# casys-kaist/CoVA

Measured on AMD Instinct MI355X. Metric: compressed-domain frames/sec (BlobNet+bboxcc) at 1080p b=256, higher is better.
Workload: dtype f16

## Files before the change

cova_amd/_lib.py:

```python
from __future__ import annotations

import ctypes as C
import os

import numpy as np

_HERE = os.path.dirname(os.path.abspath(__file__))
LIB_PATH = os.path.join(_HERE, "libcovahip.so")

OK = 0
MEM_HOST, MEM_DEVICE = 0, 1
AU_DELTA_UNIT, AU_DISCONT, AU_DROPPABLE = 1, 2, 4


class CovahipError(RuntimeError):
    def __init__(self, status: int, where: str, detail: str = ""):
        self.status = status
        try:
            text = lib().covahip_strerror(status).decode()
        except AttributeError:
            text = "error"
        msg = f"{where}: {text} (status {status})"
        if detail:
            msg += f" [{detail}]"
# ... 114 lines not shown
    "covahip_memcpy_h2d": (C.c_int, [_P, _P, _P, _SZ]),
    "covahip_memcpy_d2h": (C.c_int, [_P, _P, _P, _SZ]),
    "covahip_memset": (C.c_int, [_P, _P, C.c_int, _SZ]),
    "covahip_timer_start": (C.c_int, [_P, C.c_int]),
    "covahip_timer_stop": (C.c_int, [_P, C.c_int]),
    "covahip_timer_elapsed_ms": (C.c_int, [_P, C.c_int, C.POINTER(C.c_float)]),
    "covahip_profile_enable": (C.c_int, [_P, C.c_int]),
    "covahip_profile_filter": (C.c_int, [_P, C.c_char_p]),
    "covahip_profile_reset": (C.c_int, [_P]),
    "covahip_profile_read": (C.c_int, [_P, _P, C.c_int, C.POINTER(C.c_int)]),
    "covahip_blobnet_load": (C.c_int, [_P, _P, _SZ, C.c_int, C.c_int, C.c_int, C.c_int]),
    "covahip_blobnet_forward": (C.c_int, [_P, _P, C.c_int, _P, _P, C.c_int]),
    "covahip_blobnet_macs_per_frame": (C.c_int, [_P, C.POINTER(C.c_int64)]),
    "covahip_bboxcc": (C.c_int, [_P, _P, C.c_int, C.c_int, C.c_int, C.c_int, _P, _P, C.c_int, C.c_int]),
    "covahip_filter_forward": (C.c_int, [_P, _P, C.c_int, C.c_int, _P, _P, C.c_int, _P, _P, C.c_int]),
    "covahip_filter_forward_frames": (C.c_int, [_P, _P, C.c_int, _P, C.c_int, C.c_int, _P, _P, C.c_int, _P, _P, C.c_int]),
    "covahip_pipe_create": (C.c_int, [_P, C.c_int, C.c_int, C.c_int, C.c_int, C.c_int, C.POINTER(_P)]),
    "covahip_pipe_destroy": (None, [_P]),
    "covahip_pipe_set_packed": (C.c_int, [_P, C.c_int]),
    "covahip_pipe_set_blocking_wait": (C.c_int, [_P, C.c_int]),
    "covahip_pipe_acquire": (C.c_int, [_P, C.POINTER(C.c_int), C.POINTER(_P), C.POINTER(_P)]),
    "covahip_pipe_submit": (C.c_int, [_P, C.c_int, C.c_int, C.c_int, C.c_int]),
    "covahip_pipe_wait": (C.c_int, [_P, C.c_int]),
    "covahip_pipe_abort": (C.c_int, [_P, C.c_int]),
    "covahip_pipe_collect": (C.c_int, [_P, C.c_int, C.POINTER(_P), C.POINTER(_P), C.POINTER(_P), C.POINTER(_P)]),
    "covahip_pipe_release": (C.c_int, [_P, C.c_int]),
    "covahip_boxes_to_bbox": (None, [_P, C.c_int, _P]),
    "covahip_bbox_serialize_vec": (_SZ, [_P, _SZ, _P, _SZ, C.POINTER(C.c_int)]),
    "covahip_bbox_deserialize_vec": (C.c_int, [_P, _SZ, _P, _SZ, C.POINTER(_SZ)]),
    "covahip_frame_serialize": (_SZ, [C.c_uint64, C.c_uint64, _P, _SZ, _P, _SZ, C.POINTER(C.c_int)]),
    "covahip_bbox_iou": (C.c_float, [_P, _P]),
    "covahip_tfrecord_example": (_SZ, [_P, _P, C.c_int, C.c_int, C.c_int, C.c_int, _P, _SZ, C.POINTER(C.c_int)]),
    "covahip_bbox_csv": (_SZ, [_P, _SZ, C.c_int, _P, _SZ, C.POINTER(C.c_int)]),
    "covahip_tracks_export": (_SZ, [C.c_uint64, C.c_uint64, _P, _P, _SZ, _P, _SZ, C.POINTER(C.c_int)]),
    "covahip_assoc_default_cfg": (None, [C.POINTER(AssocCfg)]),
    "covahip_assoc_new": (C.c_int, [C.POINTER(AssocCfg), _P, _SZ, C.POINTER(_P)]),
    "covahip_assoc_free": (None, [_P]),
    "covahip_assoc_push_track": (C.c_int, [_P, C.c_uint64, C.c_uint64, _P, _SZ]),
    "covahip_assoc_push_track_frame": (C.c_int, [_P, _P, _SZ]),
    "covahip_assoc_push_dnn": (C.c_int, [_P, _P, _SZ]),
    "covahip_assoc_push_dnn_text": (C.c_int, [_P, C.c_char_p, _SZ]),
    "covahip_assoc_terminate": (C.c_int, [_P]),
    "covahip_assoc_csv": (_SZ, [_P, C.c_int, _P, _SZ, C.POINTER(C.c_int)]),
    "covahip_h264_open_mp4": (C.c_int, [_P, _SZ, C.POINTER(_P)]),
    "covahip_h264_close": (None, [_P]),
    "covahip_h264_get_info": (C.c_int, [_P, _P]),
    "covahip_h264_sample": (C.c_int, [_P, C.c_int, C.POINTER(C.c_uint64), C.POINTER(C.c_uint32), C.POINTER(C.c_int)]),
    "covahip_h264_sample_slices": (C.c_int, [_P, C.c_int, _P, C.c_int, C.POINTER(C.c_int)]),
    "covahip_h264_decode_records": (C.c_int, [_P, C.c_int, _P, _SZ]),
    "covahip_h264_display_order": (C.c_int, [_P, C.c_void_p, C.c_int, C.POINTER(C.c_int)]),
    "covahip_h264_colocated": (C.c_int, [_P, C.c_int, C.POINTER(C.c_int), C.POINTER(C.c_int)]),
    "covahip_h264_open_avcc": (C.c_int, [_P, _SZ, C.POINTER(_P)]),
    "covahip_h264_decode_au": (C.c_int, [_P, _P, _SZ, _P, _SZ, _P, C.POINTER(C.c_int64)]),
    "covahip_carrier_write_records": (C.c_int, [_P, _P, _P, C.c_int, C.c_int, _P, _SZ]),
    "covahip_carrier_pack": (None, [_P, _SZ, _P]),
    "covahip_filter_forward_frames_packed": (C.c_int, [_P, _P, C.c_int, _P, C.c_int, C.c_int, _P, _P, C.c_int, _P, _P]),
    "covahip_blobnet_load_set": (C.c_int, [_P, C.c_int, _P, _P, C.c_int, C.c_int, C.c_int, C.c_int]),
    "covahip_blobnet_num_models": (C.c_int, [_P, _P]),
    "covahip_blobnet_set_post": (C.c_int, [_P, C.c_int, C.POINTER(BlobNetPost)]),
    "covahip_blobnet_get_post": (C.c_int, [_P, C.c_int, C.POINTER(C.c_float), _P, C.POINTER(C.c_int)]),
    "covahip_blobnet_set_area": (C.c_int, [_P, C.c_int, C.c_int]),
    "covahip_blobnet_get_area": (C.c_int, [_P, C.c_int, C.POINTER(C.c_int)]),
    "covahip_bboxcc_v": (C.c_int, [_P, _P, C.c_int, C.c_int, C.c_int, _P, _P, _P, C.c_int, C.c_int]),
    "covahip_pipe_model_ids": (C.c_int, [_P, C.c_int, _P]),
    "covahip_blobnet_forward_m": (C.c_int, [_P, _P, _P, C.c_int, _P, _P, C.c_int]),
    "covahip_filter_forward_m": (C.c_int, [_P, _P, _P, C.c_int, C.c_int, _P, _P, C.c_int, _P, _P, C.c_int]),
    "covahip_filter_forward_frames_m": (C.c_int, [_P, _P, C.c_int, _P, _P, C.c_int, C.c_int, _P, _P, C.c_int, _P, _P, C.c_int]),
    "covahip_filter_forward_frames_packed_m": (C.c_int, [_P, _P, C.c_int, _P, _P, C.c_int, C.c_int, _P, _P, C.c_int, _P, _P]),
    "covahip_stack_new": (C.c_int, [_SZ, C.c_uint, C.c_uint, C.POINTER(_P)]),
    "covahip_stack_free": (None, [_P]),
    "covahip_stack_push": (C.c_int, [_P, _P, _SZ, _P, _SZ, C.POINTER(C.c_int)]),
    "covahip_stack_out_dims": (None, [C.c_int, C.c_int, C.c_uint, C.POINTER(C.c_int), C.POINTER(C.c_int)]),
    "covahip_sort_new": (C.c_int, [C.c_uint64, C.c_uint64, C.c_float, C.POINTER(_P)]),
    "covahip_sort_free": (None, [_P]),
    "covahip_sort_update": (C.c_int, [_P, _P, _SZ, C.c_uint64, _P, _SZ, C.POINTER(_SZ), _P, _SZ, C.POINTER(_SZ)]),
    "covahip_sort_finalize": (C.c_int, [_P, _P, _SZ, C.POINTER(_SZ), _P, _SZ, C.POINTER(_SZ)]),
    "covahip_sort_mark_seen": (C.c_int, [_P, C.c_uint64]),
    "covahip_sort_num_trackers": (C.c_int, [_P, C.POINTER(_SZ)]),
    "covahip_sort_tracker_info": (C.c_int, [_P, _SZ, C.POINTER(C.c_uint64), C.POINTER(C.c_int),
                                            C.POINTER(C.c_uint64), C.POINTER(C.c_uint64), _P]),
    "covahip_sort_tracker_predict": (C.c_int, [_P, _SZ, C.c_uint64, _P]),
    "covahip_sort_tracker_update": (C.c_int, [_P, _SZ, _P]),
    "covahip_linear_assignment": (_SZ, [_P, _SZ, _SZ, _P, _SZ]),
    "covahip_gopfilter_default_cfg": (None, [C.POINTER(GopFilterCfg)]),
    "covahip_gopfilter_new": (C.c_int, [C.POINTER(GopFilterCfg), C.POINTER(_P)]),
    "covahip_gopfilter_free": (None, [_P]),
    "covahip_gopfilter_push_enc": (C.c_int, [_P, C.c_uint64, C.c_uint64, C.c_uint32]),
    "covahip_gopfilter_push_boxes": (C.c_int, [_P, _P, _SZ, C.c_uint64, _P, _SZ, C.POINTER(_SZ)]),
    "covahip_gopfilter_eos": (C.c_int, [_P, _P, _SZ, C.POINTER(_SZ)]),
    "covahip_gopfilter_take_dropped": (C.c_int, [_P, _P, _SZ, C.POINTER(_SZ)]),
    "covahip_gopfilter_take_track_export": (_SZ, [_P, _P, _SZ, C.POINTER(C.c_int)]),
    "covahip_gopfilter_counters": (C.c_int, [_P, C.POINTER(C.c_uint64), C.POINTER(C.c_uint64),
                                             C.POINTER(C.c_uint64)]),
    "covahip_train_default_cfg": (None, [C.POINTER(TrainCfg)]),
    "covahip_train_create": (C.c_int, [_P, C.POINTER(TrainCfg), _P, _SZ, C.POINTER(_P)]),
    "covahip_train_step": (C.c_int, [_P, _P, _P, C.c_int, C.c_float, C.POINTER(C.c_float), C.c_int]),
    "covahip_train_metrics": (C.c_int, [_P, C.POINTER(C.c_int64)]),
    "covahip_train_weights": (C.c_int, [_P, _P, _SZ, C.POINTER(_SZ)]),
    "covahip_train_grads": (C.c_int, [_P, _P, _SZ]),
    "covahip_train_create_set": (C.c_int, [_P, C.POINTER(TrainCfg), C.c_int, _P, _P, _P, C.POINTER(_P)]),
    "covahip_train_num_models": (C.c_int, [_P, C.POINTER(C.c_int)]),
    "covahip_train_step_set": (C.c_int, [_P, _P, _P, _P, _P, _P, C.c_int]),
    "covahip_train_metrics_m": (C.c_int, [_P, C.c_int, C.POINTER(C.c_int64)]),
    "covahip_train_weights_m": (C.c_int, [_P, C.c_int, _P, _SZ, C.POINTER(_SZ)]),
    "covahip_train_grads_m": (C.c_int, [_P, C.c_int, _P, _SZ]),
    "covahip_train_eval": (C.c_int, [_P, _P, _P, C.c_int, _P, _P, C.POINTER(TrainEvalResult), C.c_int]),
    "covahip_train_eval_set": (C.c_int, [_P, _P, _P, _P, _P, _P, C.POINTER(TrainEvalResult), C.c_int]),
    "covahip_train_state_size": (C.c_int, [_P, C.POINTER(_SZ)]),
    "covahip_train_save_state": (C.c_int, [_P, C.c_uint64, _P, _SZ, C.POINTER(_SZ)]),
    "covahip_train_load_state": (C.c_int, [_P, _P, _SZ, C.POINTER(C.c_uint64)]),
    "covahip_train_set_plan": (C.c_int, [_P, C.POINTER(TrainPlan)]),
    "covahip_train_get_plan": (C.c_int, [_P, C.POINTER(TrainPlan)]),
    "covahip_train_set_post": (C.c_int, [_P, C.c_int, C.POINTER(BlobNetPost)]),
    "covahip_train_get_post": (C.c_int, [_P, C.c_int, C.POINTER(C.c_float), _P, C.POINTER(C.c_int)]),
    "covahip_train_destroy": (None, [_P]),
    "covahip_train_data_create": (C.c_int, [_P, C.c_int, C.c_int, C.c_int64, C.POINTER(_P)]),
    "covahip_train_data_append": (C.c_int, [_P, _P, _P, C.c_int, C.c_int, C.POINTER(C.c_int64)]),
    "covahip_train_data_frames": (C.c_int, [_P, C.POINTER(C.c_int64)]),
    "covahip_train_data_gather": (C.c_int, [_P, _P, C.c_int, _P, _P, C.c_int]),
    "covahip_train_data_label_mass": (C.c_int, [_P, C.c_int64, C.c_int64, _P, _P, C.c_int]),
    "covahip_train_data_destroy": (None, [_P]),
    "covahip_train_step_data": (C.c_int, [_P, _P, _P, C.c_int, C.c_float, C.POINTER(C.c_float)]),
    "covahip_train_step_set_data": (C.c_int, [_P, _P, _P, _P, _P, _P]),
    "covahip_train_eval_data": (C.c_int, [_P, _P, _P, C.c_int, _P, _P, C.POINTER(TrainEvalResult), C.c_int]),
    "covahip_train_eval_set_data": (C.c_int, [_P, _P, _P, _P, _P, _P, C.POINTER(TrainEvalResult), C.c_int]),
    "covahip_post_sweep": (C.c_int, [_P, C.POINTER(SweepCfg), _P, _P, C.c_int, C.c_int, _P, _P, _P, C.POINTER(SweepResult)]),
    "covahip_post_heat_begin": (C.c_int, [_P, C.POINTER(HeatCfg)]),
    "covahip_post_heat_add": (C.c_int, [_P, _P, _P, C.c_int, C.c_int]),
    "covahip_post_heat_end": (C.c_int, [_P, _P, _P, _P, C.POINTER(C.c_int64)]),
    "covahip_monitor_begin": (C.c_int, [_P, C.POINTER(MonitorCfg)]),
    "covahip_monitor_add": (C.c_int, [_P, _P, _P, _P, _P, C.c_int, C.c_int]),
    "covahip_monitor_read": (C.c_int, [_P, C.c_int, _P, _P, _P, _P, _P, _P, C.POINTER(C.c_int64), C.POINTER(C.c_int64)]),
    "covahip_monitor_end": (C.c_int, [_P]),
    "covahip_mog_default_cfg": (None, [C.POINTER(MogCfg)]),
    "covahip_mog_create": (C.c_int, [_P, C.POINTER(MogCfg), C.POINTER(_P)]),
    "covahip_mog_create_grid": (C.c_int, [_P, C.POINTER(MogCfg), C.c_int, C.POINTER(_P)]),
    "covahip_mog_dims": (C.c_int, [_P, C.POINTER(C.c_int32), C.POINTER(C.c_int32), C.POINTER(C.c_int32), C.POINTER(C.c_int32)]),
    "covahip_mog_apply": (C.c_int, [_P, _P, C.c_int, _P, _P, C.c_int]),
    "covahip_mog_yuv_tight": (C.c_int, [_P, C.c_int, C.c_int, C.POINTER(MogYuv)]),
    "covahip_mog_apply_yuv": (C.c_int, [_P, C.POINTER(MogYuv), _P, C.c_int, _P, _P, C.c_int]),
    "covahip_mog_reset": (C.c_int, [_P, C.c_int]),
    "covahip_mog_destroy": (None, [_P]),
}

DEV_PROTOTYPES = {
    "covahip_blobnet_set_impl": (C.c_int, [_P, C.c_int]),
    "covahip_bboxcc_set_wave_cap": (C.c_int, [_P, C.c_int]),
    "covahip_blobnet_set_enc_plan": (C.c_int, [_P, C.c_int, C.c_int, C.c_int]),
    "covahip_dev_clock_mhz": (C.c_int, [_P, C.c_int, C.POINTER(C.c_float)]),
    "covahip_dev_graph_probe": (C.c_int, [_P, _P, C.c_int, _P, C.c_int, C.c_int, _P, _P, C.c_int, _P, C.c_int, C.POINTER(C.c_float),
                                          C.POINTER(C.c_float)]),
    "covahip_dev_bboxcc_overflow": (C.c_int, [_P, C.POINTER(C.c_int32)]),
    "covahip_dev_blobnet_tail_form": (C.c_int, [_P, C.POINTER(C.c_int)]),
    "covahip_dev_pipe_queue_plan": (C.c_int, [_P, C.POINTER(C.c_int), C.POINTER(C.c_int)]),
    "covahip_dev_blobnet_buffer": (C.c_int, [_P, C.c_int, C.c_int, C.POINTER(C.c_void_p), C.POINTER(C.c_size_t), C.POINTER(C.c_int32)]),
    "covahip_dev_mog_masks": (C.c_int, [_P, _P, _P, _SZ, C.POINTER(C.c_int)]),
    "covahip_dev_mog_state": (C.c_int, [_P, C.c_int, _P, _P, _P, _P, C.POINTER(C.c_int64)]),
    "covahip_dev_mog_set_stage_budget": (C.c_int, [_P, _SZ]),
    "covahip_dev_mog_post_masks": (C.c_int, [_P, _P, C.c_int, _P]),
    "covahip_dev_mog_set_post_form": (C.c_int, [_P, C.c_int, C.c_int]),
    "covahip_dev_mog_band_plan": (C.c_int, [C.c_int, C.c_int, C.POINTER(C.c_int), C.POINTER(C.c_int), C.POINTER(C.c_size_t)]),
    "covahip_dev_monitor_slice": (C.c_int, [_P, C.c_int]),
    "covahip_dev_heat_set_stage": (C.c_int, [_P, _SZ]),
    "covahip_dev_train_data_set_stage": (C.c_int, [_P, _SZ]),
}

_lib = None


def lib() -> C.CDLL:
    global _lib
    if _lib is None:
        san = os.environ.get("COVAHIP_HOST_SAN_LIB")
        if san:
            L = C.CDLL(san)
            for name, (res, args) in list(PROTOTYPES.items()) + list(DEV_PROTOTYPES.items()):
                fn = getattr(L, name, None)
                if fn is not None:
                    fn.restype = res
                    fn.argtypes = args
            _lib = L
            return _lib
        if not os.path.exists(LIB_PATH):
            raise ImportError(
                f"{LIB_PATH} not found: build it with `python -c 'import __graft_entry__ as g; g.build()'` "
                "or `make -C cova_amd/csrc` -- cova_amd has no CPU fallback")
        L = C.CDLL(LIB_PATH)
        for name, (res, args) in list(PROTOTYPES.items()) + list(DEV_PROTOTYPES.items()):
            fn = getattr(L, name)
            fn.restype = res
            fn.argtypes = args
        _lib = L
    return _lib


def check(status: int, where: str, ctx=None) -> None:
    if status != OK:
        detail = ""
        if ctx is not None and status == 3:
            detail = lib().covahip_last_hip_error(ctx).decode()
        raise CovahipError(status, where, detail)
```

cova_amd/csrc/blobnet.h:

```cpp
#pragma once
#include <hip/hip_fp16.h>

#include <vector>

#include "blobnet_params.h"
#include "internal.h"

constexpr int BN_KTAB_STACKS = 256;

struct BnLevelGeom {
    int H, W;
};

struct BnWorkspace {
    bool ready = false;
    __half *act[BN_LEVELS + 1] = {};
    __half *dact[BN_LEVELS] = {};
    __half *pbuf = nullptr;
    size_t pbuf_frames = 0;
    float *part = nullptr;
    ResidentTable<int32_t> index;
    int index_frames = 0;
    std::vector<int32_t> kept_table;
    ResidentTable<uint8_t> models;
    ResidentTable<int32_t> areas;
};

struct covahip_blobnet {
    int H = 0, W = 0, max_batch = 0;
    int n_models = 1;
    BnLevelGeom lv[BN_LEVELS + 1];
    int enc_c[BN_LEVELS + 1], dec_ci[BN_LEVELS], dec_co[BN_LEVELS];
    int dec_cy[BN_LEVELS], dec_cx[BN_LEVELS];
    BnWorkspace ws[COVAHIP_MAX_LANES];
    void *d_prepared = nullptr;
    size_t prepared_bytes = 0;
    struct Prepared *prep = nullptr;
    int fuse_tail = 1;
    int fuse_dec = 1;
    int enc1_tile16 = 1;
    int tail_rows = 1;
    int tail_part = 1;
    int fuse_enc23 = 1;
    int enc_rowtiles = 1;
    int64_t macs_per_frame = 0;
    std::vector<float> post_thr;
    std::vector<int32_t> post_area;
    bool area_on = false;
    std::vector<std::vector<uint8_t>> post_keep;
    bool post_on = false;
    void *d_post = nullptr;
    size_t post_area_off = 0, post_keep_off = 0, post_planes_off = 0, post_keep_stride = 0, post_planes_stride = 0, post_bytes = 0;
    covahip_blobnet() {
        std::copy(BN_ENC_C, BN_ENC_C + BN_LEVELS + 1, enc_c);
        std::copy(BN_DEC_CI, BN_DEC_CI + BN_LEVELS, dec_ci);
        std::copy(BN_DEC_CO, BN_DEC_CO + BN_LEVELS, dec_co);
    }
};

constexpr int BN_E1_MAXW = 62;
inline bool bn_level1_on_enc1(const covahip_ctx *ctx, const covahip_blobnet *m) {
    return m->enc1_tile16 && m->enc_c[1] == 16 && m->enc_c[2] == 32 && m->lv[1].W <= BN_E1_MAXW && m->lv[1].H >= 2 &&
           !ctx->enc_plan[1].nbands;
}

int blobnet_prepare_mfma(covahip_ctx *ctx, covahip_blobnet *m, const float *const *h_weights, int n_models);
void blobnet_release_mfma(covahip_ctx *ctx, covahip_blobnet *m);
struct BnCcTail {
    int area_thresh, max_boxes;
    covahip_box *boxes;
    int32_t *counts;
};
struct BnInput {
    const uint8_t *stack = nullptr;
    const uint8_t *frames = nullptr;
    int n_frames = 0;
    const int32_t *index = nullptr;
    const int32_t *h_index = nullptr;
    bool packed = false;
    bool dry = false;
    int model = 0;
    const uint8_t *model_ids = nullptr;
    const uint8_t *frame_models = nullptr;
    const uint8_t *h_model_ids = nullptr;
    bool mixed = false;
};
int blobnet_forward_mfma(covahip_ctx *ctx, covahip_blobnet *m, BnWorkspace &ws, const BnInput &in, int batch, float *d_logits,
                         uint8_t *d_mask, const BnCcTail *cc = nullptr, bool *cc_done = nullptr);
```

cova_amd/csrc/blobnet.hip:

```cpp
#include <algorithm>
#include <cmath>
#include <cstdlib>
#include <cstring>
#include <vector>

#include "blobnet.h"
#include "covahip_dev.h"

static void free_model(covahip_ctx *ctx, covahip_blobnet *m) {
    if (!m) return;
    blobnet_release_mfma(ctx, m);
    if (m->d_post) hipFree(m->d_post);
    for (BnWorkspace &ws : m->ws) {
        for (int i = 0; i <= BN_LEVELS; i++)
            if (ws.act[i]) hipFree(ws.act[i]);
        for (int j = 0; j < BN_LEVELS; j++)
            if (ws.dact[j]) hipFree(ws.dact[j]);
        if (ws.pbuf) hipFree(ws.pbuf);
        if (ws.part) hipFree(ws.part);
        ws.index.release();
        ws.models.release();
        ws.areas.release();
    }
    delete m;
}

void covahip_blobnet_destroy(covahip_ctx *ctx) {
    if (!ctx->blobnet) return;
    hipSetDevice(ctx->device);
    covahip_sync_all(ctx);
    covahip_monitor_close(ctx, true);
    free_model(ctx, ctx->blobnet);
    ctx->blobnet = nullptr;
}

int covahip_blobnet_geometry(covahip_ctx *ctx, int *h, int *w) {
    if (!ctx->blobnet) return COVAHIP_ERR_NOT_LOADED;
    *h = ctx->blobnet->H;
    *w = ctx->blobnet->W;
    return COVAHIP_OK;
}

static int check_model_ids(const covahip_blobnet *m, const uint8_t *model_ids, int batch) {
    if (model_ids)
        for (int b = 0; b < batch; b++)
            if (model_ids[b] >= m->n_models) return COVAHIP_ERR_INVALID_ARG;
    return COVAHIP_OK;
}

static int resolve_models(covahip_ctx *ctx, covahip_blobnet *m, BnWorkspace &ws, const uint8_t *model_ids, int batch,
                          const int32_t *table, int n_frames, BnInput &in) {
    in.model = 0;
    in.model_ids = nullptr;
    in.frame_models = nullptr;
    in.h_model_ids = nullptr;
    if (!model_ids) return COVAHIP_OK;
    if (int rc = check_model_ids(m, model_ids, batch)) return rc;
    bool uniform = true;
    for (int b = 1; b < batch && uniform; b++) uniform = model_ids[b] == model_ids[0];
    if (uniform) {
        in.model = model_ids[0];
        return COVAHIP_OK;
    }
    std::vector<uint8_t> ids((size_t)batch + n_frames, 0);
    std::vector<uint8_t> seen((size_t)n_frames, 0);
    std::copy(model_ids, model_ids + batch, ids.begin());
    for (int b = 0; b < batch; b++)
        for (int t = 0; t < BN_T; t++) {
            const int f = table ? table[(size_t)b * BN_T + t] : b * BN_T + t;
            uint8_t &fm = ids[(size_t)batch + f];
            if (seen[f] && fm != model_ids[b]) return COVAHIP_ERR_INVALID_ARG;
            seen[f] = 1;
            fm = model_ids[b];
        }
    if (int rc = ws.models.reserve(ctx, (size_t)m->max_batch * (1 + BN_T))) return rc;
    if (int rc = ws.models.upload(ctx, ids.data(), ids.size(), &in.model_ids)) return rc;
    in.frame_models = in.model_ids + batch;
    in.h_model_ids = model_ids;
    return COVAHIP_OK;
}

static int resolve_areas(covahip_ctx *ctx, covahip_blobnet *m, BnWorkspace &ws, const BnInput &in, int batch, int area_thresh,
                         const int32_t **d_out) {
    *d_out = nullptr;
    if (!m->area_on) return COVAHIP_OK;
    std::vector<int32_t> eff((size_t)batch);
    for (int b = 0; b < batch; b++) {
        const int32_t a = m->post_area[in.h_model_ids ? in.h_model_ids[b] : in.model];
        eff[b] = a >= 1 ? a : area_thresh;
    }
    if (int rc = ws.areas.reserve(ctx, (size_t)m->max_batch)) return rc;
    return ws.areas.upload(ctx, eff.data(), eff.size(), d_out);
}

static int ensure_pbuf(covahip_ctx *ctx, covahip_blobnet *m, BnWorkspace &ws, int n_frames);
static int filter_dev(covahip_ctx *ctx, BnInput &in, int batch, float *d_logits, uint8_t *d_mask,
                      bool with_cc, int area_thresh, covahip_box *d_boxes, int32_t *d_counts, int max_boxes,
                      const uint8_t *model_ids = nullptr) {
    covahip_blobnet *m = ctx->blobnet;
    if (!m) return COVAHIP_ERR_NOT_LOADED;
    if (batch > m->max_batch) return COVAHIP_ERR_INVALID_ARG;
    if (batch == 0) return COVAHIP_OK;
    if (in.stack) {
        int rc = resolve_models(ctx, m, m->ws[ctx->cur_lane], model_ids, batch, nullptr, batch * BN_T, in);
        if (rc) return rc;
        rc = ensure_pbuf(ctx, m, m->ws[ctx->cur_lane], batch * BN_T);
        if (rc) return rc;
    }
    BnCcTail tail{area_thresh, max_boxes, d_boxes, d_counts};
    bool cc_done = false;
    int rc = blobnet_forward_mfma(ctx, m, m->ws[ctx->cur_lane], in, batch, d_logits, d_mask, with_cc ? &tail : nullptr, &cc_done);
    if (rc) return rc;
    if (with_cc && !cc_done) {
        const int32_t *d_areas = nullptr;
        rc = resolve_areas(ctx, m, m->ws[ctx->cur_lane], in, batch, area_thresh, &d_areas);
        if (rc) return rc;
        rc = covahip_bboxcc_launch(ctx, d_mask, batch, m->H, m->W, area_thresh, d_boxes, d_counts, max_boxes, d_areas);
    }
    return rc;
}

static int prepare_frames(covahip_ctx *ctx, covahip_blobnet *m, BnWorkspace &ws, const uint8_t *d_frames, int n_frames,
                          const int32_t *stack_index, int batch, BnInput &in, const uint8_t *model_ids = nullptr) {
    if (n_frames < BN_T || n_frames > BN_T * m->max_batch) return COVAHIP_ERR_INVALID_ARG;
    if (!stack_index && batch != n_frames - (BN_T - 1)) return COVAHIP_ERR_INVALID_ARG;
    std::vector<int32_t> table((size_t)batch * BN_T);
    for (int b = 0; b < batch; b++)
        for (int t = 0; t < BN_T; t++) {
            const int32_t f = stack_index ? stack_index[b * BN_T + t] : b + (BN_T - 1) - t;
            if (f < 0 || f >= n_frames) return COVAHIP_ERR_INVALID_ARG;
            table[(size_t)b * BN_T + t] = f;
        }
    if (int rc = resolve_models(ctx, m, ws, model_ids, batch, table.data(), n_frames, in)) return rc;
    const bool by_value = batch <= BN_KTAB_STACKS && n_frames <= 65535 && bn_level1_on_enc1(ctx, m);
    in.frames = d_frames;
    in.n_frames = n_frames;
    if (by_value) {
        ws.kept_table = std::move(table);
        in.h_index = ws.kept_table.data();
    } else {
        if (n_frames != ws.index_frames) ws.index.invalidate();
        if (int rc = ws.index.reserve(ctx, (size_t)m->max_batch * BN_T)) return rc;
        if (int rc = ws.index.upload(ctx, table.data(), table.size(), &in.index)) return rc;
        ws.index_frames = n_frames;
    }
    return ensure_pbuf(ctx, m, ws, n_frames);
}

static int ensure_pbuf(covahip_ctx *ctx, covahip_blobnet *m, BnWorkspace &ws, int n_frames) {
    if (ws.pbuf_frames < (size_t)n_frames) {
        const size_t want = std::min((size_t)BN_T * m->max_batch, std::max((size_t)n_frames, 2 * ws.pbuf_frames));
        const size_t bytes = want * m->lv[1].H * m->lv[1].W * m->enc_c[1] * sizeof(__half);
        if (ws.pbuf) {
            COVAHIP_CHECK_HIP(ctx, hipStreamSynchronize(ctx->stream));
            COVAHIP_CHECK_HIP(ctx, hipFree(ws.pbuf));
            ws.pbuf = nullptr;
            ws.pbuf_frames = 0;
        }
        COVAHIP_CHECK_HIP(ctx, hipMalloc((void **)&ws.pbuf, bytes));
        COVAHIP_CHECK_HIP(ctx, hipMemsetAsync(ws.pbuf, 0, bytes, ctx->stream));
        ws.pbuf_frames = want;
    }
    return COVAHIP_OK;
}

int covahip_blobnet_forward_dev(covahip_ctx *ctx, const uint8_t *d_stack, int batch, float *d_logits,
                                uint8_t *d_mask, const uint8_t *model_ids) {
    BnInput in;
    in.stack = d_stack;
    return filter_dev(ctx, in, batch, d_logits, d_mask, false, 0, nullptr, nullptr, 0, model_ids);
}

static int alloc_workspace(covahip_ctx *ctx, covahip_blobnet *m, BnWorkspace &ws) {
    if (ws.ready) return COVAHIP_OK;
    for (int i = 1; i <= BN_LEVELS; i++) {
        const size_t tt = (i == BN_LEVELS) ? 1 : BN_T;
        const size_t n = (size_t)m->max_batch * tt * m->lv[i].H * m->lv[i].W * m->enc_c[i];
        COVAHIP_CHECK_HIP(ctx, hipMalloc((void **)&ws.act[i], n * sizeof(__half)));
        COVAHIP_CHECK_HIP(ctx, hipMemsetAsync(ws.act[i], 0, n * sizeof(__half), ctx->stream));
    }
    for (int j = 0; j < BN_LEVELS - 1; j++) {
        const BnLevelGeom out = m->lv[BN_LEVELS - 1 - j];
        const size_t n = (size_t)m->max_batch * out.H * out.W * m->dec_co[j];
        COVAHIP_CHECK_HIP(ctx, hipMalloc((void **)&ws.dact[j], n * sizeof(__half)));
    }
    COVAHIP_CHECK_HIP(ctx, hipMalloc((void **)&ws.part, (size_t)m->max_batch * (m->lv[1].H + 1) * (m->lv[1].W + 1) * 4 * sizeof(float)));
    ws.ready = true;
    return COVAHIP_OK;
}

int covahip_blobnet_grow_lanes(covahip_ctx *ctx, int n_lanes) {
    covahip_blobnet *m = ctx->blobnet;
    if (!m) return COVAHIP_OK;
    for (int k = 0; k < n_lanes && k < COVAHIP_MAX_LANES; k++) {
        const int rc = alloc_workspace(ctx, m, m->ws[k]);
        if (rc) return rc;
    }
    COVAHIP_CHECK_HIP(ctx, hipStreamSynchronize(ctx->stream));
    return COVAHIP_OK;
}

static int build_model(covahip_ctx *ctx, covahip_blobnet *m, const float *const *h_w, int n_models, int h_mb, int w_mb, int max_batch) {
    m->H = h_mb;
    m->W = w_mb;
    m->max_batch = max_batch;
    m->lv[0] = {h_mb, w_mb};
    for (int i = 0; i < BN_LEVELS; i++) m->lv[i + 1] = {(m->lv[i].H + 1) / 2, (m->lv[i].W + 1) / 2};
    for (int j = 0; j < BN_LEVELS; j++) {
        const BnLevelGeom in = m->lv[BN_LEVELS - j], out = m->lv[BN_LEVELS - 1 - j];
        const int ph = 2 * in.H + 2 - out.H, pw = 2 * in.W + 2 - out.W;
        if (ph < 0 || pw < 0) return COVAHIP_ERR_UNSUPPORTED;
        m->dec_cy[j] = ph / 2 + ph % 2;
        m->dec_cx[j] = pw / 2 + pw % 2;
    }
    int64_t macs = 0;
    for (int i = 0; i < BN_LEVELS; i++) {
        macs += (int64_t)BN_T * m->lv[i].H * m->lv[i].W * 9 * m->enc_c[i] * m->enc_c[i + 1];
        macs += (int64_t)m->lv[i + 1].H * m->lv[i + 1].W * m->enc_c[i + 1] * 32;
    }
    for (int j = 0; j < BN_LEVELS; j++) {
        const BnLevelGeom in = m->lv[BN_LEVELS - j];
        macs += (int64_t)in.H * in.W * 16 * m->dec_ci[j] * m->dec_co[j];
    }
    macs += (int64_t)h_mb * w_mb * 16;
    m->macs_per_frame = macs;

    for (int k = 0; k < ctx->n_lanes; k++) {
        const int rc = alloc_workspace(ctx, m, m->ws[k]);
        if (rc) return rc;
    }
    int rc = blobnet_prepare_mfma(ctx, m, h_w, n_models);
    if (rc) return rc;
    m->post_thr.assign(n_models, 0.f);
    m->post_keep.assign(n_models, {});
    m->post_area.assign(n_models, 0);
    BnInput plan;
    plan.dry = true;
    for (int pass = 0; pass < (n_models > 1 ? 8 : 4) && !rc; pass++) {
        const int b = (pass & 1) ? max_batch : 1;
        plan.n_frames = (pass & 2) ? b + BN_T - 1 : 0;
        plan.mixed = (pass & 4) != 0;
        rc = blobnet_forward_mfma(ctx, m, m->ws[0], plan, b, nullptr, nullptr, nullptr, nullptr);
    }
    return rc;
}

extern "C" {

int covahip_blobnet_load(covahip_ctx *ctx, const void *weights, size_t weights_bytes, int h_mb, int w_mb, int t,
                         int max_batch) {
    if (!ctx || !weights) return COVAHIP_ERR_INVALID_ARG;
    if (t == BN_T && h_mb >= 16 && w_mb >= 16 && h_mb <= 1024 && w_mb <= 1024 && max_batch > 0 && !bn_check_blob(weights, weights_bytes))
        return COVAHIP_ERR_BAD_WEIGHTS;
    return covahip_blobnet_load_set(ctx, 1, &weights, &weights_bytes, h_mb, w_mb, t, max_batch);
}

int covahip_blobnet_load_set(covahip_ctx *ctx, int n_models, const void *const *weights, const size_t *weights_bytes, int h_mb,
                             int w_mb, int t, int max_batch) {
    if (!ctx || !weights || !weights_bytes || h_mb <= 0 || w_mb <= 0 || max_batch <= 0) return COVAHIP_ERR_INVALID_ARG;
    if (n_models < 1 || n_models > COVAHIP_MAX_MODELS) return COVAHIP_ERR_INVALID_ARG;
    for (int k = 0; k < n_models; k++)
        if (!weights[k]) return COVAHIP_ERR_INVALID_ARG;
    if (t != BN_T) return COVAHIP_ERR_UNSUPPORTED;
    if (h_mb < 16 || w_mb < 16 || h_mb > 1024 || w_mb > 1024) return COVAHIP_ERR_UNSUPPORTED;
    std::vector<const float *> h_w(n_models);
    bool bad = false;
    for (int k = 0; k < n_models; k++) bad = bad || !(h_w[k] = bn_check_blob(weights[k], weights_bytes[k]));

    COVAHIP_CHECK_HIP(ctx, hipSetDevice(ctx->device));
    covahip_blobnet_destroy(ctx);
    if (bad) return COVAHIP_ERR_BAD_WEIGHTS;
    covahip_blobnet *m = new covahip_blobnet();
    int rc = build_model(ctx, m, h_w.data(), n_models, h_mb, w_mb, max_batch);
    if (rc == COVAHIP_OK && hipStreamSynchronize(ctx->stream) != hipSuccess) rc = COVAHIP_ERR_HIP;
    if (rc) {
        hipStreamSynchronize(ctx->stream);
        (void)hipGetLastError();
        free_model(ctx, m);
        return rc;
    }
    ctx->blobnet = m;
    return COVAHIP_OK;
}

int covahip_blobnet_num_models(covahip_ctx *ctx, int *n_models) {
    if (!ctx || !n_models) return COVAHIP_ERR_INVALID_ARG;
    if (!ctx->blobnet) return COVAHIP_ERR_NOT_LOADED;
    *n_models = ctx->blobnet->n_models;
    return COVAHIP_OK;
}

static int upload_post(covahip_ctx *ctx, covahip_blobnet *m) {
    const size_t hw = (size_t)m->H * m->W, n = (size_t)m->n_models;
    if (!m->d_post) {
        m->post_keep_stride = (hw + 15) & ~(size_t)15;
        m->post_planes_stride = (size_t)m->H * 16;
        m->post_area_off = n * sizeof(float);
        m->post_keep_off = align256(m->post_area_off + n * sizeof(int32_t));
        m->post_planes_off = align256(m->post_keep_off + n * m->post_keep_stride);
        m->post_bytes = m->post_planes_off + n * m->post_planes_stride;
        COVAHIP_CHECK_HIP(ctx, hipMalloc(&m->d_post, m->post_bytes));
    }
    std::vector<uint8_t> host(m->post_bytes, 0);
    std::memcpy(host.data(), m->post_thr.data(), n * sizeof(float));
    std::memcpy(host.data() + m->post_area_off, m->post_area.data(), n * sizeof(int32_t));
    for (size_t k = 0; k < n; k++) {
        uint8_t *kb = host.data() + m->post_keep_off + k * m->post_keep_stride;
        uint32_t *kp = reinterpret_cast<uint32_t *>(host.data() + m->post_planes_off + k * m->post_planes_stride);
        const std::vector<uint8_t> &keep = m->post_keep[k];
        for (int y = 0; y < m->H; y++)
            for (int x = 0; x < m->W; x++) {
                const bool on = keep.empty() || keep[(size_t)y * m->W + x];
                kb[(size_t)y * m->W + x] = on ? 1 : 0;
                if (on && x < 128) kp[y * 4 + 2 * (x & 1) + (x >> 6)] |= 1u << ((x >> 1) & 31);
            }
    }
    COVAHIP_CHECK_HIP(ctx, hipMemcpy(m->d_post, host.data(), host.size(), hipMemcpyHostToDevice));
    return COVAHIP_OK;
}

static int commit_post(covahip_ctx *ctx, covahip_blobnet *m) {
    bool on = false, area = false;
    for (int k = 0; k < m->n_models; k++) {
        area = area || m->post_area[k] >= 1;
        on = on || m->post_thr[k] != 0.f || !m->post_keep[k].empty() || m->post_area[k] >= 1;
    }
    if (on || m->d_post) {
        if (int rc = upload_post(ctx, m)) {
            m->post_thr.assign(m->n_models, 0.f);
            m->post_keep.assign(m->n_models, {});
            m->post_area.assign(m->n_models, 0);
            m->post_on = m->area_on = false;
            return rc;
        }
    }
    m->post_on = on;
    m->area_on = area;
    return COVAHIP_OK;
}

int covahip_blobnet_set_post(covahip_ctx *ctx, int model, const covahip_blobnet_post *post) {
    if (!ctx) return COVAHIP_ERR_INVALID_ARG;
    covahip_blobnet *m = ctx->blobnet;
    if (!m) return COVAHIP_ERR_NOT_LOADED;
    if (model < 0 || model >= m->n_models) return COVAHIP_ERR_INVALID_ARG;
    if (post && !std::isfinite(post->logit_thresh)) return COVAHIP_ERR_INVALID_ARG;
    COVAHIP_CHECK_HIP(ctx, hipSetDevice(ctx->device));
    if (int rc = covahip_sync_all(ctx)) return rc;
    const size_t hw = (size_t)m->H * m->W;
    m->post_thr[model] = post ? post->logit_thresh : 0.f;
    m->post_keep[model].clear();
    if (post && post->keep) {
        m->post_keep[model].resize(hw);
        for (size_t i = 0; i < hw; i++) m->post_keep[model][i] = post->keep[i] ? 1 : 0;
    }
    return commit_post(ctx, m);
}

int covahip_blobnet_set_area(covahip_ctx *ctx, int model, int area_thresh) {
    if (!ctx) return COVAHIP_ERR_INVALID_ARG;
    covahip_blobnet *m = ctx->blobnet;
    if (!m) return COVAHIP_ERR_NOT_LOADED;
    if (model < 0 || model >= m->n_models || area_thresh < 0) return COVAHIP_ERR_INVALID_ARG;
    COVAHIP_CHECK_HIP(ctx, hipSetDevice(ctx->device));
    if (int rc = covahip_sync_all(ctx)) return rc;
    m->post_area[model] = area_thresh;
    return commit_post(ctx, m);
}

int covahip_blobnet_get_area(covahip_ctx *ctx, int model, int *area_thresh) {
    if (!ctx || !area_thresh) return COVAHIP_ERR_INVALID_ARG;
    covahip_blobnet *m = ctx->blobnet;
    if (!m) return COVAHIP_ERR_NOT_LOADED;
    if (model < 0 || model >= m->n_models) return COVAHIP_ERR_INVALID_ARG;
    *area_thresh = m->post_area[model];
    return COVAHIP_OK;
}

int covahip_blobnet_get_post(covahip_ctx *ctx, int model, float *logit_thresh, uint8_t *keep_or_null, int *has_keep) {
    if (!ctx) return COVAHIP_ERR_INVALID_ARG;
    covahip_blobnet *m = ctx->blobnet;
    if (!m) return COVAHIP_ERR_NOT_LOADED;
    if (model < 0 || model >= m->n_models) return COVAHIP_ERR_INVALID_ARG;
    const std::vector<uint8_t> &keep = m->post_keep[model];
    if (logit_thresh) *logit_thresh = m->post_thr[model];
    if (has_keep) *has_keep = keep.empty() ? 0 : 1;
    if (keep_or_null) {
        const size_t hw = (size_t)m->H * m->W;
        if (keep.empty()) std::memset(keep_or_null, 1, hw);
        else std::memcpy(keep_or_null, keep.data(), hw);
    }
    return COVAHIP_OK;
}

int covahip_blobnet_macs_per_frame(covahip_ctx *ctx, int64_t *macs) {
    if (!ctx || !macs) return COVAHIP_ERR_INVALID_ARG;
    if (!ctx->blobnet) return COVAHIP_ERR_NOT_LOADED;
    *macs = ctx->blobnet->macs_per_frame;
    return COVAHIP_OK;
}

int covahip_blobnet_set_enc_plan(covahip_ctx *ctx, int level, int nbands, int nbuf) {
    if (!ctx || level < 1 || level > 3 || nbands < 0 || nbands > 64 || (nbands && nbuf != 1 && nbuf != 2)) return COVAHIP_ERR_INVALID_ARG;
    ctx->enc_plan[level].nbands = nbands;
    ctx->enc_plan[level].nbuf = nbands ? nbuf : 0;
    return COVAHIP_OK;
}

int covahip_blobnet_set_impl(covahip_ctx *ctx, int impl) {
    if (!ctx || !ctx->blobnet) return COVAHIP_ERR_NOT_LOADED;
    if (impl != 1 && (impl < 4 || impl > 10)) return COVAHIP_ERR_INVALID_ARG;
    ctx->blobnet->fuse_dec = impl != 4;
    ctx->blobnet->enc1_tile16 = impl != 5;
    ctx->blobnet->enc_rowtiles = impl != 6;
    ctx->blobnet->fuse_enc23 = impl == 7 ? 0 : impl == 8 ? 2 : 1;
    ctx->blobnet->tail_part = impl != 9;
    ctx->blobnet->tail_rows = impl != 10;
    return COVAHIP_OK;
}

static int filter_placed(covahip_ctx *ctx, covahip_blobnet *m, const uint8_t *d_src, int n_frames, const int32_t *stack_index,
                         int batch, int area_thresh, covahip_box *d_boxes, int32_t *d_counts, int max_boxes, float *d_logits,
                         uint8_t *d_mask, bool packed = false, const uint8_t *model_ids = nullptr) {
    if (!d_mask) {
        CtxLane &l = ctx->lane();
        int rc = covahip_ensure_buffer(ctx, &l.cc_scratch, &l.cc_scratch_bytes, (size_t)batch * m->H * m->W);
        if (rc) return rc;
        d_mask = (uint8_t *)l.cc_scratch;
    }
    BnInput in;
    if (n_frames > 0) {
        int rc = prepare_frames(ctx, m, m->ws[ctx->cur_lane], d_src, n_frames, stack_index, batch, in, model_ids);
        if (rc) return rc;
        in.packed = packed;
    } else {
        in.stack = d_src;
    }
    int rc = filter_dev(ctx, in, batch, d_logits, d_mask, true, area_thresh, d_boxes, d_counts, max_boxes, n_frames > 0 ? nullptr : model_ids);
    if (rc == COVAHIP_OK && batch > 0 && ctx->mon && ctx->mon->attached && !ctx->mon_suspended)
        rc = covahip_monitor_hook(ctx, d_mask, d_counts, d_boxes, max_boxes, model_ids, batch);
    return rc;
}

static int filter_any(covahip_ctx *ctx, const uint8_t *src, int n_frames, const int32_t *stack_index, int batch,
                      int area_thresh, covahip_box *boxes, int32_t *counts, int max_boxes, float *logits, uint8_t *mask,
                      int mem_kind, const uint8_t *model_ids = nullptr) {
    if (!ctx || batch < 0 || max_boxes < 0 || n_frames < 0) return COVAHIP_ERR_INVALID_ARG;
    covahip_blobnet *m = ctx->blobnet;
    if (!m) return COVAHIP_ERR_NOT_LOADED;
    if (batch == 0) return COVAHIP_OK;
    if (!src || !counts || (!boxes && max_boxes > 0) || batch > m->max_batch) return COVAHIP_ERR_INVALID_ARG;
    if (int rc = check_model_ids(m, model_ids, batch)) return rc;
    COVAHIP_CHECK_HIP(ctx, hipSetDevice(ctx->device));
    const bool by_frames = n_frames > 0;
    const size_t hw = (size_t)m->H * m->W;
    const size_t in_bytes = by_frames ? (size_t)n_frames * hw * 4 : (size_t)batch * BN_T * hw * 4;
    const size_t mask_bytes = (size_t)batch * hw;
    const size_t logit_bytes = mask_bytes * sizeof(float);
    const size_t box_bytes = (size_t)batch * max_boxes * sizeof(covahip_box);
    const size_t cnt_bytes = (size_t)batch * sizeof(int32_t);
    if (mem_kind != COVAHIP_MEM_DEVICE && mem_kind != COVAHIP_MEM_HOST) return COVAHIP_ERR_INVALID_ARG;

    if (mem_kind == COVAHIP_MEM_DEVICE) {
        LaneScope lane(ctx);
        if (!lane.ok()) return COVAHIP_ERR_HIP;
        return filter_placed(ctx, m, src, n_frames, stack_index, batch, area_thresh, boxes, counts, max_boxes, logits, mask, false, model_ids);
    }
    if (int rc = covahip_primary_op(ctx)) return rc;
    const uint8_t *d_src = src;
    int rc = covahip_ensure_buffer(ctx, &ctx->stage_in, &ctx->stage_in_bytes, in_bytes);
    if (rc) return rc;
    rc = covahip_ensure_buffer(ctx, &ctx->stage_out, &ctx->stage_out_bytes,
                               align256(mask_bytes) + align256(logit_bytes) + align256(box_bytes) + align256(cnt_bytes));
    if (rc) return rc;
    uint8_t *base = (uint8_t *)ctx->stage_out;
    uint8_t *d_mask = base;
    float *d_logits = logits ? (float *)(base + align256(mask_bytes)) : nullptr;
    covahip_box *d_boxes = (covahip_box *)(base + align256(mask_bytes) + align256(logit_bytes));
    int32_t *d_counts = (int32_t *)(base + align256(mask_bytes) + align256(logit_bytes) + align256(box_bytes));
    COVAHIP_CHECK_HIP(ctx, hipMemcpyAsync(ctx->stage_in, src, in_bytes, hipMemcpyHostToDevice, ctx->stream));
    d_src = (const uint8_t *)ctx->stage_in;
    rc = filter_placed(ctx, m, d_src, n_frames, stack_index, batch, area_thresh, d_boxes, d_counts, max_boxes, d_logits, d_mask, false,
                       model_ids);
    if (rc) return rc;
    if (logits) COVAHIP_CHECK_HIP(ctx, hipMemcpyAsync(logits, d_logits, logit_bytes, hipMemcpyDeviceToHost, ctx->stream));
    if (mask) COVAHIP_CHECK_HIP(ctx, hipMemcpyAsync(mask, d_mask, mask_bytes, hipMemcpyDeviceToHost, ctx->stream));
    if (box_bytes) COVAHIP_CHECK_HIP(ctx, hipMemcpyAsync(boxes, d_boxes, box_bytes, hipMemcpyDeviceToHost, ctx->stream));
    COVAHIP_CHECK_HIP(ctx, hipMemcpyAsync(counts, d_counts, cnt_bytes, hipMemcpyDeviceToHost, ctx->stream));
    COVAHIP_CHECK_HIP(ctx, hipStreamSynchronize(ctx->stream));
    return COVAHIP_OK;
}

int covahip_filter_forward(covahip_ctx *ctx, const uint8_t *rgba_stack, int batch, int area_thresh,
                           covahip_box *boxes, int32_t *counts, int max_boxes, float *logits, uint8_t *mask,
                           int mem_kind) {
    return filter_any(ctx, rgba_stack, 0, nullptr, batch, area_thresh, boxes, counts, max_boxes, logits, mask, mem_kind);
}

int covahip_filter_forward_m(covahip_ctx *ctx, const uint8_t *rgba_stack, const uint8_t *model_ids, int batch, int area_thresh,
                             covahip_box *boxes, int32_t *counts, int max_boxes, float *logits, uint8_t *mask, int mem_kind) {
    return filter_any(ctx, rgba_stack, 0, nullptr, batch, area_thresh, boxes, counts, max_boxes, logits, mask, mem_kind, model_ids);
}

int covahip_filter_forward_frames(covahip_ctx *ctx, const uint8_t *frames, int n_frames, const int32_t *stack_index,
                                  int batch, int area_thresh, covahip_box *boxes, int32_t *counts, int max_boxes,
                                  float *logits, uint8_t *mask, int mem_kind) {
    if (n_frames <= 0) return COVAHIP_ERR_INVALID_ARG;
    return filter_any(ctx, frames, n_frames, stack_index, batch, area_thresh, boxes, counts, max_boxes, logits, mask, mem_kind);
}

int covahip_filter_forward_frames_m(covahip_ctx *ctx, const uint8_t *frames, int n_frames, const int32_t *stack_index,
                                    const uint8_t *model_ids, int batch, int area_thresh, covahip_box *boxes, int32_t *counts,
                                    int max_boxes, float *logits, uint8_t *mask, int mem_kind) {
    if (n_frames <= 0) return COVAHIP_ERR_INVALID_ARG;
    return filter_any(ctx, frames, n_frames, stack_index, batch, area_thresh, boxes, counts, max_boxes, logits, mask, mem_kind,
                      model_ids);
}

int covahip_filter_forward_frames_packed(covahip_ctx *ctx, const uint16_t *d_records, int n_frames, const int32_t *stack_index,
                                         int batch, int area_thresh, covahip_box *d_boxes, int32_t *d_counts, int max_boxes,
                                         float *d_logits, uint8_t *d_mask) {
    return covahip_filter_forward_frames_packed_m(ctx, d_records, n_frames, stack_index, nullptr, batch, area_thresh, d_boxes,
                                                  d_counts, max_boxes, d_logits, d_mask);
}

int covahip_filter_forward_frames_packed_m(covahip_ctx *ctx, const uint16_t *d_records, int n_frames, const int32_t *stack_index,
                                           const uint8_t *model_ids, int batch, int area_thresh, covahip_box *d_boxes,
                                           int32_t *d_counts, int max_boxes, float *d_logits, uint8_t *d_mask) {
    if (!ctx || batch < 0 || max_boxes < 0 || n_frames <= 0) return COVAHIP_ERR_INVALID_ARG;
    covahip_blobnet *m = ctx->blobnet;
    if (!m) return COVAHIP_ERR_NOT_LOADED;
    if (batch == 0) return COVAHIP_OK;
    if (!d_records || !d_counts || (!d_boxes && max_boxes > 0) || batch > m->max_batch) return COVAHIP_ERR_INVALID_ARG;
    if (int rc = check_model_ids(m, model_ids, batch)) return rc;
    COVAHIP_CHECK_HIP(ctx, hipSetDevice(ctx->device));
    LaneScope lane(ctx);
    if (!lane.ok()) return COVAHIP_ERR_HIP;
    return filter_placed(ctx, m, reinterpret_cast<const uint8_t *>(d_records), n_frames, stack_index, batch, area_thresh, d_boxes, d_counts,
                         max_boxes, d_logits, d_mask, true, model_ids);
}

int covahip_dev_blobnet_tail_form(covahip_ctx *ctx, int *form) {
    if (!ctx || !form) return COVAHIP_ERR_INVALID_ARG;
    *form = ctx->tail_form;
    return COVAHIP_OK;
}

int covahip_dev_blobnet_buffer(covahip_ctx *ctx, int which, int index, void **dptr, size_t *bytes, int32_t dims[5]) {
    if (!ctx || !dptr || !bytes || !dims) return COVAHIP_ERR_INVALID_ARG;
    covahip_blobnet *m = ctx->blobnet;
    if (!m) return COVAHIP_ERR_NOT_LOADED;
    const BnWorkspace &ws = m->ws[0];
    int64_t d[5] = {0, 0, 0, 0, 0};
    size_t elem = sizeof(__half);
    void *p = nullptr;
    if (which == 0 && index == 0) {
        p = ws.pbuf;
        d[0] = (int64_t)ws.pbuf_frames; d[1] = m->lv[1].H; d[2] = m->lv[1].W; d[3] = m->enc_c[1];
    } else if (which == 1 && index >= 1 && index <= BN_LEVELS) {
        p = ws.act[index];
        const BnLevelGeom g = m->lv[index];
        if (index < BN_LEVELS) { d[0] = m->max_batch; d[1] = BN_T; d[2] = g.H; d[3] = g.W; d[4] = m->enc_c[index]; }
        else { d[0] = m->max_batch; d[1] = g.H; d[2] = g.W; d[3] = m->enc_c[index]; }
    } else if (which == 2 && index >= 0 && index < BN_LEVELS - 1) {
        p = ws.dact[index];
        const BnLevelGeom g = m->lv[BN_LEVELS - 1 - index];
        d[0] = m->max_batch; d[1] = g.H; d[2] = g.W; d[3] = m->dec_co[index];
    } else if (which == 3 && index == 0) {
        p = ws.part;
        elem = sizeof(float);
        d[0] = m->max_batch; d[1] = m->lv[1].H + 1; d[2] = m->lv[1].W + 1; d[3] = 4;
    } else {
        return COVAHIP_ERR_INVALID_ARG;
    }
    size_t n = p ? elem : 0;
    for (int k = 0; k < 5; k++) {
        dims[k] = p ? (int32_t)d[k] : 0;
        if (d[k]) n *= (size_t)d[k];
    }
    *dptr = p;
    *bytes = n;
    return COVAHIP_OK;
}

int covahip_dev_graph_probe(covahip_ctx *ctx, const uint8_t *d_frames, int n_frames, const int32_t *stack_index, int batch,
                            int area_thresh, covahip_box *d_boxes, int32_t *d_counts, int max_boxes, uint8_t *d_mask, int iters,
                            float *ms_direct, float *ms_graph) {
    if (!ctx || !ctx->blobnet || !ms_direct || !ms_graph || iters < 1) return COVAHIP_ERR_INVALID_ARG;
    covahip_blobnet *m = ctx->blobnet;
    COVAHIP_CHECK_HIP(ctx, hipSetDevice(ctx->device));
    if (int rc = covahip_primary_op(ctx)) return rc;
    if (!m->fuse_tail) return COVAHIP_ERR_UNSUPPORTED;
    hipEvent_t e0 = nullptr, e1 = nullptr;
    hipGraph_t graph = nullptr;
    hipGraphExec_t exec = nullptr;
    int rc = COVAHIP_OK;
    auto hip_ok = [&](hipError_t e, const char *what) {
        if (e == hipSuccess || rc) return e == hipSuccess;
        ctx->last_hip_error = std::string(what) + ": " + hipGetErrorString(e);
        rc = COVAHIP_ERR_HIP;
        return false;
    };
    auto run = [&](int n) {
        for (int i = 0; i < n && !rc; i++)
            rc = filter_placed(ctx, m, d_frames, n_frames, stack_index, batch, area_thresh, d_boxes, d_counts, max_boxes, nullptr, d_mask);
    };
    bool capturing = false;
    const bool was_suspended = ctx->mon_suspended;
    ctx->mon_suspended = true;
    do {
        if (!hip_ok(hipEventCreate(&e0), "hipEventCreate") || !hip_ok(hipEventCreate(&e1), "hipEventCreate")) break;
        run(3);
        if (rc || !hip_ok(hipStreamSynchronize(ctx->stream), "hipStreamSynchronize")) break;
        if (!hip_ok(hipEventRecord(e0, ctx->stream), "hipEventRecord")) break;
        run(iters);
        if (rc || !hip_ok(hipEventRecord(e1, ctx->stream), "hipEventRecord") || !hip_ok(hipEventSynchronize(e1), "hipEventSynchronize") ||
            !hip_ok(hipEventElapsedTime(ms_direct, e0, e1), "hipEventElapsedTime"))
            break;
        if (!hip_ok(hipStreamBeginCapture(ctx->stream, hipStreamCaptureModeRelaxed), "hipStreamBeginCapture")) break;
        capturing = true;
        run(1);
        capturing = false;
        const hipError_t ee = hipStreamEndCapture(ctx->stream, &graph);
        if (rc || !hip_ok(ee, "hipStreamEndCapture")) break;
        if (!hip_ok(hipGraphInstantiate(&exec, graph, nullptr, nullptr, 0), "hipGraphInstantiate")) break;
        for (int i = 0; i < 3 && !rc; i++) hip_ok(hipGraphLaunch(exec, ctx->stream), "hipGraphLaunch");
        if (rc || !hip_ok(hipStreamSynchronize(ctx->stream), "hipStreamSynchronize") || !hip_ok(hipEventRecord(e0, ctx->stream), "hipEventRecord")) break;
        for (int i = 0; i < iters && !rc; i++) hip_ok(hipGraphLaunch(exec, ctx->stream), "hipGraphLaunch");
        if (rc || !hip_ok(hipEventRecord(e1, ctx->stream), "hipEventRecord") || !hip_ok(hipEventSynchronize(e1), "hipEventSynchronize")) break;
        hip_ok(hipEventElapsedTime(ms_graph, e0, e1), "hipEventElapsedTime");
    } while (false);
    ctx->mon_suspended = was_suspended;
    if (capturing) (void)hipStreamEndCapture(ctx->stream, &graph);
    if (exec) (void)hipGraphExecDestroy(exec);
    if (graph) (void)hipGraphDestroy(graph);
    if (e0) (void)hipEventDestroy(e0);
    if (e1) (void)hipEventDestroy(e1);
    return rc;
}

int covahip_blobnet_forward(covahip_ctx *ctx, const uint8_t *rgba_stack, int batch, float *logits, uint8_t *mask,
                            int mem_kind) {
    return covahip_blobnet_forward_m(ctx, rgba_stack, nullptr, batch, logits, mask, mem_kind);
}

int covahip_blobnet_forward_m(covahip_ctx *ctx, const uint8_t *rgba_stack, const uint8_t *model_ids, int batch, float *logits,
                              uint8_t *mask, int mem_kind) {
    if (!ctx || batch < 0) return COVAHIP_ERR_INVALID_ARG;
    covahip_blobnet *m = ctx->blobnet;
    if (!m) return COVAHIP_ERR_NOT_LOADED;
    if (batch == 0) return COVAHIP_OK;
    if (!rgba_stack || batch > m->max_batch) return COVAHIP_ERR_INVALID_ARG;
    if (int rc = check_model_ids(m, model_ids, batch)) return rc;
    COVAHIP_CHECK_HIP(ctx, hipSetDevice(ctx->device));
    if (int prc = covahip_primary_op(ctx)) return prc;
    if (mem_kind == COVAHIP_MEM_DEVICE) return covahip_blobnet_forward_dev(ctx, rgba_stack, batch, logits, mask, model_ids);
    if (mem_kind != COVAHIP_MEM_HOST) return COVAHIP_ERR_INVALID_ARG;
    const size_t hw = (size_t)m->H * m->W;
    const size_t in_bytes = (size_t)batch * BN_T * hw * 4;
    const size_t mask_bytes = (size_t)batch * hw;
    const size_t logit_bytes = mask_bytes * sizeof(float);
    int rc = covahip_ensure_buffer(ctx, &ctx->stage_in, &ctx->stage_in_bytes, in_bytes);
    if (rc) return rc;
    rc = covahip_ensure_buffer(ctx, &ctx->stage_out, &ctx->stage_out_bytes, align256(mask_bytes) + align256(logit_bytes));
    if (rc) return rc;
    uint8_t *d_mask = (uint8_t *)ctx->stage_out;
    float *d_logits = (float *)((uint8_t *)ctx->stage_out + align256(mask_bytes));
    COVAHIP_CHECK_HIP(ctx, hipMemcpyAsync(ctx->stage_in, rgba_stack, in_bytes, hipMemcpyHostToDevice, ctx->stream));
    rc = covahip_blobnet_forward_dev(ctx, (const uint8_t *)ctx->stage_in, batch, logits ? d_logits : nullptr,
                                     mask ? d_mask : nullptr, model_ids);
    if (rc) return rc;
    if (logits) COVAHIP_CHECK_HIP(ctx, hipMemcpyAsync(logits, d_logits, logit_bytes, hipMemcpyDeviceToHost, ctx->stream));
    if (mask) COVAHIP_CHECK_HIP(ctx, hipMemcpyAsync(mask, d_mask, mask_bytes, hipMemcpyDeviceToHost, ctx->stream));
    COVAHIP_CHECK_HIP(ctx, hipStreamSynchronize(ctx->stream));
    return COVAHIP_OK;
}

}
```

cova_amd/csrc/blobnet_mfma.hip:

```cpp
#include <algorithm>
#include <cmath>
#include <cstdlib>
#include <cstring>
#include <mutex>
#include <type_traits>
#include <utility>
#include <vector>

#include "bboxcc_body.h"
#include "bboxcc_wave.h"
#include "blobnet.h"
#include "covahip_dev.h"

typedef _Float16 half8 __attribute__((ext_vector_type(8)));
typedef _Float16 half4 __attribute__((ext_vector_type(4)));
typedef float f32x16 __attribute__((ext_vector_type(16)));
typedef float f32x4 __attribute__((ext_vector_type(4)));
typedef _Float16 half2v __attribute__((ext_vector_type(2)));

namespace {

constexpr float BN_EPS = 1e-3f;
constexpr int WG = 256;

struct EncPrep {
    size_t wfrag;
    size_t epi;
};
struct DecPrep {
    size_t wfrag;
    size_t epi;
};

}

struct Prepared {
    EncPrep enc[BN_LEVELS];
    DecPrep dec[BN_LEVELS - 1];
    size_t enc1w;
    size_t final_w;
    size_t final_epi;
    size_t final_w_up;
    size_t tail_w;
    size_t zero;
    bool allpos[BN_LEVELS];
    size_t total;
};

namespace {

inline _Float16 f2h(float v) { return (_Float16)v; }

__device__ __forceinline__ uint32_t fdiv(uint32_t n, uint32_t mul) { return mul ? __umulhi(n, mul) : n; }
inline uint32_t magic(uint32_t d) { return d <= 1 ? 0u : (uint32_t)(((1ull << 32) / d) + 1); }

template <bool MS>
__device__ __forceinline__ uint32_t model_off(const uint8_t *mid, uint32_t stride, int idx) {
    if constexpr (!MS) return 0u;
    else return __builtin_amdgcn_readfirstlane((uint32_t)mid[idx] * stride);
}
template <typename T>
__device__ __forceinline__ const T *at_model(const T *ptr, uint32_t off) {
    return reinterpret_cast<const T *>(reinterpret_cast<const uint8_t *>(ptr) + off);
}
template <typename T>
using gptr = const __attribute__((address_space(1))) T *;
template <typename T>
__device__ __forceinline__ gptr<T> as_global(const T *ptr) {
    return (gptr<T>)ptr;
}

template <bool ALLPOS>
__device__ __forceinline__ float pool4(float a0, float a1, float a2, float a3, float e0, float e1, float e2) {
    if constexpr (ALLPOS) {
        const float t = fmaxf(fmaxf(a0, a1), a2);
        return fmaxf(fmaxf(t, a3), e0) + e1;
    } else {
        const float mx = fmaxf(fmaxf(fmaxf(a0, a1), a2), a3);
        return __builtin_amdgcn_fmed3f(mx, e0, e2) + e1;
    }
}

struct TmixW {
    half4 a1, a2, id;
};
__device__ __forceinline__ TmixW load_tmix(const float *tm, int lane) {
    const int i = lane & 3;
    TmixW w;
#pragma unroll
    for (int t = 0; t < BN_T; t++) {
        w.a1[t] = (_Float16)tm[t * BN_T + i];
        w.a2[t] = (_Float16)tm[16 + t * BN_T + i];
        w.id[t] = (_Float16)(t == i ? 1.f : 0.f);
    }
    return w;
}
template <int N>
__device__ __forceinline__ void tmix_core(const TmixW &w, const half4 (&pb)[N], f32x4 (&sum)[N], f32x4 (&pvf)[N]) {
    const f32x4 z = {0.f, 0.f, 0.f, 0.f};
    const half4 hz = {(_Float16)0, (_Float16)0, (_Float16)0, (_Float16)0};
    f32x4 u[N];
#pragma unroll
    for (int e = 0; e < N; e++) u[e] = __builtin_amdgcn_mfma_f32_4x4x4f16(w.a1, pb[e], z, 0, 0, 0);
#pragma unroll
    for (int e = 0; e < N; e++) pvf[e] = __builtin_amdgcn_mfma_f32_4x4x4f16(w.id, pb[e], z, 0, 0, 0);
#pragma unroll
    for (int e = 0; e < N; e++) {
        const half4 ub = __builtin_elementwise_max(__builtin_convertvector(u[e], half4), hz);
        sum[e] = __builtin_amdgcn_mfma_f32_4x4x4f16(w.a2, ub, pvf[e], 0, 0, 0);
    }
}
template <int N>
__device__ __forceinline__ void tmix4f(const TmixW &w, const half4 (&pb)[N], f32x4 (&r)[N]) {
    f32x4 sum[N], pvf[N];
    tmix_core<N>(w, pb, sum, pvf);
#pragma unroll
    for (int e = 0; e < N; e++)
#pragma unroll
        for (int t = 0; t < BN_T; t++) r[e][t] = fmaxf(fmaxf(sum[e][t], pvf[e][t]), 0.f);
}
template <int N>
__device__ __forceinline__ void tmix4h(const TmixW &w, const half4 (&pb)[N], half4 (&o)[N]) {
    f32x4 r[N];
    tmix4f<N>(w, pb, r);
#pragma unroll
    for (int e = 0; e < N; e++) o[e] = __builtin_convertvector(r[e], half4);
}
__device__ __forceinline__ void tmix4h(const TmixW &w, const half4 pb, half4 &o) {
    const half4 pbs[1] = {pb};
    half4 os[1];
    tmix4h<1>(w, pbs, os);
    o = os[0];
}
typedef __attribute__((address_space(3))) void lds_void;
__device__ __forceinline__ void glds16(const void *gsrc, uint8_t *lds_base_uniform) {
    const uint32_t a = __builtin_amdgcn_readfirstlane((uint32_t)(uintptr_t)(lds_void *)lds_base_uniform);
    __builtin_amdgcn_global_load_lds((const __attribute__((address_space(1))) void *)gsrc,
                                     (lds_void *)(uintptr_t)a, 16, 0, 0);
}

__device__ __forceinline__ void lds_barrier() {
    __builtin_amdgcn_fence(__ATOMIC_RELEASE, "workgroup", "local");
    __builtin_amdgcn_s_barrier();
    __builtin_amdgcn_fence(__ATOMIC_ACQUIRE, "workgroup", "local");
}
__device__ __forceinline__ void wait_vmem() { __builtin_amdgcn_s_waitcnt(0x0F70); }
template <int N>
__device__ __forceinline__ void lds_barrier_vmem_but() {
    static_assert(N >= 0 && N < 64, "vmcnt is a six-bit counter");
    asm volatile("" ::: "memory");
    __builtin_amdgcn_s_waitcnt(0x0070 | (N & 15) | ((N >> 4) << 14));
    __builtin_amdgcn_s_barrier();
    asm volatile("" ::: "memory");
}

struct Swz {
    int p, a, b, c, L;
};
template <int CPP>
__device__ __forceinline__ int swz_eval(const Swz &w, int xx, int yy) {
    return ((((yy * w.L + xx) >> w.p) * w.a) + yy * w.b + (yy & 1) * w.c) & (CPP - 1);
}

struct ItemPlan {
    int paired;
    int cnt[2];
    unsigned long long band[2];
};
struct ItemIter {
    int b, band;
    int k, j, role, half;
    int my_cnt;
    unsigned long long my_bands;
    __device__ __forceinline__ bool start(const ItemPlan &pl, int B, int nbands) {
        k = 0; j = 0;
        half = (int)gridDim.x >> 1;
        role = pl.paired && (int)blockIdx.x >= half;
        my_cnt = role ? pl.cnt[1] : pl.cnt[0];
        my_bands = role ? pl.band[1] : pl.band[0];
        return next(pl, B, nbands);
    }
    __device__ __forceinline__ bool next(const ItemPlan &pl, int B, int nbands) {
        if (!pl.paired) {
            const int item = (int)blockIdx.x + k * (int)gridDim.x;
            k++;
            if (item >= B * nbands) return false;
            b = item / nbands;
            band = item - b * nbands;
            return true;
        }
        if (j >= my_cnt) { j = 0; k++; }
        b = ((int)blockIdx.x - role * half) + k * half;
        if (b >= B) return false;
        band = (int)((my_bands >> (8 * j)) & 0xFF);
        j++;
        return true;
    }
};

struct EncArgs {
    const __half *in;
    __half *out;
    const half8 *wfrag;
    const float *epi;
    int B, H, W, Hp, Wp, Ho, Wo, oy, ox, To;
    int RB, nbands, TR, TC;
    uint32_t mWp, mNb, mRC;
    const void *zero;
    Swz swz;
    int scr_off;
    int nbuf, buf_stride;
    ItemPlan plan;
// ... 1273 lines not shown
            if constexpr (!FINAL) {
#pragma unroll
                for (int r = 0; r < 16; r++) {
                    const int n = mtile * 32 + (r & 3) + 8 * (r >> 2) + 4 * kh;
                    es[r] = ep[n % COUT];
                    eb[r] = ep[COUT + n % COUT];
                }
            } else {
                fbias = ep[0];
            }
        }
        const int u0 = band * GH / p.nbands, u1 = (band + 1) * GH / p.nbands;
        const int nu = u1 - u0;
        lds_barrier();
        {
            const int RC = TC * CPP;
            const int nchunk = (nu + 1) * RC;
            const __half *su = p.up + ((size_t)b) * p.Hi * p.Wi * C1;
            const __half *ss = p.skip + ((size_t)b * p.Ts) * p.Hi * p.Wi * C2;
            for (int s0 = wave * 64; s0 < nchunk; s0 += NW * 64) {
                const int sidx = s0 + lane;
                if (sidx < nchunk) {
                    const int r = fdiv(sidx, p.mRC), within = sidx - r * RC;
                    const int c = within / CPP, chp = within % CPP;
                    const int cb = (chp ^ swz_eval<CPP>(p.swz, c, r)) * 8;
                    const int y = u0 - 1 + r, x = c - 1;
                    const void *src = p.zero;
                    if (y >= 0 && y < p.Hi && x >= 0 && x < p.Wi) {
                        const size_t pix = (size_t)y * p.Wi + x;
                        if constexpr (C1 == 0) {
                            src = ss + pix * C2 + cb;
                        } else {
                            if (cb < C1) src = su + pix * C1 + cb;
                            else src = ss + pix * C2 + (cb - C1);
                        }
                    }
                    glds16(src, smem + s0 * 16);
                }
            }
        }
        wait_vmem();
        lds_barrier();
        uint8_t *const mrows = smem + p.mask_off;
        const int Yb = max(0, 2 * u0 - p.cy), Ye = min(p.Hd, 2 * u1 - p.cy);
        const int npos = nu * GW;
        const int ntiles = (npos + 31) / 32;
        for (int tile = pgroup; tile < ntiles; tile += PG) {
            const int q = tile * 32 + (lane & 31);
            const int qc = min(q, npos - 1);
            const int ul = fdiv(qc, p.mGW), v = qc - ul * GW;
            f32x16 acc;
#pragma unroll
            for (int r = 0; r < 16; r++) acc[r] = 0.f;
#pragma unroll
            for (int a = 0; a < 2; a++)
#pragma unroll
                for (int bb = 0; bb < 2; bb++) {
                    const int yy = ul + 1 - a, xx = v + 1 - bb;
                    const int pbase = (yy * TC + xx) * PS;
                    const int s = swz_eval<CPP>(p.swz, xx, yy);
#pragma unroll
                    for (int kc = 0; kc < KC; kc++) {
                        const half8 av = *reinterpret_cast<const half8 *>(smem + pbase + (((kc * 2 + kh) ^ s) * 16));
                        acc = __builtin_amdgcn_mfma_f32_32x32x16_f16(wf[(a * 2 + bb) * KC + kc], av, acc, 0, 0, 0);
                    }
                }
            if constexpr (FINAL) {
                if (q >= npos) continue;
                const int u = u0 + ul;
                if (kh == 0) {
                    f32x4 pl = {0.f, 0.f, 0.f, 0.f};
                    if constexpr (C2 == 0) pl = reinterpret_cast<const f32x4 *>(p.part)[((size_t)b * GH + u) * GW + v];
#pragma unroll
                    for (int r = 0; r < 4; r++) {
                        const int Y = 2 * u + (r >> 1) - p.cy, X = 2 * v + (r & 1) - p.cx;
                        if (Y >= 0 && Y < p.Hd && X >= 0 && X < p.Wd) {
                            float l = acc[r] + fbias;
                            if constexpr (C2 == 0) l += pl[r];
                            if (p.logits) p.logits[((size_t)b * p.Hd + Y) * p.Wd + X] = l;
                            bool fg = l > sp.thr;
                            if constexpr (POST) fg = fg && sp.keep[Y * p.Wd + X];
                            mrows[(Y - Yb) * p.Wd + X] = fg ? 1 : 0;
                        }
                    }
                }
            } else {
                uint8_t *const scr = smem + p.scr_off + wave * 2048;
                const int pos = lane & 31;
#pragma unroll
                for (int g = 0; g < 4; g++) {
                    half4 o;
#pragma unroll
                    for (int j = 0; j < 4; j++)
                        o[j] = (_Float16)fmaxf(acc[4 * g + j] * es[4 * g + j] + eb[4 * g + j], 0.f);
                    *reinterpret_cast<half4 *>(scr + pos * 64 + ((g ^ ((pos >> 2) & 3)) * 16) + kh * 8) = o;
                }
                __builtin_amdgcn_fence(__ATOMIC_RELEASE, "wavefront");
                __builtin_amdgcn_wave_barrier();
                __builtin_amdgcn_fence(__ATOMIC_ACQUIRE, "wavefront");
#pragma unroll
                for (int j = 0; j < 2; j++) {
                    const int c = j * 64 + lane;
                    const int rp = c >> 2;
                    const int g = (c & 3) ^ ((rp >> 2) & 3);
                    const int rq = tile * 32 + rp;
                    if (rq < npos) {
                        const int rul = fdiv(rq, p.mGW), rv = rq - rul * GW;
                        const int n0 = mtile * 32 + 8 * g;
                        const int phase = n0 / COUT, co0 = n0 % COUT;
                        const int Y = 2 * (u0 + rul) + (phase >> 1) - p.cy, X = 2 * rv + (phase & 1) - p.cx;
                        if (Y >= 0 && Y < p.Hd && X >= 0 && X < p.Wd)
                            *reinterpret_cast<uint4 *>(p.out + (((size_t)b * p.Hd + Y) * p.Wd + X) * COUT + co0) =
                                *reinterpret_cast<const uint4 *>(scr + c * 16);
                    }
                }
                __builtin_amdgcn_fence(__ATOMIC_RELEASE, "wavefront");
                __builtin_amdgcn_wave_barrier();
            }
        }
        if constexpr (FINAL) {
            if (p.mask) {
                lds_barrier();
                uint8_t *dst = p.mask + ((size_t)b * p.Hd + Yb) * p.Wd;
                const int nbytes = (Ye - Yb) * p.Wd;
                if ((p.Wd & 3) == 0 && (reinterpret_cast<uintptr_t>(p.mask) & 3) == 0) {
                    for (int i = tid; i < nbytes / 4; i += NW * 64)
                        reinterpret_cast<uint32_t *>(dst)[i] = reinterpret_cast<const uint32_t *>(mrows)[i];
                } else {
                    for (int i = tid; i < nbytes; i += NW * 64) dst[i] = mrows[i];
                }
            }
        }
    }
}

struct DecLvl {
    int Hi, Wi, Hd, Wd, cy, cx;
    uint32_t mGW, mRC;
    Swz swz;
    int tile_off;
};
struct Dec012Args {
    const __half *skip[3];
    int Ts[3];
    __half *out;
    const half8 *wf[3];
    const float *epi[3];
    DecLvl lv[3];
    int B, scr_off;
    const void *zero;
    const uint8_t *model_ids;
    uint32_t mstride;
};

template <int C>
__device__ __forceinline__ void dec012_zero_border(uint8_t *tile, const DecLvl &g, int tid) {
    constexpr int CPP = C / 8;
    const int RC = (g.Wi + 2) * CPP;
    const int n_rows = 2 * RC, n_cols = 2 * CPP * g.Hi;
    for (int i = tid; i < n_rows + n_cols; i += 512) {
        int piece;
        if (i < n_rows) {
            piece = i < RC ? i : (g.Hi + 1) * RC + (i - RC);
        } else {
            const int j = i - n_rows, y = j / (2 * CPP), k = j % (2 * CPP);
            piece = (y + 1) * RC + (k < CPP ? k : (g.Wi + 1) * CPP + (k - CPP));
        }
        *reinterpret_cast<uint4 *>(tile + piece * 16) = uint4{0, 0, 0, 0};
    }
}
template <int C1, int C2>
__device__ __forceinline__ void dec012_stage(uint8_t *tile, const __half *ss, const DecLvl &g, int wave, int lane, int first) {
    constexpr int C = C1 + C2, CPP = C / 8;
    const int RC = (g.Wi + 2) * CPP, NI = g.Wi * CPP;
    for (int y = (wave + 8 - first) & 7; y < g.Hi; y += 8) {
        const int r = y + 1;
        const __half *rowp = ss + (size_t)y * g.Wi * C2;
        uint8_t *rowl = tile + (r * RC + CPP) * 16;
        for (int q0 = 0; q0 < NI; q0 += 64) {
            const int q = q0 + lane;
            const int px = q / CPP, chp = q % CPP;
            const int cb = (chp ^ swz_eval<CPP>(g.swz, px + 1, r)) * 8;
            if (q < NI && cb >= C1) glds16(rowp + px * C2 + (cb - C1), rowl + q0 * 16);
        }
    }
}

template <int C, int COUT>
struct Dec012W {
    half8 wf[4 * (C / 16)];
    float es[16], eb[16];
};
constexpr int DEC012_W0_KEPT = 4 * (128 / 16);
template <int C, int COUT>
__device__ __forceinline__ void dec012_load(Dec012W<C, COUT> &w, const half8 *wfrag, const float *epi, int wave, int lane) {
    constexpr int MT = 4 * COUT / 32, KSTEPS = 4 * (C / 16);
    const int mtile = wave % MT, kh = lane >> 5;
    asm volatile("" : "+s"(wfrag), "+s"(epi));
    const gptr<half8> wg = as_global(wfrag);
    const gptr<float> eg = as_global(epi);
#pragma unroll
    for (int ks = 0; ks < KSTEPS; ks++) w.wf[ks] = wg[(mtile * KSTEPS + ks) * 64 + lane];
#pragma unroll
    for (int gq = 0; gq < 4; gq++) {
        const int c0 = (mtile * 32 + 8 * gq + 4 * kh) % COUT;
        const f32x4 sc = *(gptr<f32x4>)(eg + c0), sh = *(gptr<f32x4>)(eg + COUT + c0);
#pragma unroll
        for (int j = 0; j < 4; j++) { w.es[4 * gq + j] = sc[j]; w.eb[4 * gq + j] = sh[j]; }
    }
}
template <int C1, int C2, int COUT, int CN>
__device__ __forceinline__ void dec012_block(const uint8_t *lds0, const uint8_t *tile, uint8_t *next_tile, __half *gout, uint8_t *scr_base,
                                             const Dec012W<C1 + C2, COUT> &w, const DecLvl &g, const DecLvl &gn,
                                             int wave, int lane) {
    constexpr int C = C1 + C2, MT = 4 * COUT / 32, PG = 8 / MT;
    constexpr int KC = C / 16, KSTEPS = 4 * KC, CPP = C / 8, PS = C * 2;
    constexpr int AD = C == 128 ? 4 : 8;
    const int mtile = wave % MT, pgroup = wave / MT;
    const int TC = g.Wi + 2, GW = g.Wi + 1, GH = g.Hi + 1;
    const int kh = lane >> 5;
    const half8 (&wf)[KSTEPS] = w.wf;
    const float (&es)[16] = w.es, (&eb)[16] = w.eb;
    const int npos = GH * GW;
    const int ntiles = (npos + 31) / 32;
    for (int tile_i = pgroup; tile_i < ntiles; tile_i += PG) {
        const int q = tile_i * 32 + (lane & 31);
        const int qc = min(q, npos - 1);
        const int u = fdiv(qc, g.mGW), v = qc - u * GW;
        const uint32_t toff = (uint32_t)(uintptr_t)(lds_void *)tile;
        uint32_t pk[4];
#pragma unroll
        for (int tp = 0; tp < 4; tp++) {
            const int yy = u + 1 - (tp >> 1), xx = v + 1 - (tp & 1);
            pk[tp] = (toff + (uint32_t)((yy * TC + xx) * PS)) | (uint32_t)((kh ^ swz_eval<CPP>(g.swz, xx, yy)) << 4);
        }
        auto frag = [&](int ks) -> half8 {
            const int tp = ks / KC, kc = ks % KC;
            typedef const __attribute__((address_space(3))) half8 *lds_half8_ptr;
            return *(lds_half8_ptr)(uintptr_t)(pk[tp] ^ (uint32_t)(kc << 5));
        };
        half8 ring[AD];
#pragma unroll
        for (int ks = 0; ks < AD; ks++) ring[ks] = frag(ks);
        f32x16 acc;
#pragma unroll
        for (int r = 0; r < 16; r++) acc[r] = 0.f;
#pragma unroll
        for (int ks = 0; ks < KSTEPS; ks++) {
            acc = __builtin_amdgcn_mfma_f32_32x32x16_f16(wf[ks], ring[ks % AD], acc, 0, 0, 0);
            if (ks + AD < KSTEPS) ring[ks % AD] = frag(ks + AD);
        }
        __builtin_amdgcn_sched_group_barrier(0x100, AD, 0);
#pragma unroll
        for (int ks = 0; ks < KSTEPS; ks++) {
            __builtin_amdgcn_sched_group_barrier(0x008, 1, 0);
            if (ks + AD < KSTEPS) __builtin_amdgcn_sched_group_barrier(0x100, 1, 0);
        }
        if constexpr (CN > 0) {
            constexpr int CPPN = CN / 8, PSN = CN * 2;
            const int TCN = gn.Wi + 2;
            static_assert(COUT >= 32 && COUT % 32 == 0, "one output pixel per lane and tile");
            const int nb = mtile * 32 + 4 * kh;
            const int phase = nb / COUT, cob = nb % COUT;
            const int Y = 2 * u + (phase >> 1) - g.cy, X = 2 * v + (phase & 1) - g.cx;
            if (q < npos && Y >= 0 && Y < g.Hd && X >= 0 && X < g.Wd) {
                const int yy = Y + 1, xx = X + 1;
                uint8_t *const pix = next_tile + (yy * TCN + xx) * PSN + (cob & 7) * 2;
                const int sw = swz_eval<CPPN>(gn.swz, xx, yy);
#pragma unroll
                for (int gq = 0; gq < 4; gq++) {
                    half4 o;
#pragma unroll
                    for (int j = 0; j < 4; j++)
                        o[j] = (_Float16)fmaxf(acc[4 * gq + j] * es[4 * gq + j] + eb[4 * gq + j], 0.f);
                    *reinterpret_cast<half4 *>(pix + ((((cob >> 3) + gq) ^ sw) * 16)) = o;
                }
            }
        } else {
            uint8_t *const scr = scr_base + wave * 2048;
            const int pos = lane & 31;
#pragma unroll
            for (int gq = 0; gq < 4; gq++) {
                half4 o;
#pragma unroll
                for (int j = 0; j < 4; j++) o[j] = (_Float16)fmaxf(acc[4 * gq + j] * es[4 * gq + j] + eb[4 * gq + j], 0.f);
                *reinterpret_cast<half4 *>(scr + pos * 64 + ((gq ^ ((pos >> 2) & 3)) * 16) + kh * 8) = o;
            }
            __builtin_amdgcn_fence(__ATOMIC_RELEASE, "wavefront");
            __builtin_amdgcn_wave_barrier();
            __builtin_amdgcn_fence(__ATOMIC_ACQUIRE, "wavefront");
#pragma unroll
            for (int j = 0; j < 2; j++) {
                const int c = j * 64 + lane;
                const int rp = c >> 2;
                const int gq = (c & 3) ^ ((rp >> 2) & 3);
                const int rq = tile_i * 32 + rp;
                if (rq < npos) {
                    const int ru = fdiv(rq, g.mGW), rv = rq - ru * GW;
                    const int n0 = mtile * 32 + 8 * gq;
                    const int phase = n0 / COUT, co0 = n0 % COUT;
                    const int Y = 2 * ru + (phase >> 1) - g.cy, X = 2 * rv + (phase & 1) - g.cx;
                    if (Y >= 0 && Y < g.Hd && X >= 0 && X < g.Wd)
                        *reinterpret_cast<uint4 *>(gout + ((size_t)Y * g.Wd + X) * COUT + co0) =
                            *reinterpret_cast<const uint4 *>(scr + c * 16);
                }
            }
            __builtin_amdgcn_fence(__ATOMIC_RELEASE, "wavefront");
            __builtin_amdgcn_wave_barrier();
        }
    }
}

template <bool MS = false>
__global__ __launch_bounds__(512, 2) void dec012_mfma(Dec012Args p) {
    extern __shared__ __attribute__((aligned(256))) uint8_t smem[];
    const int tid = threadIdx.x, lane = tid & 63, wave = tid >> 6;
    uint8_t *const t0 = smem + p.lv[0].tile_off, *const t1 = smem + p.lv[1].tile_off, *const t2 = smem + p.lv[2].tile_off;
    WGSPAN_BEGIN();
#ifdef PHASE_TIMING
    unsigned long long ph_[9] = {0, 0, 0, 0, 0, 0, 0, 0, 0}, last_ = __builtin_amdgcn_s_memrealtime();
#endif
    dec012_zero_border<128>(t0, p.lv[0], tid);
    dec012_zero_border<128>(t1, p.lv[1], tid);
    dec012_zero_border<64>(t2, p.lv[2], tid);
    for (int b = blockIdx.x; b < p.B; b += gridDim.x) {
        [[maybe_unused]] const uint32_t moff = model_off<MS>(p.model_ids, p.mstride, b);
        if (b != (int)blockIdx.x) lds_barrier();
        PHASE_MARK(0);
        {
            dec012_stage<0, 128>(t0, p.skip[0] + (size_t)b * p.Ts[0] * p.lv[0].Hi * p.lv[0].Wi * 128, p.lv[0], wave, lane, 0);
            dec012_stage<64, 64>(t1, p.skip[1] + (size_t)b * p.Ts[1] * p.lv[1].Hi * p.lv[1].Wi * 64, p.lv[1], wave, lane, p.lv[0].Hi & 7);
            dec012_stage<32, 32>(t2, p.skip[2] + (size_t)b * p.Ts[2] * p.lv[2].Hi * p.lv[2].Wi * 32, p.lv[2], wave, lane,
                                 (p.lv[0].Hi + p.lv[1].Hi) & 7);
            __builtin_amdgcn_sched_barrier(0);
            Dec012W<128, 64> w0;
            dec012_load(w0, at_model(p.wf[0], moff), at_model(p.epi[0], moff), wave, lane);
            __builtin_amdgcn_sched_barrier(0);
            PHASE_MARK(1);
            lds_barrier_vmem_but<DEC012_W0_KEPT>();
            PHASE_MARK(2);
            dec012_block<0, 128, 64, 128>(smem, t0, t1, nullptr, nullptr, w0, p.lv[0], p.lv[1], wave, lane);
        }
        PHASE_MARK(3);
        {
            Dec012W<128, 32> w1;
            dec012_load(w1, at_model(p.wf[1], moff), at_model(p.epi[1], moff), wave, lane);
            lds_barrier();
#ifdef PHASE_TIMING
            asm volatile("s_waitcnt vmcnt(0)" ::: "memory");
#endif
            PHASE_MARK(4);
            dec012_block<64, 64, 32, 64>(smem, t1, t2, nullptr, nullptr, w1, p.lv[1], p.lv[2], wave, lane);
        }
        PHASE_MARK(5);
        {
            Dec012W<64, 16> w2;
            dec012_load(w2, at_model(p.wf[2], moff), at_model(p.epi[2], moff), wave, lane);
            lds_barrier();
#ifdef PHASE_TIMING
            asm volatile("s_waitcnt vmcnt(0)" ::: "memory");
#endif
            PHASE_MARK(6);
            dec012_block<32, 32, 16, 0>(smem, t2, nullptr, p.out + (size_t)b * p.lv[2].Hd * p.lv[2].Wd * 16, smem + p.scr_off, w2,
                                        p.lv[2], p.lv[2], wave, lane);
        }
        PHASE_MARK(7);
    }
#ifdef PHASE_TIMING
    if (tid == 0)
        for (int i = 0; i < 9; i++) atomicAdd(&g_phase[48 + i], ph_[i]);
#endif
    WGSPAN_END(3);
}

struct Dec3ccArgs {
    DecArgs d;
    ccbody::CcGeom g;
    ccwave::WvGeom wg;
    int use_wv;
    covahip_box *boxes;
    int32_t *counts;
    int area_thresh, max_boxes;
    int tile_bytes;
    int mfull_off, cc_off;
    int part_off;
    DecMs ms;
};

template <bool WV, bool PART, bool MS = false, bool POST = false>
__global__ __launch_bounds__(ccbody::CC_THREADS) void dec3cc_mfma(Dec3ccArgs q, PostArg<POST> qp) {
    constexpr int C1 = 16, C2 = PART ? 0 : 16, C = C1 + C2, NW = ccbody::CC_THREADS / 64;
    constexpr int KC = C / 16, KSTEPS = 4 * KC, CPP = C / 8, PS = C * 2;
    extern __shared__ __attribute__((aligned(16))) uint8_t smem[];
    const DecArgs &p = q.d;
    const int tid = threadIdx.x, lane = tid & 63, wave = tid >> 6;
    const int TC = p.Wi + 2;
    const int GW = p.Wi + 1, GH = p.Hi + 1;
    const int kh = lane >> 5;
    float fbias = p.epi[0];
    uint8_t *const mfull = smem + q.mfull_off;
    WGSPAN_BEGIN();
#ifdef PHASE_TIMING
    unsigned long long ph_[9] = {0, 0, 0, 0, 0, 0, 0, 0, 0}, last_ = __builtin_amdgcn_s_memrealtime();
#endif

    for (int b = blockIdx.x; b < p.B; b += gridDim.x) {
        const StackPost sp = stack_post<POST, MS>(qp, q.ms.model_ids, b);
        half8 wf[KSTEPS];
        if constexpr (MS) {
            const uint32_t moff = model_off<MS>(q.ms.model_ids, q.ms.mstride, b);
            fbias = at_model(p.epi, moff)[0];
#pragma unroll
            for (int ks = 0; ks < KSTEPS; ks++) wf[ks] = at_model(p.wfrag, moff)[ks * 64 + lane];
        } else {
#pragma unroll
            for (int ks = 0; ks < KSTEPS; ks++) wf[ks] = p.wfrag[ks * 64 + lane];
        }
        auto stage = [&](int band, uint8_t *buf) {
            const int u0 = band * GH / p.nbands, u1 = (band + 1) * GH / p.nbands;
            const int RC = TC * CPP;
            const int nchunk = (u1 - u0 + 1) * RC;
            const __half *su = p.up + ((size_t)b) * p.Hi * p.Wi * C1;
            const __half *ss = p.skip + ((size_t)b * p.Ts) * p.Hi * p.Wi * C2;
            for (int s0 = wave * 64; s0 < nchunk; s0 += NW * 64) {
                const int sidx = s0 + lane;
                if (sidx < nchunk) {
                    const int r = fdiv(sidx, p.mRC), within = sidx - r * RC;
                    const int c = within / CPP, chp = within % CPP;
                    const int cb = (chp ^ swz_eval<CPP>(p.swz, c, r)) * 8;
                    const int y = u0 - 1 + r, x = c - 1;
                    const void *src = p.zero;
                    if (y >= 0 && y < p.Hi && x >= 0 && x < p.Wi) {
                        const size_t pix = (size_t)y * p.Wi + x;
                        src = (PART || cb < C1) ? (const void *)(su + pix * C1 + cb) : (const void *)(ss + pix * C2 + (cb - C1));
                    }
                    glds16(src, buf + s0 * 16);
                }
            }
        };
        if (b != (int)blockIdx.x) lds_barrier();
        PHASE_MARK(0);
        if constexpr (PART) {
            const uint8_t *ps = reinterpret_cast<const uint8_t *>(p.part) + (size_t)b * GH * GW * 16;
            const int nch = GH * GW;
            for (int s0 = wave * 64; s0 < nch; s0 += NW * 64)
                if (s0 + lane < nch) glds16(ps + (size_t)(s0 + lane) * 16, smem + q.part_off + s0 * 16);
        }
        stage(0, smem);
        PHASE_MARK(1);
        for (int band = 0; band < p.nbands; band++) {
            uint8_t *const cur = smem + (band & 1) * q.tile_bytes;
            wait_vmem();
            lds_barrier();
            PHASE_MARK(2);
            if (band + 1 < p.nbands) stage(band + 1, smem + ((band + 1) & 1) * q.tile_bytes);
            PHASE_MARK(3);
            const int u0 = band * GH / p.nbands, u1 = (band + 1) * GH / p.nbands;
            const int npos = (u1 - u0) * GW;
            const int ntiles = (npos + 31) / 32;
            for (int tile = wave; tile < ntiles; tile += NW) {
                const int qi = tile * 32 + (lane & 31);
                const int qc = min(qi, npos - 1);
                const int ul = fdiv(qc, p.mGW), v = qc - ul * GW;
                f32x16 acc;
#pragma unroll
                for (int r = 0; r < 16; r++) acc[r] = 0.f;
#pragma unroll
                for (int a = 0; a < 2; a++)
#pragma unroll
                    for (int bb = 0; bb < 2; bb++) {
                        const int yy = ul + 1 - a, xx = v + 1 - bb;
                        const int pbase = (yy * TC + xx) * PS;
                        const int s = swz_eval<CPP>(p.swz, xx, yy);
#pragma unroll
                        for (int kc = 0; kc < KC; kc++) {
                            const half8 av = *reinterpret_cast<const half8 *>(cur + pbase + (((kc * 2 + kh) ^ s) * 16));
                            acc = __builtin_amdgcn_mfma_f32_32x32x16_f16(wf[(a * 2 + bb) * KC + kc], av, acc, 0, 0, 0);
                        }
                    }
                if (qi < npos && kh == 0) {
                    const int u = u0 + ul;
                    f32x4 pl = {0.f, 0.f, 0.f, 0.f};
                    if constexpr (PART) pl = reinterpret_cast<const f32x4 *>(smem + q.part_off)[u * GW + v];
#pragma unroll
                    for (int r = 0; r < 4; r++) {
                        const int Y = 2 * u + (r >> 1) - p.cy, X = 2 * v + (r & 1) - p.cx;
                        if (Y >= 0 && Y < p.Hd && X >= 0 && X < p.Wd) {
                            float l = acc[r] + fbias;
                            if constexpr (PART) l += pl[r];
                            if (p.logits) p.logits[((size_t)b * p.Hd + Y) * p.Wd + X] = l;
                            bool fg = l > sp.thr;
                            if constexpr (POST) fg = fg && sp.keep[Y * p.Wd + X];
                            mfull[Y * p.Wd + X] = fg ? 1 : 0;
                        }
                    }
                }
            }
        }
        PHASE_MARK(4);
        lds_barrier();
        PHASE_MARK(5);
        if (p.mask) {
            uint8_t *dst = p.mask + (size_t)b * p.Hd * p.Wd;
            const int nbytes = p.Hd * p.Wd;
            if ((nbytes & 3) == 0 && (reinterpret_cast<uintptr_t>(p.mask) & 3) == 0) {
                for (int i = tid; i < nbytes / 4; i += NW * 64)
                    reinterpret_cast<uint32_t *>(dst)[i] = reinterpret_cast<const uint32_t *>(mfull)[i];
            } else {
                for (int i = tid; i < nbytes; i += NW * 64) dst[i] = mfull[i];
            }
        }
        PHASE_MARK(6);
        const int area = stack_area<POST, MS>(qp, q.ms.model_ids, b, q.area_thresh);
        if constexpr (WV)
            ccwave::frame_wg<ccbody::CC_THREADS>(mfull, smem + q.cc_off, q.wg, area, q.boxes + (size_t)b * q.max_boxes,
                                                 q.counts + b, q.max_boxes, tid);
        else
            ccbody::bboxcc_frame(mfull, smem + q.cc_off, q.g, area, q.boxes + (size_t)b * q.max_boxes, q.counts + b,
                                 q.max_boxes, tid);
        PHASE_MARK(7);
    }
#ifdef PHASE_TIMING
    if (tid == 0)
        for (int i = 0; i < 9; i++) atomicAdd(&g_phase[64 + i], ph_[i]);
#endif
    WGSPAN_END(4);
}

template <bool MS = false, bool POST = false>
__global__ __launch_bounds__(ccbody::CC_THREADS) void dec3cc_rows_mfma(Dec3ccArgs q, PostArg<POST> qp) {
    constexpr int NW = ccbody::CC_THREADS / 64, PS = 32;
    extern __shared__ __attribute__((aligned(16))) uint8_t smem[];
    const DecArgs &p = q.d;
    const int tid = threadIdx.x, lane = tid & 63, wave = tid >> 6;
    const int TC = p.Wi + 2, GW = p.Wi + 1, GH = p.Hi + 1;
    const int kh = lane >> 5, pos = lane & 31;
    const float fbias0 = p.epi[0];
    uint32_t *const planes = reinterpret_cast<uint32_t *>(smem + q.mfull_off);
    const f32x4 *const part = reinterpret_cast<const f32x4 *>(smem + q.part_off);
    WGSPAN_BEGIN();
#ifdef PHASE_TIMING
    unsigned long long ph_[9] = {0, 0, 0, 0, 0, 0, 0, 0, 0}, last_ = __builtin_amdgcn_s_memrealtime();
#endif
    uint32_t lc[2][2];
#pragma unroll
    for (int h = 0; h < 2; h++)
#pragma unroll
        for (int bb = 0; bb < 2; bb++) {
            const int xx = min(32 * h + pos, GW - 1) + 1 - bb;
            lc[h][bb] = (uint32_t)(xx * PS + ((kh ^ ((xx >> 3) & 1)) << 4));
        }
    const int row_b = TC * PS;
    for (int b = blockIdx.x; b < p.B; b += gridDim.x) {
        const uint32_t moff = model_off<MS>(q.ms.model_ids, q.ms.mstride, b);
        const float fbias = MS ? at_model(p.epi, moff)[0] : fbias0;
        const StackPost sp = stack_post<POST, MS>(qp, q.ms.model_ids, b);
        half8 wf[4];
#pragma unroll
        for (int ks = 0; ks < 4; ks++) wf[ks] = (MS ? at_model(p.wfrag, moff) : p.wfrag)[ks * 64 + lane];
        if (b != (int)blockIdx.x) lds_barrier();
        PHASE_MARK(0);
        {
            const uint8_t *ps = reinterpret_cast<const uint8_t *>(p.part) + (size_t)b * GH * GW * 16;
            const int nch = GH * GW;
            for (int s0 = wave * 64; s0 < nch; s0 += NW * 64)
                if (s0 + lane < nch) glds16(ps + (size_t)(s0 + lane) * 16, smem + q.part_off + s0 * 16);
        }
        {
            const __half *su = p.up + (size_t)b * p.Hi * p.Wi * 16;
            const int NI = 2 * p.Wi;
            for (int y = wave; y < p.Hi; y += NW) {
                const __half *rowp = su + (size_t)y * p.Wi * 16;
                uint8_t *rowl = smem + ((y + 1) * TC + 1) * PS;
                for (int q0 = 0; q0 < NI; q0 += 64) {
                    const int qq = q0 + lane, px = qq >> 1;
                    const int cb = ((qq & 1) ^ (((px + 1) >> 3) & 1)) * 8;
                    if (qq < NI) glds16(rowp + px * 16 + cb, rowl + q0 * 16);
                }
            }
            const int n_rows = 4 * TC, n_cols = 4 * p.Hi;
            for (int i = tid; i < n_rows + n_cols; i += NW * 64) {
                int piece;
                if (i < n_rows) {
                    piece = i < 2 * TC ? i : (p.Hi + 1) * 2 * TC + (i - 2 * TC);
                } else {
                    const int j = i - n_rows, y = j >> 2, k = j & 3;
                    piece = (y + 1) * 2 * TC + (k < 2 ? k : (p.Wi + 1) * 2 + (k - 2));
                }
                *reinterpret_cast<uint4 *>(smem + piece * 16) = uint4{0, 0, 0, 0};
            }
            for (int i = tid; i < q.wg.rows_bytes / 4; i += NW * 64) planes[i] = 0;
        }
        PHASE_MARK(1);
        wait_vmem();
        lds_barrier();
        PHASE_MARK(2);
        for (int t = wave; t < 2 * GH; t += NW) {
            const int u = t >> 1, h = t & 1;
            if (32 * h >= GW) continue;
            const uint32_t rb = (uint32_t)(u * row_b);
            const uint32_t a00 = rb + row_b + (h ? lc[1][0] : lc[0][0]), a01 = rb + row_b + (h ? lc[1][1] : lc[0][1]);
            const uint32_t a10 = rb + (h ? lc[1][0] : lc[0][0]), a11 = rb + (h ? lc[1][1] : lc[0][1]);
            f32x16 acc;
#pragma unroll
            for (int r = 0; r < 16; r++) acc[r] = 0.f;
            acc = __builtin_amdgcn_mfma_f32_32x32x16_f16(wf[0], *reinterpret_cast<const half8 *>(smem + a00), acc, 0, 0, 0);
            acc = __builtin_amdgcn_mfma_f32_32x32x16_f16(wf[1], *reinterpret_cast<const half8 *>(smem + a01), acc, 0, 0, 0);
            acc = __builtin_amdgcn_mfma_f32_32x32x16_f16(wf[2], *reinterpret_cast<const half8 *>(smem + a10), acc, 0, 0, 0);
            acc = __builtin_amdgcn_mfma_f32_32x32x16_f16(wf[3], *reinterpret_cast<const half8 *>(smem + a11), acc, 0, 0, 0);
            const int v = 32 * h + pos;
            const bool live = kh == 0 && v < GW;
            const f32x4 pl = part[u * GW + min(v, GW - 1)];
            float l[4];
#pragma unroll
            for (int r = 0; r < 4; r++) l[r] = (acc[r] + fbias) + pl[r];
            if (p.logits && live) {
#pragma unroll
                for (int r = 0; r < 4; r++) {
                    const int Y = 2 * u + (r >> 1) - p.cy, X = 2 * v + (r & 1) - p.cx;
                    if (Y >= 0 && Y < p.Hd && X >= 0 && X < p.Wd) p.logits[((size_t)b * p.Hd + Y) * p.Wd + X] = l[r];
                }
            }
#pragma unroll
            for (int r = 0; r < 4; r++) {
                const uint64_t bits = (uint64_t)(uint32_t)__ballot(live && l[r] > sp.thr) << (32 * h);
                const int Y = 2 * u + (r >> 1) - p.cy, X0 = (r & 1) - p.cx;
                const int pln = X0 & 1, sh = X0 >> 1;
                const int nb = (p.Wd - pln + 1) >> 1;
                uint64_t w = sh >= 0 ? bits << sh : bits >> (-sh);
                w &= nb >= 64 ? ~0ull : ((1ull << nb) - 1);
                if (Y >= 0 && Y < p.Hd && lane == 0) {
                    uint32_t *rw = planes + (Y + 1) * 4 + 2 * pln;
                    if ((uint32_t)w) atomicOr(rw, (uint32_t)w);
                    if ((uint32_t)(w >> 32)) atomicOr(rw + 1, (uint32_t)(w >> 32));
                }
            }
        }
        PHASE_MARK(4);
        lds_barrier();
        if constexpr (POST) {
            for (int i = tid; i < 4 * p.Hd; i += NW * 64) planes[4 + i] &= sp.planes[i];
            lds_barrier();
        }
        PHASE_MARK(5);
        if (p.mask) {
            uint32_t *dst = reinterpret_cast<uint32_t *>(p.mask + (size_t)b * p.Hd * p.Wd);
            const int wq = p.Wd >> 2, nq = p.Hd * wq;
            for (int i = tid; i < nq; i += NW * 64) {
                const int y = fdiv(i, p.mRC), xq = i - y * wq;
                const int bx = 2 * xq;
                const uint32_t *rw = planes + (y + 1) * 4 + (bx >> 5);
                const uint32_t e2 = (rw[0] >> (bx & 31)) & 3u, o2 = (rw[2] >> (bx & 31)) & 3u;
                dst[i] = (e2 & 1u) | ((o2 & 1u) << 8) | ((e2 >> 1) << 16) | ((o2 >> 1) << 24);
            }
        }
        PHASE_MARK(6);
        ccwave::frame_wg<ccbody::CC_THREADS, true>(nullptr, smem + q.cc_off, q.wg, stack_area<POST, MS>(qp, q.ms.model_ids, b, q.area_thresh), q.boxes + (size_t)b * q.max_boxes,
                                                   q.counts + b, q.max_boxes, tid, planes);
        PHASE_MARK(7);
    }
#ifdef PHASE_TIMING
    if (tid == 0)
        for (int i = 0; i < 9; i++) atomicAdd(&g_phase[64 + i], ph_[i]);
#endif
    WGSPAN_END(4);
}

void enc_epilogue(int cout, bool allpos, const float *bias, const float *gamma, const float *beta, const float *mean,
                  const float *var, std::vector<float> &wscale, float *epi) {
    wscale.assign(cout, 1.f);
    for (int c = 0; c < cout; c++) {
        const float sc = gamma[c] / std::sqrt(var[c] + BN_EPS), sh = beta[c] - mean[c] * sc;
        wscale[c] = sc;
        const float bp = bias[c] * sc;
        epi[cout + c] = bp + sh;
        if (allpos) {
            epi[c] = -bp;
            epi[2 * cout + c] = 0.f;
        } else {
            epi[c] = sc >= 0.f ? -bp : -3.0e38f;
            epi[2 * cout + c] = sc >= 0.f ? 3.0e38f : -bp;
        }
    }
}

void prep_enc0(bool allpos, const float *k, const float *bias, const float *gamma, const float *beta, const float *mean,
               const float *var, const float *w1, const float *w2, _Float16 *wfrag, float *epi) {
    std::vector<float> ws;
    enc_epilogue(16, allpos, bias, gamma, beta, mean, var, ws, epi);
    for (int set = 0; set < 2; set++)
        for (int ks = 0; ks < 2; ks++)
            for (int l = 0; l < 64; l++)
                for (int j = 0; j < 8; j++) {
                    const int n = l & 15, g = l >> 4;
                    const int px = 2 * (g & 1) + (j >> 2), ch = j & 3;
                    const int kx = set == 0 ? px - 1 : px;
                    int ky = -1;
                    if (ks == 0) ky = g >> 1;
                    else if ((g >> 1) == 0) ky = 2;
                    float w = 0.f;
                    if (ky >= 0 && kx >= 0 && kx < 3 && ch < 3) w = k[((ky * 3 + kx) * 3 + ch) * 16 + n] * ws[n] / 6.0f;
                    wfrag[((set * 2 + ks) * 64 + l) * 8 + j] = f2h(w);
                }
    std::memcpy(epi + 48, w1, 16 * sizeof(float));
    std::memcpy(epi + 64, w2, 16 * sizeof(float));
}

void prep_enc(bool allpos, int cin, int cout, const float *k, const float *bias, const float *gamma, const float *beta,
              const float *mean, const float *var, const float *w1, const float *w2, _Float16 *wfrag, float *epi) {
    const int NT = cout / 32, KC = cin / 16, KSTEPS = 9 * KC;
    std::vector<float> ws;
    enc_epilogue(cout, allpos, bias, gamma, beta, mean, var, ws, epi);
    for (int nt = 0; nt < NT; nt++)
        for (int ks = 0; ks < KSTEPS; ks++)
            for (int l = 0; l < 64; l++)
                for (int j = 0; j < 8; j++) {
                    const int tap = ks / KC, kc = ks % KC;
                    const int c = kc * 16 + 8 * (l >> 5) + j, n = nt * 32 + (l & 31);
                    wfrag[(((size_t)nt * KSTEPS + ks) * 64 + l) * 8 + j] = f2h(k[((size_t)tap * cin + c) * cout + n] * ws[n]);
                }
    std::memcpy(epi + 3 * cout, w1, 16 * sizeof(float));
    std::memcpy(epi + 3 * cout + 16, w2, 16 * sizeof(float));
}

void prep_enc1w(bool allpos, const float *k, const float *bias, const float *gamma, const float *beta, const float *mean,
                const float *var, _Float16 *wfrag) {
    static const int pairs[5][2] = {{0, 1}, {3, 4}, {6, 7}, {2, 5}, {8, -1}};
    std::vector<float> ws, epi(3 * 32);
    enc_epilogue(32, allpos, bias, gamma, beta, mean, var, ws, epi.data());
    for (int nt = 0; nt < 2; nt++)
        for (int s = 0; s < 5; s++)
            for (int l = 0; l < 64; l++)
                for (int j = 0; j < 8; j++) {
                    const int kg = l >> 4, tap = pairs[s][kg >> 1], c = 8 * (kg & 1) + j, n = nt * 16 + (l & 15);
                    wfrag[(((size_t)nt * 5 + s) * 64 + l) * 8 + j] = f2h(tap < 0 ? 0.f : k[((size_t)tap * 16 + c) * 32 + n] * ws[n]);
                }
}

void prep_dec(int cin, int cout, const float *k, const float *bias, const float *gamma, const float *beta,
              const float *mean, const float *var, _Float16 *wfrag, float *epi) {
    const int NTT = 4 * cout / 32, KC = cin / 16, KSTEPS = 4 * KC;
    for (int nt = 0; nt < NTT; nt++)
        for (int ks = 0; ks < KSTEPS; ks++)
            for (int l = 0; l < 64; l++)
                for (int j = 0; j < 8; j++) {
                    const int tap = ks / KC, kc = ks % KC, a = tap >> 1, bb = tap & 1;
                    const int c = kc * 16 + 8 * (l >> 5) + j, n = nt * 32 + (l & 31);
                    const int phase = n / cout, co = n % cout, py = phase >> 1, px = phase & 1;
                    const int ky = py + 2 * a, kx = px + 2 * bb;
                    wfrag[(((size_t)nt * KSTEPS + ks) * 64 + l) * 8 + j] =
                        f2h(k[(((size_t)ky * 4 + kx) * cout + co) * cin + c]);
                }
    for (int c = 0; c < cout; c++) {
        const float sc = gamma[c] / std::sqrt(var[c] + BN_EPS);
        epi[c] = sc;
        epi[cout + c] = bias[c] * sc + (beta[c] - mean[c] * sc);
    }
}

float final_fold(int cin, int cout, const float *k, const float *fk, int n, int a, int bb, int c) {
    const int ky = (n >> 1) + 2 * a, kx = (n & 1) + 2 * bb;
    double sacc = 0.0;
    for (int o = 0; o < cout; o++) sacc += (double)fk[o] * k[(((size_t)ky * 4 + kx) * cout + o) * cin + c];
    return (float)sacc;
}
void prep_final(int cin, int cout, const float *k, const float *bias, const float *fk, const float *fb,
                _Float16 *wfrag, float *epi, int c0 = 0, int cwin = 0) {
    if (!cwin) cwin = cin;
    const int KC = cwin / 16, KSTEPS = 4 * KC;
    for (int ks = 0; ks < KSTEPS; ks++)
        for (int l = 0; l < 64; l++)
            for (int j = 0; j < 8; j++) {
                const int tap = ks / KC, kc = ks % KC, a = tap >> 1, bb = tap & 1;
                const int c = c0 + kc * 16 + 8 * (l >> 5) + j, n = l & 31;
                wfrag[((size_t)ks * 64 + l) * 8 + j] = f2h(n < 4 ? final_fold(cin, cout, k, fk, n, a, bb, c) : 0.f);
            }
    if (epi) {
        double bsum = fb[0];
        for (int o = 0; o < cout; o++) bsum += (double)fk[o] * bias[o];
        epi[0] = (float)bsum;
    }
}
void prep_tail(int cin, int cout, const float *k, const float *fk, int c0, _Float16 *wfrag) {
    for (int s = 0; s < 2; s++)
        for (int l = 0; l < 64; l++)
            for (int j = 0; j < 8; j++) {
                const int i = l & 15, kg = l >> 4, c = c0 + 8 * (kg & 1) + j;
                wfrag[((size_t)s * 64 + l) * 8 + j] = f2h(i < 4 ? final_fold(cin, cout, k, fk, i, 1 - s, 1 - (kg >> 1), c) : 0.f);
            }
}

inline int swz_host(const Swz &w, int cpp, int xx, int yy) {
    return ((((yy * w.L + xx) >> w.p) * w.a) + yy * w.b + (yy & 1) * w.c) & (cpp - 1);
}
inline long long lds_cycles(const int (&addr)[64]) {
    static const int grp[4][16] = {{0, 1, 2, 3, 12, 13, 14, 15, 20, 21, 22, 23, 24, 25, 26, 27},
                                   {4, 5, 6, 7, 8, 9, 10, 11, 16, 17, 18, 19, 28, 29, 30, 31},
                                   {32, 33, 34, 35, 44, 45, 46, 47, 52, 53, 54, 55, 56, 57, 58, 59},
                                   {36, 37, 38, 39, 40, 41, 42, 43, 48, 49, 50, 51, 60, 61, 62, 63}};
    long long tot = 0;
    for (int g = 0; g < 4; g++) {
        int cnt[16] = {0}, worst = 0;
        for (int k = 0; k < 16; k++) {
            const int a = addr[grp[g][k]];
            bool dup = false;
            for (int j = 0; j < k; j++) dup = dup || addr[grp[g][j]] == a;
            if (!dup) worst = std::max(worst, ++cnt[(a >> 4) & 15]);
        }
        tot += worst;
    }
    return tot;
}
long long model_enc(int cin, int W, int Wp, int rb, const Swz &w) {
    const int TC = W + 2, PS = cin * 2, KC = cin / 16, CPP = cin / 8, nwin = rb * Wp;
    long long tot = 0;
    for (int tile = 0; tile < (nwin + 7) / 8; tile++)
        for (int ky = 0; ky < 3; ky++)
            for (int kx = 0; kx < 3; kx++)
                for (int kc = 0; kc < KC; kc++) {
                    int addr[64];
                    for (int lane = 0; lane < 64; lane++) {
                        const int m = lane & 31, kh = lane >> 5;
                        const int win = std::min(tile * 8 + (m >> 2), nwin - 1);
                        const int wy = win / Wp, wx = win % Wp;
                        const int yy = 2 * wy + ((m >> 1) & 1) + ky, xx = 2 * wx + (m & 1) + kx;
                        addr[lane] = (yy * TC + xx) * PS + (((kc * 2 + kh) ^ swz_host(w, CPP, xx, yy)) * 16);
                    }
                    tot += lds_cycles(addr);
                }
    return tot;
}
long long model_enc_rows(int cin, int W, int Wp, const Swz &w) {
    const int TC = W + 2, PS = cin * 2, KC = cin / 16, CPP = cin / 8;
    long long tot = 0;
    for (int tc = 0; tc < (Wp + 7) / 8; tc++)
        for (int wy = 0; wy < 2; wy++)
            for (int ky = 0; ky < 3; ky++)
                for (int kx = 0; kx < 3; kx++)
                    for (int kc = 0; kc < KC; kc++) {
                        int addr[64];
                        for (int lane = 0; lane < 64; lane++) {
                            const int m = lane & 31, kh = lane >> 5;
                            const int yy = 2 * wy + ((m >> 1) & 1) + ky, xx = 2 * (8 * tc + (m >> 2)) + (m & 1) + kx;
                            addr[lane] = (yy * TC + xx) * PS + (((kc * 2 + kh) ^ swz_host(w, CPP, xx, yy)) * 16);
                        }
                        tot += lds_cycles(addr);
                    }
    return tot;
}
long long model_dec(int C, int Wi, int nu, const Swz &w) {
    const int TC = Wi + 2, PS = C * 2, KC = C / 16, CPP = C / 8, GW = Wi + 1, npos = nu * GW;
    long long tot = 0;
    for (int tile = 0; tile < (npos + 31) / 32; tile++)
        for (int a = 0; a < 2; a++)
            for (int b = 0; b < 2; b++)
                for (int kc = 0; kc < KC; kc++) {
                    int addr[64];
                    for (int lane = 0; lane < 64; lane++) {
                        const int q = std::min(tile * 32 + (lane & 31), npos - 1);
                        const int yy = q / GW + 1 - a, xx = q % GW + 1 - b;
                        addr[lane] = (yy * TC + xx) * PS + (((kc * 2 + (lane >> 5)) ^ swz_host(w, CPP, xx, yy)) * 16);
                    }
                    tot += lds_cycles(addr);
                }
    return tot;
}
std::mutex g_swz_mutex;
Swz choose_swz(bool enc, int C, int W, int Wp, int rows) {
    struct Key { bool enc; int C, W, Wp, rows; Swz s; };
    static std::vector<Key> cache;
    std::lock_guard<std::mutex> lock(g_swz_mutex);
    for (auto &k : cache)
        if (k.enc == enc && k.C == C && k.W == W && k.Wp == Wp && k.rows == rows) return k.s;
    const int cpp = C / 8, TC = W + 2;
    Swz best{0, 0, 0, 0, 0};
    long long best_cost = -1;
    const long long ideal = enc ? 4LL * ((rows * Wp + 7) / 8) * 9 * (C / 16) : 4LL * ((rows * (W + 1) + 31) / 32) * 4 * (C / 16);
    static const int mult[3] = {0, 1, 3};
    bool done = false;
    for (int L = 0; L <= TC && !done; L += TC)
        for (int p = 0; p < 3 && !done; p++)
            for (int ai = 0; ai < 3 && !done; ai++)
                for (int b = 0; b < cpp && !done; b++)
                    for (int c = 0; c < cpp && !done; c++) {
                        const Swz w{p, mult[ai] % cpp, b, c, L};
                        const long long cost = enc ? model_enc(C, W, Wp, rows, w) : model_dec(C, W, rows, w);
                        if (best_cost < 0 || cost < best_cost) { best_cost = cost; best = w; }
                        if (ideal && cost == ideal) done = true;
                    }
    cache.push_back(Key{enc, C, W, Wp, rows, best});
    return best;
}

Swz choose_swz_periodic(int C, int W, int Wp) {
    struct Key { int C, W, Wp; Swz s; };
    static std::vector<Key> cache;
    std::lock_guard<std::mutex> lock(g_swz_mutex);
    for (auto &k : cache)
        if (k.C == C && k.W == W && k.Wp == Wp) return k.s;
    const int cpp = C / 8;
    Swz best{0, 0, 0, 0, 0};
    long long best_cost = -1;
    for (int p = 0; p < 4; p++)
        for (int a = 0; a < cpp; a++) {
            if (((16 >> p) * a) % cpp) continue;
            for (int c = 0; c < cpp; c++) {
                const Swz w{p, a, 0, c, 0};
                const long long cost = model_enc_rows(C, W, Wp, w);
                if (best_cost < 0 || cost < best_cost) { best_cost = cost; best = w; }
            }
        }
    cache.push_back(Key{C, W, Wp, best});
    return best;
}

ItemPlan make_plan(int grid, int num_cu, int wgs_per_cu, int batch, int nbands, int Hp) {
    ItemPlan pl{};
    if (wgs_per_cu != 2 || grid != 2 * num_cu || (nbands & 1) || nbands > 16 || batch * nbands < grid) return pl;
    std::vector<int> order(nbands);
    for (int k = 0; k < nbands; k++) order[k] = k;
    auto rows = [&](int k) { return ((k + 1) * Hp) / nbands - (k * Hp) / nbands; };
    std::stable_sort(order.begin(), order.end(), [&](int x, int y) { return rows(x) > rows(y); });
    pl.paired = 1;
    pl.cnt[0] = pl.cnt[1] = nbands / 2;
    for (int k = 0; k < nbands / 2; k++) {
        pl.band[0] |= (unsigned long long)order[k] << (8 * k);
        pl.band[1] |= (unsigned long long)order[nbands / 2 + k] << (8 * k);
    }
    return pl;
}


constexpr size_t LDS_LIMIT = 160 * 1024 - 256;

template <typename F>
int with_bools(F &&f) {
    return f();
}
template <typename F, typename... Bs>
int with_bools(F &&f, bool b, Bs... bs) {
    return b ? with_bools([&](auto... rest) { return f(std::true_type{}, rest...); }, bs...)
             : with_bools([&](auto... rest) { return f(std::false_type{}, rest...); }, bs...);
}

template <typename Fit>
int plan_bands(int Hp, int batch, long long slots, Fit fits) {
    long long best = -1;
    int nbands = 0;
    for (int nb = 1; nb <= Hp; nb++) {
        const int rb = (Hp + nb - 1) / nb;
        if (!fits(rb)) continue;
        const long long rounds = ((long long)batch * nb + slots - 1) / slots;
        const long long cost = rounds * (rb + 1);
        if (best < 0 || cost < best) { best = cost; nbands = nb; }
    }
    return nbands;
}

}

int blobnet_prepare_mfma(covahip_ctx *ctx, covahip_blobnet *m, const float *const *ws, int n_models) {
    const BnEncOff *const he = BN_LAYOUT.enc;
    const BnDecOff *const hd = BN_LAYOUT.dec;

    Prepared *pr = new Prepared();
    size_t off = 0;
    for (int i = 0; i < BN_LEVELS; i++) {
        const int ci = m->enc_c[i], co = m->enc_c[i + 1];
        const size_t nfrag = (i == 0) ? 4 * 64 : (size_t)(co / 32) * (9 * ci / 16) * 64;
        pr->enc[i].wfrag = off; off = align256(off + nfrag * 16);
        pr->enc[i].epi = off; off = align256(off + (3 * co + 32) * sizeof(float));
    }
    for (int j = 0; j < BN_LEVELS - 1; j++) {
        const int ci = m->dec_ci[j], co = m->dec_co[j];
        const size_t nfrag = (size_t)(4 * co / 32) * (4 * ci / 16) * 64;
        pr->dec[j].wfrag = off; off = align256(off + nfrag * 16);
        pr->dec[j].epi = off; off = align256(off + 3 * co * sizeof(float));
    }
    pr->enc1w = off; off = align256(off + (size_t)2 * 5 * 64 * 16);
    pr->final_w = off; off = align256(off + (size_t)(4 * m->dec_ci[3] / 16) * 64 * 16);
    pr->final_epi = off; off = align256(off + 16 * sizeof(float));
    pr->final_w_up = off; off = align256(off + (size_t)4 * 64 * 16);
    pr->tail_w = off; off = align256(off + (size_t)2 * 64 * 16);
    pr->zero = off; off = align256(off + 256);
    pr->total = off;

    std::vector<uint8_t> host_all(off * (size_t)n_models, 0);
    for (int i = 0; i < BN_LEVELS; i++) pr->allpos[i] = true;
    for (int k = 0; k < n_models; k++)
        for (int i = 0; i < BN_LEVELS; i++)
            for (int c = 0; c < m->enc_c[i + 1]; c++) pr->allpos[i] = pr->allpos[i] && ws[k][he[i].gamma + c] >= 0.f;
    for (int k = 0; k < n_models; k++) {
        const float *const w = ws[k], *const fk = w + BN_LAYOUT.fk, *const fb = w + BN_LAYOUT.fb;
        uint8_t *const host = host_all.data() + (size_t)k * off;
        prep_enc0(pr->allpos[0], w + he[0].k, w + he[0].b, w + he[0].gamma, w + he[0].beta, w + he[0].mean, w + he[0].var, w + he[0].w1,
                  w + he[0].w2, (_Float16 *)(host + pr->enc[0].wfrag), (float *)(host + pr->enc[0].epi));
        for (int i = 1; i < BN_LEVELS; i++)
            prep_enc(pr->allpos[i], m->enc_c[i], m->enc_c[i + 1], w + he[i].k, w + he[i].b, w + he[i].gamma, w + he[i].beta, w + he[i].mean,
                     w + he[i].var, w + he[i].w1, w + he[i].w2, (_Float16 *)(host + pr->enc[i].wfrag),
                     (float *)(host + pr->enc[i].epi));
        if (m->enc_c[1] == 16 && m->enc_c[2] == 32)
            prep_enc1w(pr->allpos[1], w + he[1].k, w + he[1].b, w + he[1].gamma, w + he[1].beta, w + he[1].mean, w + he[1].var,
                       (_Float16 *)(host + pr->enc1w));
        for (int j = 0; j < BN_LEVELS - 1; j++)
            prep_dec(m->dec_ci[j], m->dec_co[j], w + hd[j].k, w + hd[j].b, w + hd[j].gamma, w + hd[j].beta, w + hd[j].mean, w + hd[j].var,
                     (_Float16 *)(host + pr->dec[j].wfrag), (float *)(host + pr->dec[j].epi));
        prep_final(m->dec_ci[3], m->dec_co[3], w + hd[3].k, w + hd[3].b, fk, fb, (_Float16 *)(host + pr->final_w),
                   (float *)(host + pr->final_epi));
        if (m->dec_ci[3] == 32) {
            prep_final(32, m->dec_co[3], w + hd[3].k, w + hd[3].b, fk, fb, (_Float16 *)(host + pr->final_w_up), nullptr, 0, 16);
            prep_tail(32, m->dec_co[3], w + hd[3].k, fk, 16, (_Float16 *)(host + pr->tail_w));
        }
    }
    m->prep = pr;
    COVAHIP_CHECK_HIP(ctx, hipMalloc(&m->d_prepared, host_all.size()));
    COVAHIP_CHECK_HIP(ctx, hipMemcpy(m->d_prepared, host_all.data(), host_all.size(), hipMemcpyHostToDevice));
    m->prepared_bytes = host_all.size();
    m->n_models = n_models;
    return COVAHIP_OK;
}

void blobnet_release_mfma(covahip_ctx *, covahip_blobnet *m) {
    if (m->d_prepared) hipFree(m->d_prepared);
    m->d_prepared = nullptr;
    delete m->prep;
    m->prep = nullptr;
}

namespace {

struct Fwd {
    covahip_ctx *ctx;
    const covahip_blobnet *m;
    const Prepared *pr;
    BnWorkspace &ws;
    const BnInput &inp;
    int batch;
    const uint8_t *prep;
    uint32_t mstride;
    bool ms;
    bool dry;
    bool by_frames;
    int num_cu;
    const uint8_t *d_frames;
    int n_frames;
    const int32_t *d_index;
    float *d_logits;
    uint8_t *d_mask;
    const BnCcTail *cc;
    bool part_written = false;
    bool post = false;
    DecPost pp{};
};

template <bool POST>
PostArg<POST> post_arg(const Fwd &f) {
    if constexpr (POST) return f.pp;
    else return DecNoPost{};
}

template <typename K, typename... A>
int launch(const Fwd &f, const char *name, K kernel, int grid, int block, size_t lds, const A &...args) {
    if (int rc = covahip_open_lds(f.ctx, kernel, lds, LDS_LIMIT)) return rc;
    ProfScope ps(f.ctx, name);
    if (!f.dry) hipLaunchKernelGGL(kernel, dim3(grid), dim3(block), lds, f.ctx->stream, args...);
    return COVAHIP_OK;
}
int launched(const Fwd &f, int rc) {
    if (rc) return rc;
    COVAHIP_CHECK_HIP(f.ctx, hipGetLastError());
    return COVAHIP_OK;
}

int run_enc0p(const Fwd &f) {
    const covahip_blobnet *m = f.m;
    const Prepared *pr = f.pr;
    const int H = m->lv[0].H, W = m->lv[0].W, Hp = H / 2, Wp = W / 2;
    const int TC = ((W + 4 - 16 + 31) / 32) * 32 + 16;
    if (W % 4) return COVAHIP_ERR_UNSUPPORTED;
    int nbands = 0;
    for (int nb = 1; nb <= Hp; nb++) {
        const int rb = (Hp + nb - 1) / nb, n2 = 2 * rb + 2;
        if (n2 * (W / 4) > 2 * WG0 || (size_t)n2 * TC * 8 > 30 * 1024) continue;
        if ((long long)f.n_frames * nb < 2LL * f.num_cu && nb < Hp) continue;
        nbands = nb;
        break;
    }
    if (!nbands) return COVAHIP_ERR_UNSUPPORTED;
    const int rbmax = (Hp + nbands - 1) / nbands;
    const size_t tile_bytes = (((size_t)(2 * rbmax + 2) * TC * 8) + 15) & ~(size_t)15;
    Enc0pArgs a;
    a.in = f.d_frames; a.out = f.ws.pbuf;
    a.wfrag = (const half8 *)(f.prep + pr->enc[0].wfrag); a.epi = (const float *)(f.prep + pr->enc[0].epi);
    a.F = f.n_frames; a.H = H; a.W = W; a.Hp = Hp; a.Wp = Wp; a.Ho = m->lv[1].H; a.Wo = m->lv[1].W;
    a.oy = H & 1; a.ox = W & 1; a.nbands = nbands; a.TC = TC;
    a.mWp = magic(Wp); a.mNb = magic(nbands); a.mW4 = magic(W / 4); a.scr_off = (int)tile_bytes;
    a.model_ids = f.inp.frame_models; a.mstride = f.mstride;
    const size_t lds = tile_bytes + (size_t)(WG0 / 64) * 1024;
    const int grid = std::min(f.n_frames * nbands, 3 * f.num_cu);
    return launched(f, with_bools([&](auto AP, auto PACKED, auto MS) {
        return launch(f, "enc0p_mfma", enc0p_mfma<AP.value, PACKED.value, MS.value>, grid, WG0, lds, a);
    }, pr->allpos[0], f.inp.packed, f.ms));
}

bool run_enc1_tile16(Fwd &f, int &rc) {
    const covahip_blobnet *m = f.m;
    const Prepared *pr = f.pr;
    if (!bn_level1_on_enc1(f.ctx, m)) return false;
    const int H = m->lv[1].H, W = m->lv[1].W, Hp = H / 2, Wp = W / 2;
    const int nbands = plan_bands(Hp, f.batch, 2LL * f.num_cu, [](int rb) { return 2 * rb + 2 <= E1_TR; });
    if (!nbands) return false;
    Enc1Args a;
    a.in = f.ws.pbuf; a.out = f.ws.act[2];
    a.wfrag = (const half8 *)(f.prep + pr->enc1w); a.epi = (const float *)(f.prep + pr->enc[1].epi);
    a.B = f.batch; a.H = H; a.W = W; a.Hp = Hp; a.Wp = Wp; a.Ho = m->lv[2].H; a.Wo = m->lv[2].W;
    a.oy = H & 1; a.ox = W & 1; a.nbands = nbands;
    a.mWp = magic(Wp); a.mRC = magic(2 * (W + 2));
    a.scr_off = BN_T * E1_TSZ;
    const int grid = std::min(f.batch * nbands, 2 * f.num_cu);
    a.plan = make_plan(grid, f.num_cu, 2, f.batch, nbands, Hp);
    a.pidx = f.d_index; a.skip = f.ws.act[1]; a.tm_pre = (const float *)(f.prep + pr->enc[0].epi) + 48;
    f.part_written = m->tail_part && f.ws.part && m->dec_ci[3] == 32 && m->dec_co[3] == 16 && m->enc_c[1] == 16;
    a.part = f.part_written ? f.ws.part : nullptr;
    a.wtail = (const half8 *)(f.prep + pr->tail_w);
    a.mXe = magic(2 * Wp);
    a.use_ktab = 0;
    if (f.by_frames && f.inp.h_index && f.batch <= BN_KTAB_STACKS) {
        a.use_ktab = 1;
        for (int k = 0; k < f.batch * BN_T; k++) a.ktab[k] = (uint16_t)f.inp.h_index[k];
    } else if (f.by_frames && !f.d_index && !f.dry) {
        rc = COVAHIP_ERR_INVALID_ARG;
        return true;
    }
    const size_t lds = (size_t)BN_T * E1_TSZ + 8 * 1024 + E1_CONST;
    a.model_ids = f.inp.model_ids; a.mstride = f.mstride;
    rc = launched(f, with_bools([&](auto AP, auto MS) {
        return launch(f, "enc1_mfma", enc1_mfma<AP.value, MS.value>, grid, 512, lds, a);
    }, pr->allpos[1], f.ms));
    return true;
}

bool run_enc23(const Fwd &f, int &rc) {
    const covahip_blobnet *m = f.m;
    const Prepared *pr = f.pr;
    if (!(m->fuse_enc23 && m->enc_rowtiles && !f.ctx->enc_plan[2].nbands && !f.ctx->enc_plan[3].nbands && m->enc_c[2] == 32 &&
          m->enc_c[3] == 64 && m->enc_c[4] == 128))
        return false;
    const int H = m->lv[2].H, W = m->lv[2].W, Hp = H / 2, Wp = W / 2;
    const int H3 = m->lv[3].H, W3 = m->lv[3].W, Hp3 = H3 / 2, Wp3 = W3 / 2;
    const size_t lds = (size_t)BN_T * E3_TSZ + (size_t)BN_T * E23_TSZ2 + 4096;
    const bool pays = 4 * f.batch >= 3 * f.num_cu && 20 * Wp >= 17 * 8 * ((Wp + 7) / 8) && 20 * Wp3 >= 17 * 8 * ((Wp3 + 7) / 8);
    if (!((pays || m->fuse_enc23 == 2 || f.ms) && (W + 2) * 64 <= E23_RP2 && Wp <= 16 && Hp >= 1 && Hp3 >= 1 && Wp3 >= 1 &&
          (size_t)std::max(2 * Hp3 + 2, H3 + 1) * (W3 + 2) * 128 <= (size_t)E3_TSZ && lds <= 160 * 1024 - 256))
        return false;
    Enc23Args a;
    a.in = f.ws.act[2]; a.mid = f.ws.act[3]; a.out = f.ws.act[4];
    a.wf2 = (const half8 *)(f.prep + pr->enc[2].wfrag); a.wf3 = (const half8 *)(f.prep + pr->enc[3].wfrag);
    a.epi2 = (const float *)(f.prep + pr->enc[2].epi); a.epi3 = (const float *)(f.prep + pr->enc[3].epi);
    a.B = f.batch;
    a.H2 = H; a.W2 = W; a.Hp2 = Hp; a.Wp2 = Wp;
    a.H3 = H3; a.W3 = W3; a.Hp3 = Hp3; a.Wp3 = Wp3; a.oy3 = H & 1; a.ox3 = W & 1;
    a.H4 = m->lv[4].H; a.W4 = m->lv[4].W; a.oy4 = H3 & 1; a.ox4 = W3 & 1;
    a.swz2 = choose_swz_periodic(32, 30, Wp); a.swz3 = choose_swz_periodic(64, W3, Wp3);
    a.ring_off = BN_T * E3_TSZ; a.xchg_off = a.ring_off + BN_T * E23_TSZ2; a.scr_off = a.ring_off;
    a.model_ids = f.inp.model_ids; a.mstride = f.mstride;
    const int grid = std::min(f.batch, f.num_cu);
    rc = launched(f, with_bools([&](auto AP2, auto AP3, auto MS) {
        return launch(f, "enc23_mfma", enc23_mfma<AP2.value, AP3.value, MS.value>, grid, 512, lds, a);
    }, pr->allpos[2], pr->allpos[3], f.ms));
    return true;
}

int run_enc_level(const Fwd &f, int i) {
    const covahip_blobnet *m = f.m;
    const Prepared *pr = f.pr;
    const int H = m->lv[i].H, W = m->lv[i].W, Hp = H / 2, Wp = W / 2;
    const int cin = m->enc_c[i];
    const size_t px_bytes = (size_t)cin * 2;
    const int TC = W + 2;
    static const int enc_waves[BN_LEVELS] = {0, 8, 4, 8};
    int nbuf = 1, wgs_per_cu = (i == BN_LEVELS - 1) ? 1 : 2;
    int nbands = 0;
    const size_t scr_bytes = (size_t)enc_waves[i] * 2048;
    if (f.ctx->enc_plan[i].nbands) {
        nbands = std::min(f.ctx->enc_plan[i].nbands, Hp);
        nbuf = f.ctx->enc_plan[i].nbuf;
        const size_t need = (size_t)nbuf * BN_T * (2 * ((Hp + nbands - 1) / nbands) + 2) * TC * px_bytes + scr_bytes;
        if (need > 160 * 1024 - 256) return COVAHIP_ERR_UNSUPPORTED;
        wgs_per_cu = (i == BN_LEVELS - 1) ? 1 : (int)std::min<size_t>(2, (160 * 1024 - 256) / need);
    } else {
        const size_t lds_cap = (wgs_per_cu == 1 ? 150 * 1024 : 80 * 1024) - scr_bytes;
        nbands = plan_bands(Hp, f.batch, (long long)wgs_per_cu * f.num_cu,
                            [&](int rb) { return (size_t)BN_T * (2 * rb + 2) * TC * px_bytes <= lds_cap; });
        if (!nbands) return COVAHIP_ERR_UNSUPPORTED;
    }
    const int RB = 2 * ((Hp + nbands - 1) / nbands);
    const int fix_tsz = i == 2 ? E2_TSZ : i == 3 ? E3_TSZ : 0;
    bool rowtiles = false;
    if (fix_tsz && m->enc_rowtiles && !f.ctx->enc_plan[i].nbands && cin == (i == 2 ? 32 : 64) && m->enc_c[i + 1] == 2 * cin &&
        (size_t)(RB + 2) * TC * px_bytes <= (size_t)fix_tsz) {
        long long t_rows = (long long)Hp * ((Wp + 7) / 8), t_gen = 0;
        for (int k = 0; k < nbands; k++) t_gen += ((((k + 1) * Hp) / nbands - (k * Hp) / nbands) * Wp + 7) / 8;
        rowtiles = t_rows <= t_gen;
    }
    const size_t tile_bytes = rowtiles ? (size_t)BN_T * fix_tsz : (((size_t)BN_T * (RB + 2) * TC * px_bytes) + 15) & ~(size_t)15;
    const size_t lds = nbuf * tile_bytes + scr_bytes;
    if (lds > 160 * 1024 - 256) return COVAHIP_ERR_UNSUPPORTED;
    const int items = f.batch * nbands;
    const int grid = std::min(items, wgs_per_cu * f.num_cu);
    EncArgs a;
    a.in = i == 1 ? f.ws.pbuf : f.ws.act[i]; a.out = f.ws.act[i + 1];
    a.wfrag = (const half8 *)(f.prep + pr->enc[i].wfrag); a.epi = (const float *)(f.prep + pr->enc[i].epi);
    a.B = f.batch; a.H = H; a.W = W; a.Hp = Hp; a.Wp = Wp; a.Ho = m->lv[i + 1].H; a.Wo = m->lv[i + 1].W;
    a.oy = H & 1; a.ox = W & 1; a.To = (i == BN_LEVELS - 1) ? 1 : BN_T;
    a.RB = RB; a.nbands = nbands; a.TR = RB + 2; a.TC = TC;
    a.mWp = magic(Wp); a.mNb = magic(nbands); a.mRC = magic(TC * (cin / 8)); a.zero = f.prep + pr->zero;
    a.nbuf = nbuf; a.buf_stride = (int)tile_bytes; a.scr_off = (int)(nbuf * tile_bytes);
    a.plan = make_plan(grid, f.num_cu, wgs_per_cu, f.batch, nbands, Hp);
    a.swz = rowtiles ? choose_swz_periodic(cin, W, Wp) : choose_swz(true, cin, W, Wp, RB / 2);
    a.pidx = f.d_index; a.skip = f.ws.act[1]; a.tm_pre = (const float *)(f.prep + pr->enc[0].epi) + 48;
    a.model_ids = f.inp.model_ids; a.mstride = f.mstride;
    const bool ap = pr->allpos[i];
    if (i == 1) {
        if (f.by_frames && !f.d_index && !f.dry) return COVAHIP_ERR_INVALID_ARG;
        return launched(f, with_bools([&](auto AP, auto MS) {
            return launch(f, "enc1_mfma", enc_mfma<16, 32, 2, 4, 8, true, AP.value, true, 0, MS.value>, grid, 512, lds, a);
        }, ap, f.ms));
    }
    if (i == 2)
        return launched(f, with_bools([&](auto AP, auto ROWS, auto MS) {
            return launch(f, "enc2_mfma", enc_mfma<32, 64, 4, 2, 4, true, AP.value, false, ROWS.value ? E2_TSZ : 0, MS.value>, grid, WG, lds, a);
        }, ap, rowtiles, f.ms));
    return launched(f, with_bools([&](auto AP, auto ROWS, auto MS) {
        return launch(f, "enc3_mfma", enc_mfma<64, 128, 2, 2, 8, true, AP.value, false, ROWS.value ? E3_TSZ : 0, MS.value>, grid, 512, lds, a);
    }, ap, rowtiles, f.ms));
}

bool run_dec012(const Fwd &f, int &rc) {
    const covahip_blobnet *m = f.m;
    const Prepared *pr = f.pr;
    if (!(m->fuse_dec && m->dec_ci[0] == 128 && m->dec_ci[1] == 128 && m->dec_ci[2] == 64 && m->dec_co[0] == 64 &&
          m->dec_co[1] == 32 && m->dec_co[2] == 16))
        return false;
    Dec012Args a;
    size_t off = 0;
    for (int j = 0; j < 3; j++) {
        const BnLevelGeom in = m->lv[BN_LEVELS - j], out = m->lv[BN_LEVELS - 1 - j];
        DecLvl &g = a.lv[j];
        g.Hi = in.H; g.Wi = in.W; g.Hd = out.H; g.Wd = out.W; g.cy = m->dec_cy[j]; g.cx = m->dec_cx[j];
        g.mGW = magic(in.W + 1);
        g.mRC = magic((in.W + 2) * (m->dec_ci[j] / 8));
        g.swz = choose_swz(false, m->dec_ci[j], in.W, 0, in.H + 1);
        g.tile_off = (int)off;
        off += align256((size_t)(in.H + 2) * (in.W + 2) * m->dec_ci[j] * 2);
        a.skip[j] = f.ws.act[BN_LEVELS - j];
        a.Ts[j] = j == 0 ? 1 : BN_T;
        a.wf[j] = (const half8 *)(f.prep + pr->dec[j].wfrag);
        a.epi[j] = (const float *)(f.prep + pr->dec[j].epi);
    }
    a.scr_off = (int)off;
    const size_t lds = off + 8 * 2048;
    if (lds > 160 * 1024 - 256) return false;
    a.out = f.ws.dact[2]; a.B = f.batch; a.zero = f.prep + pr->zero;
    a.model_ids = f.inp.model_ids; a.mstride = f.mstride;
    rc = launched(f, with_bools([&](auto MS) {
        return launch(f, "dec012_mfma", dec012_mfma<MS.value>, std::min(f.batch, f.num_cu), 512, lds, a);
    }, f.ms));
    return true;
}

struct DecPlan {
    DecArgs a;
    DecMs am;
    BnLevelGeom in, out;
    bool half;
    int ci, GH, grid;
    size_t row_bytes, lds;
};
int plan_dec_block(const Fwd &f, int j, DecPlan &p) {
    const covahip_blobnet *m = f.m;
    const Prepared *pr = f.pr;
    const BnLevelGeom in = m->lv[BN_LEVELS - j], out = m->lv[BN_LEVELS - 1 - j];
    const bool last = j == BN_LEVELS - 1;
    const bool half = last && f.part_written;
    const int ci_j = half ? m->dec_ci[j] / 2 : m->dec_ci[j];
    DecArgs &a = p.a;
    a.up = j == 0 ? nullptr : f.ws.dact[j - 1];
    a.skip = f.ws.act[BN_LEVELS - j];
    a.out = last ? nullptr : f.ws.dact[j];
    a.logits = last ? f.d_logits : nullptr;
    a.mask = last ? f.d_mask : nullptr;
    a.wfrag = (const half8 *)(f.prep + (half ? pr->final_w_up : last ? pr->final_w : pr->dec[j].wfrag));
    a.part = half ? f.ws.part : nullptr;
    a.epi = (const float *)(f.prep + (last ? pr->final_epi : pr->dec[j].epi));
    a.B = f.batch; a.Hi = in.H; a.Wi = in.W; a.Hd = out.H; a.Wd = out.W; a.cy = m->dec_cy[j]; a.cx = m->dec_cx[j];
    a.Ts = j == 0 ? 1 : BN_T;
    p.am = DecMs{f.inp.model_ids, f.mstride};
    const int GH = in.H + 1;
    const size_t row_bytes = (size_t)(in.W + 2) * ci_j * 2;
    const size_t wbytes = (size_t)(last ? 1 : 4 * m->dec_co[j] / 32) * (4 * ci_j / 16) * 1024;
    const bool heavy = wbytes >= 192 * 1024 && (size_t)(GH + 1) * row_bytes <= 72 * 1024;
    int nbands = 1;
    if (!heavy)
        while (nbands < GH && (((size_t)((GH + nbands - 1) / nbands) + 1) * row_bytes > 30 * 1024 ||
                               (long long)f.batch * nbands < 2LL * f.num_cu))
            nbands++;
    a.nbands = nbands; a.mNb = magic(nbands); a.mGW = magic(in.W + 1);
    a.mRC = magic((in.W + 2) * (ci_j / 8)); a.zero = f.prep + pr->zero;
    a.swz = choose_swz(false, ci_j, in.W, 0, (GH + nbands - 1) / nbands);
    const size_t tile_bytes = (((size_t)((GH + nbands - 1) / nbands) + 1) * row_bytes + 15) & ~(size_t)15;
    const size_t mask_bytes = last ? ((((size_t)2 * ((GH + nbands - 1) / nbands) * out.W) + 15) & ~(size_t)15) : 0;
    const size_t scr_bytes = last ? 0 : (size_t)std::max(4, 4 * m->dec_co[j] / 32) * 2048;
    p.lds = tile_bytes + mask_bytes + scr_bytes;
    a.mask_off = (int)tile_bytes;
    a.scr_off = (int)tile_bytes;
    if (p.lds > 160 * 1024 - 256) return COVAHIP_ERR_UNSUPPORTED;
    p.in = in; p.out = out; p.half = half; p.ci = ci_j; p.GH = GH; p.row_bytes = row_bytes;
    p.grid = std::min(f.batch * nbands, (heavy ? 1 : 4) * f.num_cu);
    return COVAHIP_OK;
}
int launch_dec_block(const Fwd &f, int j, const DecPlan &p) {
    if (j == 0)
        return launched(f, with_bools([&](auto MS) {
            return launch(f, "dec0_mfma", dec_mfma<0, 128, 64, false, MS.value>, p.grid, 512, p.lds, p.a, p.am, DecNoPost{});
        }, f.ms));
    if (j == 1)
        return launched(f, with_bools([&](auto MS) {
            return launch(f, "dec1_mfma", dec_mfma<64, 64, 32, false, MS.value>, p.grid, 256, p.lds, p.a, p.am, DecNoPost{});
        }, f.ms));
    if (j == 2)
        return launched(f, with_bools([&](auto MS) {
            return launch(f, "dec2_mfma", dec_mfma<32, 32, 16, false, MS.value>, p.grid, 256, p.lds, p.a, p.am, DecNoPost{});
        }, f.ms));
    return launched(f, with_bools([&](auto HALF, auto MS, auto POST) {
        return launch(f, "dec3_final_mfma", dec_mfma<16, HALF.value ? 0 : 16, 16, true, MS.value, POST.value>, p.grid, 256, p.lds, p.a,
                      p.am, post_arg<POST.value>(f));
    }, p.half, f.ms, f.post));
}
int run_dec_block(const Fwd &f, int j) {
    DecPlan p;
    if (int rc = plan_dec_block(f, j, p)) return rc;
    return launch_dec_block(f, j, p);
}

bool run_tail_fused(const Fwd &f, const DecPlan &p) {
    const BnLevelGeom in = p.in, out = p.out;
    const int GH = p.GH;
    Dec3ccArgs t;
    size_t cc_bytes = ccbody::cc_plan(out.H, out.W, t.g);
    t.use_wv = f.ctx->cc_wave_cap >= 0 && ccwave::wv_plan(out.H, out.W, ((out.H + 1) / 2) * ((out.W + 1) / 2), t.wg) ? 1 : 0;
    if (t.use_wv) cc_bytes = (size_t)t.wg.wave_bytes;
    if (!cc_bytes) return false;
    const size_t mfull = ((size_t)out.H * out.W + 15) & ~(size_t)15;
    const size_t partb = p.half ? (size_t)GH * (in.W + 1) * 16 : 0;
    int best_nb = 0;
    long long best_cost = -1;
    for (int nb = 1; nb <= GH; nb++) {
        const size_t tb = (((size_t)((GH + nb - 1) / nb) + 1) * p.row_bytes + 15) & ~(size_t)15;
        const size_t nbuf = nb == 1 ? 1 : 2;
        if (std::max(nbuf * tb, cc_bytes) + mfull + partb > 160 * 1024 - 512) continue;
        long long rounds = 0;
        for (int k = 0; k < nb; k++) {
            const int nu = (k + 1) * GH / nb - k * GH / nb;
            rounds += ((nu * (in.W + 1) + 31) / 32 + 15) / 16;
        }
        const long long cost = rounds * 8 + nb;
        if (best_cost < 0 || cost < best_cost) { best_cost = cost; best_nb = nb; }
    }
    if (!best_nb) return false;
    const size_t tb = (((size_t)((GH + best_nb - 1) / best_nb) + 1) * p.row_bytes + 15) & ~(size_t)15;
    t.d = p.a;
    t.ms = p.am;
    t.d.nbands = best_nb; t.d.mNb = magic(best_nb);
    t.d.swz = choose_swz(false, p.ci, in.W, 0, (GH + best_nb - 1) / best_nb);
    t.boxes = f.cc->boxes; t.counts = f.cc->counts;
    t.area_thresh = f.cc->area_thresh; t.max_boxes = f.cc->max_boxes;
    t.tile_bytes = (int)tb; t.cc_off = 0;
    t.mfull_off = (int)std::max((best_nb == 1 ? 1 : 2) * tb, cc_bytes);
    t.part_off = (int)((size_t)t.mfull_off + mfull);
    const size_t tl = (size_t)t.part_off + partb;
    const int grid = std::min(f.batch, 2 * f.num_cu);
    if (p.half && t.use_wv && best_nb == 1 && in.W + 1 <= 64 && f.m->tail_rows && (out.W & 7) == 0 &&
        (size_t)t.wg.rows_bytes <= mfull && (!f.d_mask || (reinterpret_cast<uintptr_t>(f.d_mask) & 3) == 0)) {
        t.d.swz = Swz{3, 1, 0, 0, 0};
        t.d.mRC = magic(out.W / 4);
        if (!f.dry) f.ctx->tail_form = COVAHIP_DEV_TAIL_ROWS;
        return !with_bools([&](auto MS, auto POST) {
            return launch(f, "dec3_bboxcc_fused", dec3cc_rows_mfma<MS.value, POST.value>, grid, ccbody::CC_THREADS, tl, t, post_arg<POST.value>(f));
        }, f.ms, f.post);
    }
    if (!f.dry) f.ctx->tail_form = COVAHIP_DEV_TAIL_BANDS + (t.use_wv ? 2 : 0) + (p.half ? 1 : 0);
    return !with_bools([&](auto WV, auto PART, auto MS, auto POST) {
        return launch(f, "dec3_bboxcc_fused", dec3cc_mfma<WV.value, PART.value, MS.value, POST.value>, grid, ccbody::CC_THREADS, tl, t, post_arg<POST.value>(f));
    }, t.use_wv != 0, p.half, f.ms, f.post);
}

}

int blobnet_forward_mfma(covahip_ctx *ctx, covahip_blobnet *m, BnWorkspace &ws, const BnInput &inp, int batch, float *d_logits,
                         uint8_t *d_mask, const BnCcTail *cc, bool *cc_done) {
    if (cc_done) *cc_done = false;
    const Prepared *pr = m->prep;
    const bool dry = inp.dry;
    const bool by_frames = inp.frames != nullptr || (dry && inp.n_frames > 0);
    const bool ms = inp.model_ids != nullptr || (dry && inp.mixed);
    Fwd f{ctx, m, pr, ws, inp, batch,
          (const uint8_t *)m->d_prepared + (ms ? 0 : (size_t)inp.model * pr->total), (uint32_t)pr->total,
          ms, dry, by_frames, ctx->props.multiProcessorCount,
          by_frames ? inp.frames : inp.stack, by_frames ? inp.n_frames : batch * BN_T, by_frames ? inp.index : nullptr,
          d_logits, d_mask, cc};
    if ((size_t)f.n_frames > ws.pbuf_frames && !dry) return COVAHIP_ERR_INVALID_ARG;
    f.post = m->post_on;
    if (f.post) {
        if (!m->d_post) return COVAHIP_ERR_INVALID_ARG;
        const uint8_t *const dp = (const uint8_t *)m->d_post;
        const size_t k = ms ? 0 : (size_t)inp.model;
        f.pp.thr = m->post_thr[k];
        f.pp.thr_tab = (const float *)dp;
        f.pp.area = m->post_area[k] >= 1 ? m->post_area[k] : (cc ? cc->area_thresh : 0);
        f.pp.area_tab = (const int32_t *)(dp + m->post_area_off);
        f.pp.keep = dp + m->post_keep_off + k * m->post_keep_stride;
        f.pp.planes = (const uint32_t *)(dp + m->post_planes_off + k * m->post_planes_stride);
        f.pp.keep_stride = (uint32_t)m->post_keep_stride;
        f.pp.planes_stride = (uint32_t)m->post_planes_stride;
    }

    int rc = run_enc0p(f);
    if (rc) return rc;
    if (!run_enc1_tile16(f, rc)) rc = run_enc_level(f, 1);
    if (rc) return rc;
    if (!run_enc23(f, rc)) {
        rc = run_enc_level(f, 2);
        if (!rc) rc = run_enc_level(f, 3);
    }
    if (rc) return rc;
    if (!run_dec012(f, rc))
        for (int j = 0; j < BN_LEVELS - 1 && !rc; j++) rc = run_dec_block(f, j);
    if (rc) return rc;
    DecPlan last;
    rc = plan_dec_block(f, BN_LEVELS - 1, last);
    if (rc) return rc;
    if (!(cc && m->fuse_tail && run_tail_fused(f, last))) {
        if (!dry) ctx->tail_form = COVAHIP_DEV_TAIL_ALONE;
        return launch_dec_block(f, BN_LEVELS - 1, last);
    }
    if (cc_done) *cc_done = true;
    return launched(f, COVAHIP_OK);
}

#if defined(PHASE_TIMING) || defined(WGSPAN_ONLY)
extern "C" int covahip_dev_wgspan_read(unsigned long long *out, int kid) {
    return hipMemcpyFromSymbol(out, HIP_SYMBOL(g_wgspan), sizeof(unsigned long long) * 1024 * 4, sizeof(unsigned long long) * 1024 * 4 * kid) != hipSuccess;
}
#endif
#ifdef WGSPAN_ONLY
extern "C" int covahip_dev_itemspan_read(unsigned long long *out, int kid) {
    return hipMemcpyFromSymbol(out, HIP_SYMBOL(g_itemspan), sizeof(unsigned long long) * 1024 * 16, sizeof(unsigned long long) * 1024 * 16 * kid) != hipSuccess;
}
#endif
#ifdef PHASE_TIMING
extern "C" int covahip_dev_ccphase_read(unsigned long long *out8, int reset) {
    if (hipMemcpyFromSymbol(out8, HIP_SYMBOL(g_ccph), sizeof(g_ccph)) != hipSuccess) return 1;
    if (reset) {
        unsigned long long z[8] = {0};
        if (hipMemcpyToSymbol(HIP_SYMBOL(g_ccph), z, sizeof(z)) != hipSuccess) return 1;
    }
    return 0;
}
extern "C" int covahip_dev_phase_read(unsigned long long *out64, int reset) {
    if (hipMemcpyFromSymbol(out64, HIP_SYMBOL(g_phase), sizeof(g_phase)) != hipSuccess) return 1;
    if (reset) {
        unsigned long long z[80] = {0};
        if (hipMemcpyToSymbol(HIP_SYMBOL(g_phase), z, sizeof(z)) != hipSuccess) return 1;
    }
    return 0;
}
#endif
```

cova_amd/csrc/internal.h:

```cpp
#pragma once
#include <hip/hip_runtime.h>

#include <algorithm>
#include <cmath>
#include <cstdint>
#include <map>
#include <string>
#include <vector>

#include "covahip.h"

struct covahip_blobnet;
struct covahip_ctx;

constexpr size_t align256(size_t x) { return (x + 255) & ~(size_t)255; }

inline bool covahip_thresholds_ok(const float *v, int n) {
    for (int t = 0; t < n; t++)
        if (!std::isfinite(v[t]) || (t && !(v[t] > v[t - 1]))) return false;
    return true;
}

template <typename T>
struct ResidentTable {
    T *dev = nullptr;
    T *pinned = nullptr;
    size_t cap = 0;
    hipEvent_t ev = nullptr;
    bool recorded = false;
    std::vector<T> resident;

    int reserve(covahip_ctx *ctx, size_t n);
    int upload(covahip_ctx *ctx, const T *src, size_t n, const T **d_out);
    void invalidate() { resident.clear(); }
    void release();
};

constexpr int COVAHIP_MAX_LANES = 4;
struct CtxLane {
    hipStream_t stream = nullptr;
    hipEvent_t done = nullptr;
    bool pending = false;
    uint64_t seen_seq = 0;
    void *cc_scratch = nullptr;
    size_t cc_scratch_bytes = 0;
    void *cc_ovf = nullptr;
    size_t cc_ovf_bytes = 0;
    void *cc_slab = nullptr;
    size_t cc_slab_bytes = 0;
    int32_t *cc_stat = nullptr;
    int32_t *cc_stat_ring = nullptr;
    unsigned cc_stat_turn = 0;
    bool cc_second_skipped = false;
    int cc_stat_batch = 0, cc_stat_cap = 0;
    int cc_first_cap = 0;
};

using MonTable = ResidentTable<int32_t>;
struct CovahipMonitor {
    int h = 0, w = 0, n_models = 0, max_boxes = 0, every = 1;
    bool attached = false;
    unsigned long long *d_tab = nullptr;
    size_t words = 0;
    int64_t batches_seen = 0, batches_counted = 0;
    MonTable lane[COVAHIP_MAX_LANES];
};

struct covahip_ctx {
    int device = 0;
    hipStream_t primary = nullptr;
    hipStream_t stream = nullptr;
    CtxLane lanes[COVAHIP_MAX_LANES];
    int n_lanes = 1, next_lane = 0, cur_lane = 0;
    bool in_lane = false;
    uint64_t primary_seq = 1;
    hipEvent_t ev_fork = nullptr;
    std::string last_hip_error;
    hipDeviceProp_t props{};
    hipEvent_t t_start[16]{};
    hipEvent_t t_stop[16]{};
    bool profile = false;
    std::string profile_filter;
    struct ProfEntry {
        std::string name;
        hipEvent_t a, b;
    };
    std::vector<ProfEntry> prof_pending;
    std::vector<std::pair<hipEvent_t, hipEvent_t>> prof_pool;
    std::map<std::string, std::pair<double, int64_t>> prof_acc;
    void *stage_in = nullptr;
    size_t stage_in_bytes = 0;
    void *stage_out = nullptr;
    size_t stage_out_bytes = 0;
    void *pinned = nullptr;
    size_t pinned_bytes = 0;
    void *sweep_buf = nullptr;
    size_t sweep_bytes = 0;
    ResidentTable<int32_t> cc_area;
    int cc_wave_cap = 0;
    int tail_form = 0;
    CtxLane &lane() { return lanes[cur_lane]; }
    struct { int nbands, nbuf; } enc_plan[4] = {};
    covahip_blobnet *blobnet = nullptr;
    void *heat_buf = nullptr;
    size_t heat_bytes = 0;
    bool heat_open = false;
    int heat_h = 0, heat_w = 0, heat_T = 0;
    float heat_thresh[64] = {};
    int64_t heat_samples = 0;
    size_t heat_stage = 0;
    CovahipMonitor *mon = nullptr;
    int mon_slice = 0;
    bool mon_suspended = false;
};

#define COVAHIP_CHECK_HIP(ctx, expr)                                                        \
    do {                                                                                    \
        hipError_t _e = (expr);                                                             \
        if (_e != hipSuccess) {                                                             \
            (ctx)->last_hip_error = std::string(#expr) + ": " + hipGetErrorString(_e);      \
            return COVAHIP_ERR_HIP;                                                         \
        }                                                                                   \
    } while (0)

template <typename T>
int ResidentTable<T>::reserve(covahip_ctx *ctx, size_t n) {
    if (n <= cap) return COVAHIP_OK;
    if (dev || pinned) {
        COVAHIP_CHECK_HIP(ctx, hipStreamSynchronize(ctx->stream));
        hipFree(dev);
        hipHostFree(pinned);
        dev = pinned = nullptr;
        cap = 0;
        resident.clear();
    }
    if (!ev) COVAHIP_CHECK_HIP(ctx, hipEventCreateWithFlags(&ev, hipEventDisableTiming));
    COVAHIP_CHECK_HIP(ctx, hipMalloc((void **)&dev, n * sizeof(T)));
    COVAHIP_CHECK_HIP(ctx, hipHostMalloc((void **)&pinned, n * sizeof(T), hipHostMallocDefault));
    cap = n;
    return COVAHIP_OK;
}

template <typename T>
int ResidentTable<T>::upload(covahip_ctx *ctx, const T *src, size_t n, const T **d_out) {
    *d_out = dev;
    if (n > cap) return COVAHIP_ERR_INVALID_ARG;
    if (n && resident.size() == n && std::equal(src, src + n, resident.begin())) return COVAHIP_OK;
    if (recorded) COVAHIP_CHECK_HIP(ctx, hipEventSynchronize(ev));
    std::copy(src, src + n, pinned);
    COVAHIP_CHECK_HIP(ctx, hipMemcpyAsync(dev, pinned, n * sizeof(T), hipMemcpyHostToDevice, ctx->stream));
    resident.clear();
    COVAHIP_CHECK_HIP(ctx, hipEventRecord(ev, ctx->stream));
    recorded = true;
    resident.assign(src, src + n);
    return COVAHIP_OK;
}

template <typename T>
void ResidentTable<T>::release() {
    if (dev) hipFree(dev);
    if (pinned) hipHostFree(pinned);
    if (ev) hipEventDestroy(ev);
    *this = ResidentTable<T>();
}

int covahip_open_lds(covahip_ctx *ctx, const void *fn, size_t lds, size_t limit);
template <typename K>
int covahip_open_lds(covahip_ctx *ctx, K kernel, size_t lds, size_t limit) {
    return lds <= 64 * 1024 ? COVAHIP_OK : covahip_open_lds(ctx, reinterpret_cast<const void *>(kernel), lds, limit);
}

struct ProfScope {
    covahip_ctx *ctx;
    int idx = -1;
    ProfScope(covahip_ctx *c, const char *name);
    ~ProfScope();
};

int covahip_ensure_buffer(covahip_ctx *ctx, void **buf, size_t *cur, size_t need);

struct LaneScope {
    covahip_ctx *ctx;
    bool owner = false, failed = false;
    explicit LaneScope(covahip_ctx *c);
    ~LaneScope();
    bool ok() const { return !failed; }
};
int covahip_primary_op(covahip_ctx *ctx);
int covahip_sync_all(covahip_ctx *ctx);

uint32_t covahip_crc32c(const uint8_t *p, size_t n);

int covahip_bboxcc_launch(covahip_ctx *ctx, const uint8_t *d_mask, int batch, int h, int w, int area_thresh,
                          covahip_box *d_boxes, int32_t *d_counts, int max_boxes, const int32_t *d_area = nullptr);

int covahip_monitor_hook(covahip_ctx *ctx, const uint8_t *d_mask, const int32_t *d_counts, const covahip_box *d_boxes, int max_boxes,
                         const uint8_t *model_ids, int batch);
void covahip_monitor_close(covahip_ctx *ctx, bool attached_only);

int covahip_train_data_check(const covahip_train_data *d, const covahip_ctx *ctx, int h, int w, const covahip_train_sample *s,
                             int64_t n);
int covahip_train_data_table(covahip_train_data *d, int n, covahip_train_sample **tab);
int covahip_train_data_launch(covahip_train_data *d, int n, uint8_t *d_stack, uint8_t *d_gt);

int covahip_label_mass_launch(covahip_ctx *ctx, const uint8_t *d_gt, const uint32_t *d_bits, uint32_t *d_mass, int64_t first,
                              int64_t n, int hw);

void covahip_blobnet_destroy(covahip_ctx *ctx);
int covahip_blobnet_forward_dev(covahip_ctx *ctx, const uint8_t *d_stack, int batch, float *d_logits,
                                uint8_t *d_mask, const uint8_t *model_ids = nullptr);
int covahip_blobnet_geometry(covahip_ctx *ctx, int *h, int *w);
int covahip_blobnet_grow_lanes(covahip_ctx *ctx, int n_lanes);
```

cova_amd/elements.py:

```python
from __future__ import annotations

import ctypes as C

import numpy as np

from . import _lib as L
from . import weights as W

FLOW_OK = "ok"
FLOW_DROPPED = "dropped"


def _ptr(a: np.ndarray) -> int:
    return a.ctypes.data


def _optr(a: np.ndarray | None) -> int | None:
    return None if a is None else a.ctypes.data


class Context:

    def __init__(self, device_id: int = 0):
        self._lib = L.lib()
# ... 52 lines not shown
        L.check(self._lib.covahip_timer_start(self.handle, slot), "timer_start", self.handle)

    def timer_stop(self, slot=0):
        L.check(self._lib.covahip_timer_stop(self.handle, slot), "timer_stop", self.handle)

    def timer_ms(self, slot=0) -> float:
        ms = C.c_float()
        L.check(self._lib.covahip_timer_elapsed_ms(self.handle, slot, C.byref(ms)), "timer_elapsed", self.handle)
        return ms.value

    def profile(self, on: bool, only: str | None = None):
        L.check(self._lib.covahip_profile_filter(self.handle, only.encode() if only else None), "profile_filter")
        L.check(self._lib.covahip_profile_enable(self.handle, int(on)), "profile_enable")
        L.check(self._lib.covahip_profile_reset(self.handle), "profile_reset")

    def profile_read(self):
        buf = np.zeros(64, dtype=L.KERNEL_TIME_DTYPE)
        n = C.c_int()
        L.check(self._lib.covahip_profile_read(self.handle, _ptr(buf), 64, C.byref(n)), "profile_read")
        return {r["name"].decode(): (float(r["total_ms"]), int(r["launches"])) for r in buf[:n.value]}


class MetaPreprocess:

    def __init__(self, timestep: int = 1, gamma: int = 1):
        self.timestep = timestep
        self.gamma = gamma
        self._h = None
        self._lib = L.lib()

    def transform_caps(self, width: int, height: int):
        ow, oh = C.c_int(), C.c_int()
        self._lib.covahip_stack_out_dims(width, height, self.timestep, C.byref(ow), C.byref(oh))
        return ow.value, oh.value

    def set_caps(self, width: int, height: int):
        ow, oh = self.transform_caps(width, height)
        out_size = ow * oh * 4
        self.size_per_buf = out_size // self.timestep
        self.out_size = out_size
        self.stop()
        h = C.c_void_p()
        L.check(self._lib.covahip_stack_new(self.size_per_buf, self.timestep, self.gamma, C.byref(h)), "stack_new")
        self._h = h
        return ow, oh

    def transform(self, inbuf: bytes | np.ndarray):
        a = np.frombuffer(inbuf, dtype=np.uint8) if not isinstance(inbuf, np.ndarray) else inbuf.reshape(-1)
        a = np.ascontiguousarray(a, dtype=np.uint8)
        out = np.empty(self.out_size, dtype=np.uint8)
        em = C.c_int()
        L.check(self._lib.covahip_stack_push(self._h, _ptr(a), a.size, _ptr(out), out.size, C.byref(em)), "stack_push")
        return (FLOW_OK, out) if em.value else (FLOW_DROPPED, None)

    def stop(self):
        if self._h:
            self._lib.covahip_stack_free(self._h)
            self._h = None

    __del__ = stop


def keep_from_rects(h_mb: int, w_mb: int, ignore=(), unit: int = 16) -> np.ndarray:
    keep = np.ones((h_mb, w_mb), dtype=np.uint8)
    for left, top, width, height in ignore:
        if width <= 0 or height <= 0:
            continue
        x0, y0 = max(0, int(left) // unit), max(0, int(top) // unit)
        x1 = min(w_mb, (int(left) + int(width) + unit - 1) // unit)
        y1 = min(h_mb, (int(top) + int(height) + unit - 1) // unit)
        if x0 < x1 and y0 < y1:
            keep[y0:y1, x0:x1] = 0
    return keep


class BlobNetInfer:

    def __init__(self, ctx: Context, weights_flat, h_mb: int, w_mb: int, max_batch: int,
                 timestep: int = 4):
        self.ctx, self.h, self.w, self.t, self.max_batch = ctx, h_mb, w_mb, timestep, max_batch
        self._lib = L.lib()
        if isinstance(weights_flat, (list, tuple)):
            blobs = [W.to_bytes(w) for w in weights_flat]
            ptrs = (C.c_char_p * max(1, len(blobs)))(*blobs)
            sizes = (C.c_size_t * max(1, len(blobs)))(*[len(b) for b in blobs])
            L.check(self._lib.covahip_blobnet_load_set(ctx.handle, len(blobs), ptrs, sizes, h_mb, w_mb, timestep, max_batch),
                    "covahip_blobnet_load_set", ctx.handle)
        else:
            blob = W.to_bytes(weights_flat)
            L.check(self._lib.covahip_blobnet_load(ctx.handle, blob, len(blob), h_mb, w_mb, timestep, max_batch),
                    "covahip_blobnet_load", ctx.handle)

    @property
    def num_models(self) -> int:
        v = C.c_int()
        L.check(self._lib.covahip_blobnet_num_models(self.ctx.handle, C.byref(v)), "covahip_blobnet_num_models")
        return v.value

    @staticmethod
    def post_logit_thresh(prob_thresh=None, logit_thresh=None) -> float:
        if prob_thresh is not None and logit_thresh is not None:
            raise ValueError("prob_thresh and logit_thresh are mutually exclusive")
        if prob_thresh is not None:
            p = float(prob_thresh)
            if not 0.0 < p < 1.0:
                raise ValueError(f"prob_thresh must lie in (0, 1), got {prob_thresh!r}")
            return float(np.float32(np.log(np.float64(p) / (1.0 - np.float64(p)))))
        return float(np.float32(0.0 if logit_thresh is None else logit_thresh))

    def set_post(self, model: int = 0, *, prob_thresh=None, logit_thresh=None, keep=None):
        thr = BlobNetInfer.post_logit_thresh(prob_thresh, logit_thresh)
        post = L.BlobNetPost(thr, None)
        if keep is not None:
            keep = np.ascontiguousarray(np.asarray(keep) != 0, dtype=np.uint8)
            if keep.shape != (self.h, self.w):
                raise ValueError(f"keep must be [{self.h}][{self.w}], got {keep.shape}")
            post.keep = _ptr(keep)
        L.check(self._lib.covahip_blobnet_set_post(self.ctx.handle, model, C.byref(post)), "covahip_blobnet_set_post", self.ctx.handle)

    def reset_post(self, model: int = 0):
        L.check(self._lib.covahip_blobnet_set_post(self.ctx.handle, model, None), "covahip_blobnet_set_post", self.ctx.handle)

    def post(self, model: int = 0):
        thr, has = C.c_float(), C.c_int()
        keep = np.empty((self.h, self.w), dtype=np.uint8)
        L.check(self._lib.covahip_blobnet_get_post(self.ctx.handle, model, C.byref(thr), _ptr(keep), C.byref(has)),
                "covahip_blobnet_get_post", self.ctx.handle)
        return thr.value, (keep if has.value else None)

    def set_area(self, model: int = 0, area: int = 0):
        L.check(self._lib.covahip_blobnet_set_area(self.ctx.handle, model, int(area)), "covahip_blobnet_set_area", self.ctx.handle)

    def get_area(self, model: int = 0) -> int:
        v = C.c_int()
        L.check(self._lib.covahip_blobnet_get_area(self.ctx.handle, model, C.byref(v)), "covahip_blobnet_get_area", self.ctx.handle)
        return v.value

    def monitor_begin(self, every: int = 1):
        from . import monitor
        monitor.begin(self.ctx, self.h, self.w, self.num_models, 0, attach=True, every=every)

    def monitor_read(self, reset: bool = False) -> dict:
        from . import monitor
        return monitor.read(self.ctx, reset)

    def monitor_end(self):
        from . import monitor
        monitor.end(self.ctx)

    def set_enc_plan(self, level: int, nbands: int, nbuf: int = 1):
        L.check(self._lib.covahip_blobnet_set_enc_plan(self.ctx.handle, level, nbands, nbuf), "covahip_blobnet_set_enc_plan")

    def set_impl(self, impl: str):
        L.check(self._lib.covahip_blobnet_set_impl(self.ctx.handle, {"mfma": 1, "dec_separate": 4, "enc1_legacy": 5, "enc_general_tiles": 6, "enc23_separate": 7, "enc23_force": 8, "tail_skip_tensor": 9, "tail_band_tiles": 10}[impl]), "set_impl")

    TAIL_ALONE, TAIL_ROWS, TAIL_BANDS = 1, 2, 4

    def tail_form(self) -> int:
        v = C.c_int()
        L.check(self._lib.covahip_dev_blobnet_tail_form(self.ctx.handle, C.byref(v)), "covahip_dev_blobnet_tail_form")
        return v.value

    def read_buffer(self, which: int, index: int = 0) -> np.ndarray:
        p, n, dims = C.c_void_p(), C.c_size_t(), (C.c_int32 * 5)()
        L.check(self._lib.covahip_dev_blobnet_buffer(self.ctx.handle, which, index, C.byref(p), C.byref(n), dims),
                "covahip_dev_blobnet_buffer", self.ctx.handle)
        out = np.empty(tuple(d for d in dims if d), dtype=np.float32 if which == 3 else np.float16)
        assert p.value and out.nbytes == n.value, (which, index, n.value, tuple(dims))
        self.ctx.d2h(out, p.value)
        return out

    @property
    def macs_per_frame(self) -> int:
        v = C.c_int64()
        L.check(self._lib.covahip_blobnet_macs_per_frame(self.ctx.handle, C.byref(v)), "macs_per_frame")
        return v.value

    def infer(self, stack: np.ndarray, want_logits: bool = True, model_ids=None):
        stack = np.ascontiguousarray(stack, dtype=np.uint8)
        b = stack.shape[0]
        assert stack.shape == (b, self.t * self.h, self.w, 4), stack.shape
        logits = np.empty((b, self.h, self.w), dtype=np.float32) if want_logits else None
        mask = np.empty((b, self.h, self.w), dtype=np.uint8)
        ids = _ids(model_ids, b)
        L.check(self._lib.covahip_blobnet_forward_m(self.ctx.handle, _ptr(stack), _optr(ids), b, _ptr(logits) if want_logits else None,
                                                    _ptr(mask), L.MEM_HOST), "covahip_blobnet_forward_m", self.ctx.handle)
        return logits, mask

    def infer_device(self, d_stack: int, batch: int, d_logits: int | None, d_mask: int | None, model_ids=None):
        ids = _ids(model_ids, batch)
        L.check(self._lib.covahip_blobnet_forward_m(self.ctx.handle, d_stack, _optr(ids), batch, d_logits, d_mask, L.MEM_DEVICE),
                "covahip_blobnet_forward_m", self.ctx.handle)

    def filter(self, stack: np.ndarray, cc_threshold: int, max_boxes: int = 256, want_mask: bool = False, model_ids=None):
        return self.filter_full(stack, cc_threshold, max_boxes, want_mask, False, model_ids)[:3]

    def filter_full(self, stack: np.ndarray, cc_threshold: int, max_boxes: int = 256, want_mask: bool = False,
                    want_logits: bool = False, model_ids=None):
        stack = np.ascontiguousarray(stack, dtype=np.uint8)
        b = stack.shape[0]
        boxes = np.zeros((b, max_boxes), dtype=L.BOX_DTYPE)
        counts = np.zeros(b, dtype=np.int32)
        mask = np.empty((b, self.h, self.w), dtype=np.uint8) if want_mask else None
        logits = np.empty((b, self.h, self.w), dtype=np.float32) if want_logits else None
        ids = _ids(model_ids, b)
        L.check(self._lib.covahip_filter_forward_m(self.ctx.handle, _ptr(stack), _optr(ids), b, cc_threshold, _ptr(boxes), _ptr(counts),
                                                   max_boxes, _ptr(logits) if want_logits else None, _ptr(mask) if want_mask else None,
                                                   L.MEM_HOST),
                "covahip_filter_forward_m", self.ctx.handle)
        return boxes, counts, mask, logits

    def filter_frames(self, frames: np.ndarray, stack_index: np.ndarray | None, cc_threshold: int, max_boxes: int = 256,
                      want_mask: bool = False, want_logits: bool = False, model_ids=None):
        frames = np.ascontiguousarray(frames, dtype=np.uint8)
        f = frames.shape[0]
        assert frames.shape == (f, self.h, self.w, 4), frames.shape
        idx = None if stack_index is None else np.ascontiguousarray(stack_index, dtype=np.int32).reshape(-1, 4)
        b = f - 3 if idx is None else idx.shape[0]
        boxes = np.zeros((b, max_boxes), dtype=L.BOX_DTYPE)
        counts = np.zeros(b, dtype=np.int32)
        mask = np.empty((b, self.h, self.w), dtype=np.uint8) if want_mask else None
        logits = np.empty((b, self.h, self.w), dtype=np.float32) if want_logits else None
        ids = _ids(model_ids, b)
        L.check(self._lib.covahip_filter_forward_frames_m(self.ctx.handle, _ptr(frames), f, None if idx is None else _ptr(idx),
                                                          _optr(ids), b, cc_threshold, _ptr(boxes), _ptr(counts), max_boxes,
                                                          _ptr(logits) if want_logits else None,
                                                          _ptr(mask) if want_mask else None, L.MEM_HOST),
                "covahip_filter_forward_frames_m", self.ctx.handle)
        return boxes, counts, mask, logits

    def filter_frames_device(self, d_frames: int, n_frames: int, stack_index: np.ndarray | None, batch: int, cc_threshold: int,
                             d_boxes: int, d_counts: int, max_boxes: int, d_mask: int | None = None, model_ids=None,
                             d_logits: int | None = None, packed: bool = False):
        idx = None if stack_index is None else np.ascontiguousarray(stack_index, dtype=np.int32).reshape(-1, 4)
        ids = _ids(model_ids, batch)
        if packed:
            L.check(self._lib.covahip_filter_forward_frames_packed_m(self.ctx.handle, d_frames, n_frames, None if idx is None else _ptr(idx),
                                                                     _optr(ids), batch, cc_threshold, d_boxes, d_counts, max_boxes,
                                                                     d_logits, d_mask),
                    "covahip_filter_forward_frames_packed_m", self.ctx.handle)
            return
        L.check(self._lib.covahip_filter_forward_frames_m(self.ctx.handle, d_frames, n_frames, None if idx is None else _ptr(idx),
                                                          _optr(ids), batch, cc_threshold, d_boxes, d_counts, max_boxes, d_logits,
                                                          d_mask, L.MEM_DEVICE),
                "covahip_filter_forward_frames_m", self.ctx.handle)

    def filter_device(self, d_stack: int, batch: int, cc_threshold: int, d_boxes: int, d_counts: int, max_boxes: int,
                      d_mask: int | None = None, model_ids=None, d_logits: int | None = None):
        ids = _ids(model_ids, batch)
        L.check(self._lib.covahip_filter_forward_m(self.ctx.handle, d_stack, _optr(ids), batch, cc_threshold, d_boxes, d_counts,
                                                   max_boxes, d_logits, d_mask, L.MEM_DEVICE),
                "covahip_filter_forward_m", self.ctx.handle)


def _ids(model_ids, batch: int):
    if model_ids is None:
        return None
    ids = np.ascontiguousarray(model_ids, dtype=np.uint8).reshape(-1)
    assert ids.shape == (batch,), (ids.shape, batch)
    return ids


def pack_frames(frames: np.ndarray) -> np.ndarray:
    frames = np.ascontiguousarray(frames, dtype=np.uint8)
    out = np.empty(frames.shape[:-1], dtype=np.uint16)
    L.lib().covahip_carrier_pack(frames.ctypes.data_as(C.c_void_p), frames.size // 4, out.ctypes.data_as(C.c_void_p))
    return out


class FilterPipe:

    def __init__(self, net: "BlobNetInfer", max_batch: int, max_frames: int, max_boxes: int = 256, n_slots: int = 3,
                 want_mask: bool = False, packed: bool = False, blocking_wait: bool = False):
        self.net, self.max_batch, self.max_frames, self.max_boxes = net, max_batch, max_frames, max_boxes
        self.packed = packed
        self._lib = L.lib()
        h = C.c_void_p()
        L.check(self._lib.covahip_pipe_create(net.ctx.handle, max_batch, max_frames, max_boxes, n_slots, int(want_mask),
                                              C.byref(h)), "covahip_pipe_create", net.ctx.handle)
        self._h = h
        if packed:
            L.check(self._lib.covahip_pipe_set_packed(h, 1), "covahip_pipe_set_packed")
        if blocking_wait:
            L.check(self._lib.covahip_pipe_set_blocking_wait(h, 1), "covahip_pipe_set_blocking_wait", net.ctx.handle)
        self._batch = {}
        self._views = {}
        self._mviews = {}
        self._rviews = {}
        self._held = []

    def close(self):
        if getattr(self, "_h", None):
            if getattr(self.net.ctx, "handle", None):
                self._lib.covahip_pipe_destroy(self._h)
            self._h = None

    __del__ = close

    def queue_plan(self):
        a, b = C.c_int(-1), C.c_int(-1)
        L.check(self._lib.covahip_dev_pipe_queue_plan(self._h, C.byref(a), C.byref(b)), "covahip_dev_pipe_queue_plan")
        return a.value, b.value

    def acquire(self):
        for held in self._held:
            L.check(self._lib.covahip_pipe_release(self._h, held), "covahip_pipe_release")
        self._held = []
        slot, fp, ip = C.c_int(), C.c_void_p(), C.c_void_p()
        rc = self._lib.covahip_pipe_acquire(self._h, C.byref(slot), C.byref(fp), C.byref(ip))
        if rc == 7:
            return None
        L.check(rc, "covahip_pipe_acquire")
        if slot.value not in self._views:
            n = self.max_frames * self.net.h * self.net.w * 4
# ... 390 lines not shown
```

include/covahip_dev.h:

```cpp
#ifndef COVAHIP_DEV_H
#define COVAHIP_DEV_H

#include "covahip.h"

#ifdef __cplusplus
extern "C" {
#endif

int covahip_blobnet_set_impl(covahip_ctx *ctx, int impl);

int covahip_bboxcc_set_wave_cap(covahip_ctx *ctx, int cap);
int covahip_dev_bboxcc_overflow(covahip_ctx *ctx, int32_t *out4);

int covahip_blobnet_set_enc_plan(covahip_ctx *ctx, int level, int nbands, int nbuf);

int covahip_dev_blobnet_buffer(covahip_ctx *ctx, int which, int index, void **dptr, size_t *bytes, int32_t dims[5]);

int covahip_dev_clock_mhz(covahip_ctx *ctx, int busy_us, float *mhz);

int covahip_dev_graph_probe(covahip_ctx *ctx, const uint8_t *d_frames, int n_frames, const int32_t *stack_index, int batch,
                            int area_thresh, covahip_box *d_boxes, int32_t *d_counts, int max_boxes, uint8_t *d_mask, int iters,
                            float *ms_direct, float *ms_graph);

#define COVAHIP_DEV_TAIL_ALONE 1
#define COVAHIP_DEV_TAIL_ROWS 2
#define COVAHIP_DEV_TAIL_BANDS 4
int covahip_dev_blobnet_tail_form(covahip_ctx *ctx, int *form);

struct covahip_pipe;
int covahip_dev_pipe_queue_plan(struct covahip_pipe *pipe, int *lanes_on_upload_queue, int *lanes_on_result_queue);

struct covahip_mog;
int covahip_dev_mog_masks(struct covahip_mog *m, uint8_t *raw, uint8_t *filled, size_t cap, int *n_frames);
int covahip_dev_mog_state(struct covahip_mog *m, int stream, float *W, float *V, float *M, uint8_t *nmodes, int64_t *n);
int covahip_dev_mog_set_stage_budget(struct covahip_mog *m, size_t bytes);
int covahip_dev_mog_post_masks(struct covahip_mog *m, const uint8_t *raw, int n_frames, uint8_t *labels);
int covahip_dev_mog_set_post_form(struct covahip_mog *m, int banded, int band_rows);
int covahip_dev_mog_band_plan(int work_w, int work_h, int *rows, int *bands, size_t *lds_bytes);

int covahip_dev_monitor_slice(covahip_ctx *ctx, int samples);

int covahip_dev_heat_set_stage(covahip_ctx *ctx, size_t bytes);
struct covahip_train_data;
int covahip_dev_train_data_set_stage(struct covahip_train_data *data, size_t bytes);

#ifdef __cplusplus
}
#endif
#endif
```

Measured before the change: 2.424 million.

## Fuse final decoder tail into dec012 kernel and emit bit planes for bboxcc

Adds a variant of the dec012 decoder kernel that writes its last-level output straight into an LDS tile. It then runs the final 1-channel conv tail with MFMA rows, applies the threshold, and builds per-frame bit planes in LDS, which are copied to a new global planes buffer and optionally expanded to a mask. A separate cc_planes kernel then does connected components from those planes. This removes the dact[2] round trip through global memory and the separate dec3 tail kernel's staging. In exchange the dec012 kernel holds more LDS and registers, and the path is gated by an auto heuristic on batch size versus CU count, no logits, and single-model inputs.

Result: faster. 2.486 million, median of 6 (+2.6%).

```diff
diff --git a/cova_amd/_lib.py b/cova_amd/_lib.py
--- a/cova_amd/_lib.py
+++ b/cova_amd/_lib.py
@@ -290,6 +290,7 @@
                                           C.POINTER(C.c_float)]),
     "covahip_dev_bboxcc_overflow": (C.c_int, [_P, C.POINTER(C.c_int32)]),
     "covahip_dev_blobnet_tail_form": (C.c_int, [_P, C.POINTER(C.c_int)]),
+    "covahip_dev_blobnet_tail_in_dec012": (C.c_int, [_P, C.POINTER(C.c_int)]),
     "covahip_dev_pipe_queue_plan": (C.c_int, [_P, C.POINTER(C.c_int), C.POINTER(C.c_int)]),
     "covahip_dev_blobnet_buffer": (C.c_int, [_P, C.c_int, C.c_int, C.POINTER(C.c_void_p), C.POINTER(C.c_size_t), C.POINTER(C.c_int32)]),
     "covahip_dev_mog_masks": (C.c_int, [_P, _P, _P, _SZ, C.POINTER(C.c_int)]),
diff --git a/cova_amd/csrc/blobnet.h b/cova_amd/csrc/blobnet.h
--- a/cova_amd/csrc/blobnet.h
+++ b/cova_amd/csrc/blobnet.h
@@ -19,6 +19,7 @@
     __half *pbuf = nullptr;
     size_t pbuf_frames = 0;
     float *part = nullptr;
+    uint32_t *planes = nullptr;
     ResidentTable<int32_t> index;
     int index_frames = 0;
     std::vector<int32_t> kept_table;
@@ -40,6 +41,7 @@
     int fuse_dec = 1;
     int enc1_tile16 = 1;
     int tail_rows = 1;
+    int tail_in_dec012 = 1;
     int tail_part = 1;
     int fuse_enc23 = 1;
     int enc_rowtiles = 1;
diff --git a/cova_amd/csrc/blobnet.hip b/cova_amd/csrc/blobnet.hip
--- a/cova_amd/csrc/blobnet.hip
+++ b/cova_amd/csrc/blobnet.hip
@@ -18,6 +18,7 @@
             if (ws.dact[j]) hipFree(ws.dact[j]);
         if (ws.pbuf) hipFree(ws.pbuf);
         if (ws.part) hipFree(ws.part);
+        if (ws.planes) hipFree(ws.planes);
         ws.index.release();
         ws.models.release();
         ws.areas.release();
@@ -185,6 +186,7 @@
         COVAHIP_CHECK_HIP(ctx, hipMalloc((void **)&ws.dact[j], n * sizeof(__half)));
     }
     COVAHIP_CHECK_HIP(ctx, hipMalloc((void **)&ws.part, (size_t)m->max_batch * (m->lv[1].H + 1) * (m->lv[1].W + 1) * 4 * sizeof(float)));
+    COVAHIP_CHECK_HIP(ctx, hipMalloc((void **)&ws.planes, (size_t)m->max_batch * (2 * ((m->H + 1) / 2) + 2) * 16));
     ws.ready = true;
     return COVAHIP_OK;
 }
@@ -409,13 +411,14 @@
 
 int covahip_blobnet_set_impl(covahip_ctx *ctx, int impl) {
     if (!ctx || !ctx->blobnet) return COVAHIP_ERR_NOT_LOADED;
-    if (impl != 1 && (impl < 4 || impl > 10)) return COVAHIP_ERR_INVALID_ARG;
+    if (impl != 1 && (impl < 4 || impl > 12)) return COVAHIP_ERR_INVALID_ARG;
     ctx->blobnet->fuse_dec = impl != 4;
     ctx->blobnet->enc1_tile16 = impl != 5;
     ctx->blobnet->enc_rowtiles = impl != 6;
     ctx->blobnet->fuse_enc23 = impl == 7 ? 0 : impl == 8 ? 2 : 1;
     ctx->blobnet->tail_part = impl != 9;
     ctx->blobnet->tail_rows = impl != 10;
+    ctx->blobnet->tail_in_dec012 = impl == 11 ? 2 : impl == 12 ? 0 : 1;
     return COVAHIP_OK;
 }
 
@@ -543,6 +546,12 @@
 int covahip_dev_blobnet_tail_form(covahip_ctx *ctx, int *form) {
     if (!ctx || !form) return COVAHIP_ERR_INVALID_ARG;
     *form = ctx->tail_form;
+    return COVAHIP_OK;
+}
+
+int covahip_dev_blobnet_tail_in_dec012(covahip_ctx *ctx, int *in_dec012) {
+    if (!ctx || !in_dec012) return COVAHIP_ERR_INVALID_ARG;
+    *in_dec012 = ctx->tail_in_dec012;
     return COVAHIP_OK;
 }
 
diff --git a/cova_amd/csrc/blobnet_mfma.hip b/cova_amd/csrc/blobnet_mfma.hip
--- a/cova_amd/csrc/blobnet_mfma.hip
+++ b/cova_amd/csrc/blobnet_mfma.hip
@@ -58,6 +58,10 @@
 __device__ __forceinline__ uint32_t model_off(const uint8_t *mid, uint32_t stride, int idx) {
     if constexpr (!MS) return 0u;
     else return __builtin_amdgcn_readfirstlane((uint32_t)mid[idx] * stride);
+}
+__device__ __forceinline__ int opaque_v(int v) {
+    asm volatile("" : "+v"(v));
+    return v;
 }
 template <typename T>
 __device__ __forceinline__ const T *at_model(const T *ptr, uint32_t off) {
@@ -1637,6 +1641,20 @@
     const uint8_t *model_ids;
     uint32_t mstride;
 };
+struct Dec012Tail {
+    DecLvl lv;
+    const half8 *wfrag;
+    const float *epi;
+    const float *part;
+    float *logits;
+    uint8_t *mask;
+    uint32_t *planes_out;
+    int planes_off, rows_bytes;
+    uint32_t mW4;
+};
+struct Dec012NoTail {};
+template <bool TAILF>
+using Dec012TailArg = std::conditional_t<TAILF, Dec012Tail, Dec012NoTail>;
 
 template <int C>
 __device__ __forceinline__ void dec012_zero_border(uint8_t *tile, const DecLvl &g, int tid) {
@@ -1741,7 +1759,31 @@
             __builtin_amdgcn_sched_group_barrier(0x008, 1, 0);
             if (ks + AD < KSTEPS) __builtin_amdgcn_sched_group_barrier(0x100, 1, 0);
         }
-        if constexpr (CN > 0) {
+        if constexpr (CN > 0 && COUT == 16) {
+            static_assert(CN == 16 && MT == 2, "the row tail's tile");
+            const int TCN = gn.Wi + 2;
+            const int Y = 2 * u + mtile - g.cy;
+            if (q < npos && Y >= 0 && Y < g.Hd) {
+#pragma unroll
+                for (int px = 0; px < 2; px++) {
+                    const int X = 2 * v + px - g.cx;
+                    if (X >= 0 && X < g.Wd) {
+                        const int yy = Y + 1, xx = X + 1;
+                        uint8_t *const pix = next_tile + (yy * TCN + xx) * 32 + kh * 8;
+                        const int sw = (xx >> 3) & 1;
+#pragma unroll
+                        for (int c = 0; c < 2; c++) {
+                            const int gq = 2 * px + c;
+                            half4 o;
+#pragma unroll
+                            for (int j = 0; j < 4; j++)
+                                o[j] = (_Float16)fmaxf(acc[4 * gq + j] * es[4 * gq + j] + eb[4 * gq + j], 0.f);
+                            *reinterpret_cast<half4 *>(pix + ((c ^ sw) * 16)) = o;
+                        }
+                    }
+                }
+            }
+        } else if constexpr (CN > 0) {
             constexpr int CPPN = CN / 8, PSN = CN * 2;
             const int TCN = gn.Wi + 2;
             static_assert(COUT >= 32 && COUT % 32 == 0, "one output pixel per lane and tile");
@@ -1796,22 +1838,115 @@
     }
 }
 
-template <bool MS = false>
-__global__ __launch_bounds__(512, 2) void dec012_mfma(Dec012Args p) {
+__device__ __forceinline__ void tail_row_lanes(uint32_t (&lc)[2][2], int GW, int lane) {
+    const int kh = lane >> 5, pos = lane & 31;
+#pragma unroll
+    for (int h = 0; h < 2; h++)
+#pragma unroll
+        for (int bb = 0; bb < 2; bb++) {
+            const int xx = min(32 * h + pos, GW - 1) + 1 - bb;
+            lc[h][bb] = (uint32_t)(xx * 32 + ((kh ^ ((xx >> 3) & 1)) << 4));
+        }
+}
+__device__ __forceinline__ f32x16 tail_row_acc(const uint8_t *tile, uint32_t row_b, const uint32_t (&lc)[2][2], const half8 (&wf)[4], int u, int h) {
+    const uint32_t rb = (uint32_t)(u * row_b);
+    const uint32_t a00 = rb + row_b + (h ? lc[1][0] : lc[0][0]), a01 = rb + row_b + (h ? lc[1][1] : lc[0][1]);
+    const uint32_t a10 = rb + (h ? lc[1][0] : lc[0][0]), a11 = rb + (h ? lc[1][1] : lc[0][1]);
+    f32x16 acc;
+#pragma unroll
+    for (int r = 0; r < 16; r++) acc[r] = 0.f;
+    acc = __builtin_amdgcn_mfma_f32_32x32x16_f16(wf[0], *reinterpret_cast<const half8 *>(tile + a00), acc, 0, 0, 0);
+    acc = __builtin_amdgcn_mfma_f32_32x32x16_f16(wf[1], *reinterpret_cast<const half8 *>(tile + a01), acc, 0, 0, 0);
+    acc = __builtin_amdgcn_mfma_f32_32x32x16_f16(wf[2], *reinterpret_cast<const half8 *>(tile + a10), acc, 0, 0, 0);
+    acc = __builtin_amdgcn_mfma_f32_32x32x16_f16(wf[3], *reinterpret_cast<const half8 *>(tile + a11), acc, 0, 0, 0);
+    return acc;
+}
+__device__ __forceinline__ void tail_row_out(const f32x16 acc, const f32x4 pl, float fbias, float thr, float *logits, int Hd, int Wd, int cy, int cx,
+                                             int GW, int b, int u, int h, int lane, uint32_t *planes) {
+    const int kh = lane >> 5, pos = lane & 31;
+    const int v = 32 * h + pos;
+    const bool live = kh == 0 && v < GW;
+    float l[4];
+#pragma unroll
+    for (int r = 0; r < 4; r++) l[r] = (acc[r] + fbias) + pl[r];
+    if (logits && live) {
+#pragma unroll
+        for (int r = 0; r < 4; r++) {
+            const int Y = 2 * u + (r >> 1) - cy, X = 2 * v + (r & 1) - cx;
+            if (Y >= 0 && Y < Hd && X >= 0 && X < Wd) logits[((size_t)b * Hd + Y) * Wd + X] = l[r];
+        }
+    }
+    uint32_t bal[4];
+#pragma unroll
+    for (int r = 0; r < 4; r++) bal[r] = (uint32_t)__ballot(live && l[r] > thr);
+    {
+        const int r = lane & 3;
+        const uint64_t bits = (uint64_t)(r == 0 ? bal[0] : r == 1 ? bal[1] : r == 2 ? bal[2] : bal[3]) << (32 * h);
+        const int Y = 2 * u + (r >> 1) - cy, X0 = (r & 1) - cx;
+        const int pln = X0 & 1, sh = X0 >> 1;
+        const int nb = (Wd - pln + 1) >> 1;
+        uint64_t w = sh >= 0 ? bits << sh : bits >> (-sh);
+        w &= nb >= 64 ? ~0ull : ((1ull << nb) - 1);
+        if (lane < 4 && Y >= 0 && Y < Hd && w)
+            atomicOr(reinterpret_cast<unsigned long long *>(planes + (Y + 1) * 4 + 2 * pln), (unsigned long long)w);
+    }
+}
+__device__ __forceinline__ void tail_row_tile(const uint8_t *tile, uint32_t row_b, const uint32_t (&lc)[2][2], const half8 (&wf)[4], const f32x4 pl,
+                                              float fbias, float thr, float *logits, int Hd, int Wd, int cy, int cx, int GW, int b, int u,
+                                              int h, int lane, uint32_t *planes) {
+    tail_row_out(tail_row_acc(tile, row_b, lc, wf, u, h), pl, fbias, thr, logits, Hd, Wd, cy, cx, GW, b, u, h, lane, planes);
+}
+template <int NTH>
+__device__ __forceinline__ void tail_mask_from_planes(const uint32_t *planes, uint8_t *mask_frame, int Hd, int Wd, uint32_t mW4, int tid) {
+    uint32_t *dst = reinterpret_cast<uint32_t *>(mask_frame);
+    const int wq = Wd >> 2, nq = Hd * wq;
+    for (int i = tid; i < nq; i += NTH) {
+        const int y = fdiv(i, mW4), xq = i - y * wq;
+        const int bx = 2 * xq;
+        const uint32_t *rw = planes + (y + 1) * 4 + (bx >> 5);
+        const uint32_t e2 = (rw[0] >> (bx & 31)) & 3u, o2 = (rw[2] >> (bx & 31)) & 3u;
+        dst[i] = (e2 & 1u) | ((o2 & 1u) << 8) | ((e2 >> 1) << 16) | ((o2 >> 1) << 24);
+    }
+}
+
+constexpr int DEC012_TI = 3, DEC012_PF = 2 * DEC012_TI;
+struct Dec012Fold {
+    half8 wf[4];
+    f32x4 ring[DEC012_PF];
+    float fbias;
+};
+struct Dec012NoFold {};
+__device__ __forceinline__ f32x4 dec012_part(const Dec012Tail &pt, int b, int t, int lane) {
+    const int GW = pt.lv.Wi + 1, GH = pt.lv.Hi + 1, tpr = GW > 32 ? 2 : 1;
+    const int tc = min(t, tpr * GH - 1);
+    const int u = tpr == 2 ? tc >> 1 : tc, h = tpr == 2 ? tc & 1 : 0;
+    return as_global(reinterpret_cast<const f32x4 *>(pt.part) + (size_t)b * GH * GW)[u * GW + min(32 * h + (lane & 31), GW - 1)];
+}
+
+template <bool MS = false, bool TAILF = false>
+__global__ __launch_bounds__(512, 2) void dec012_mfma(Dec012Args p, Dec012TailArg<TAILF> pt) {
+    static_assert(!(MS && TAILF), "the form that ends in planes is the single-model kernel's");
     extern __shared__ __attribute__((aligned(256))) uint8_t smem[];
     const int tid = threadIdx.x, lane = tid & 63, wave = tid >> 6;
     uint8_t *const t0 = smem + p.lv[0].tile_off, *const t1 = smem + p.lv[1].tile_off, *const t2 = smem + p.lv[2].tile_off;
     WGSPAN_BEGIN();
 #ifdef PHASE_TIMING
-    unsigned long long ph_[9] = {0, 0, 0, 0, 0, 0, 0, 0, 0}, last_ = __builtin_amdgcn_s_memrealtime();
+    unsigned long long ph_[12] = {0, 0, 0, 0, 0, 0, 0, 0, 0, 0, 0, 0}, last_ = __builtin_amdgcn_s_memrealtime();
 #endif
-    dec012_zero_border<128>(t0, p.lv[0], tid);
-    dec012_zero_border<128>(t1, p.lv[1], tid);
+    if constexpr (!TAILF) {
+        dec012_zero_border<128>(t0, p.lv[0], tid);
+        dec012_zero_border<128>(t1, p.lv[1], tid);
+    }
     dec012_zero_border<64>(t2, p.lv[2], tid);
     for (int b = blockIdx.x; b < p.B; b += gridDim.x) {
         [[maybe_unused]] const uint32_t moff = model_off<MS>(p.model_ids, p.mstride, b);
         if (b != (int)blockIdx.x) lds_barrier();
         PHASE_MARK(0);
+        if constexpr (TAILF) {
+            const int tid_f = opaque_v(tid);
+            dec012_zero_border<128>(t0, p.lv[0], tid_f);
+            dec012_zero_border<128>(t1, p.lv[1], tid_f);
+        }
         {
             dec012_stage<0, 128>(t0, p.skip[0] + (size_t)b * p.Ts[0] * p.lv[0].Hi * p.lv[0].Wi * 128, p.lv[0], wave, lane, 0);
             dec012_stage<64, 64>(t1, p.skip[1] + (size_t)b * p.Ts[1] * p.lv[1].Hi * p.lv[1].Wi * 64, p.lv[1], wave, lane, p.lv[0].Hi & 7);
@@ -1838,6 +1973,7 @@
             dec012_block<64, 64, 32, 64>(smem, t1, t2, nullptr, nullptr, w1, p.lv[1], p.lv[2], wave, lane);
         }
         PHASE_MARK(5);
+        [[maybe_unused]] std::conditional_t<TAILF, Dec012Fold, Dec012NoFold> fold;
         {
             Dec012W<64, 16> w2;
             dec012_load(w2, at_model(p.wf[2], moff), at_model(p.epi[2], moff), wave, lane);
@@ -1846,14 +1982,73 @@
             asm volatile("s_waitcnt vmcnt(0)" ::: "memory");
 #endif
             PHASE_MARK(6);
-            dec012_block<32, 32, 16, 0>(smem, t2, nullptr, p.out + (size_t)b * p.lv[2].Hd * p.lv[2].Wd * 16, smem + p.scr_off, w2,
-                                        p.lv[2], p.lv[2], wave, lane);
+            if constexpr (!TAILF) {
+                dec012_block<32, 32, 16, 0>(smem, t2, nullptr, p.out + (size_t)b * p.lv[2].Hd * p.lv[2].Wd * 16, smem + p.scr_off, w2,
+                                            p.lv[2], p.lv[2], wave, lane);
+            } else {
+                uint8_t *const t3 = smem + pt.lv.tile_off;
+                const int tid_f = opaque_v(tid);
+                dec012_zero_border<16>(t3, pt.lv, tid_f);
+                for (int i = tid_f; i < pt.rows_bytes / 4; i += 512) reinterpret_cast<uint32_t *>(smem + pt.planes_off)[i] = 0;
+                const gptr<half8> wg = as_global(pt.wfrag);
+#pragma unroll
+                for (int ks = 0; ks < 4; ks++) fold.wf[ks] = wg[ks * 64 + (tid_f & 63)];
+                fold.fbias = pt.epi[0];
+#pragma unroll
+                for (int k = 0; k < DEC012_PF; k++) fold.ring[k] = dec012_part(pt, b, (tid_f >> 6) + 8 * k, tid_f & 63);
+                dec012_block<32, 32, 16, 16>(smem, t2, t3, nullptr, nullptr, w2, p.lv[2], pt.lv, wave, lane);
+            }
         }
         PHASE_MARK(7);
+        if constexpr (TAILF) {
+            const int tid = opaque_v((int)threadIdx.x), lane = tid & 63, wave = tid >> 6;
+            const DecLvl &g = pt.lv;
+            const int GW = g.Wi + 1, GH = g.Hi + 1;
+            const uint32_t row_b = (uint32_t)((g.Wi + 2) * 32);
+            const uint8_t *const t3 = smem + g.tile_off;
+            uint32_t *const planes = reinterpret_cast<uint32_t *>(smem + pt.planes_off);
+            const int tpr = GW > 32 ? 2 : 1, ntl = tpr * GH;
+            uint32_t lc[2][2];
+            tail_row_lanes(lc, GW, lane);
+            lds_barrier();
+            PHASE_MARK(8);
+            for (int t0 = wave; t0 < ntl; t0 += 8 * DEC012_TI) {
+                f32x4 pl[DEC012_TI];
+                f32x16 acc[DEC012_TI];
+#pragma unroll
+                for (int j = 0; j < DEC012_TI; j++) pl[j] = fold.ring[j];
+#pragma unroll
+                for (int k = 0; k + DEC012_TI < DEC012_PF; k++) fold.ring[k] = fold.ring[k + DEC012_TI];
+#pragma unroll
+                for (int j = 0; j < DEC012_TI; j++) fold.ring[DEC012_PF - DEC012_TI + j] = dec012_part(pt, b, t0 + 8 * (DEC012_PF + j), lane);
+#pragma unroll
+                for (int j = 0; j < DEC012_TI; j++) {
+                    const int t = t0 + 8 * j < ntl ? t0 + 8 * j : t0;
+                    acc[j] = tail_row_acc(t3, row_b, lc, fold.wf, tpr == 2 ? t >> 1 : t, tpr == 2 ? t & 1 : 0);
+                }
+#pragma unroll
+                for (int j = 0; j < DEC012_TI; j++) {
+                    const int t = t0 + 8 * j;
+                    if (t < ntl)
+                        tail_row_out(acc[j], pl[j], fold.fbias, 0.f, pt.logits, g.Hd, g.Wd, g.cy, g.cx, GW, b, tpr == 2 ? t >> 1 : t, tpr == 2 ? t & 1 : 0,
+                                     lane, planes);
+                }
+            }
+            PHASE_MARK(9);
+            lds_barrier();
+            PHASE_MARK(10);
+            {
+                const uint4 *const src = reinterpret_cast<const uint4 *>(planes);
+                uint4 *const dst = reinterpret_cast<uint4 *>(pt.planes_out) + (size_t)b * (pt.rows_bytes / 16);
+                for (int i = tid; i < pt.rows_bytes / 16; i += 512) dst[i] = src[i];
+            }
+            if (pt.mask) tail_mask_from_planes<512>(planes, pt.mask + (size_t)b * g.Hd * g.Wd, g.Hd, g.Wd, pt.mW4, tid);
+            PHASE_MARK(11);
+        }
     }
 #ifdef PHASE_TIMING
     if (tid == 0)
-        for (int i = 0; i < 9; i++) atomicAdd(&g_phase[48 + i], ph_[i]);
+        for (int i = 0; i < 12; i++) atomicAdd(&g_phase[48 + i], ph_[i]);
 #endif
     WGSPAN_END(3);
 }
@@ -2019,7 +2214,7 @@
     const DecArgs &p = q.d;
     const int tid = threadIdx.x, lane = tid & 63, wave = tid >> 6;
     const int TC = p.Wi + 2, GW = p.Wi + 1, GH = p.Hi + 1;
-    const int kh = lane >> 5, pos = lane & 31;
+    const int pos = lane & 31;
     const float fbias0 = p.epi[0];
     uint32_t *const planes = reinterpret_cast<uint32_t *>(smem + q.mfull_off);
     const f32x4 *const part = reinterpret_cast<const f32x4 *>(smem + q.part_off);
@@ -2028,13 +2223,7 @@
     unsigned long long ph_[9] = {0, 0, 0, 0, 0, 0, 0, 0, 0}, last_ = __builtin_amdgcn_s_memrealtime();
 #endif
     uint32_t lc[2][2];
-#pragma unroll
-    for (int h = 0; h < 2; h++)
-#pragma unroll
-        for (int bb = 0; bb < 2; bb++) {
-            const int xx = min(32 * h + pos, GW - 1) + 1 - bb;
-            lc[h][bb] = (uint32_t)(xx * PS + ((kh ^ ((xx >> 3) & 1)) << 4));
-        }
+    tail_row_lanes(lc, GW, lane);
     const int row_b = TC * PS;
     for (int b = blockIdx.x; b < p.B; b += gridDim.x) {
         const uint32_t moff = model_off<MS>(q.ms.model_ids, q.ms.mstride, b);
@@ -2083,43 +2272,9 @@
         for (int t = wave; t < 2 * GH; t += NW) {
             const int u = t >> 1, h = t & 1;
             if (32 * h >= GW) continue;
-            const uint32_t rb = (uint32_t)(u * row_b);
-            const uint32_t a00 = rb + row_b + (h ? lc[1][0] : lc[0][0]), a01 = rb + row_b + (h ? lc[1][1] : lc[0][1]);
-            const uint32_t a10 = rb + (h ? lc[1][0] : lc[0][0]), a11 = rb + (h ? lc[1][1] : lc[0][1]);
-            f32x16 acc;
-#pragma unroll
-            for (int r = 0; r < 16; r++) acc[r] = 0.f;
-            acc = __builtin_amdgcn_mfma_f32_32x32x16_f16(wf[0], *reinterpret_cast<const half8 *>(smem + a00), acc, 0, 0, 0);
-            acc = __builtin_amdgcn_mfma_f32_32x32x16_f16(wf[1], *reinterpret_cast<const half8 *>(smem + a01), acc, 0, 0, 0);
-            acc = __builtin_amdgcn_mfma_f32_32x32x16_f16(wf[2], *reinterpret_cast<const half8 *>(smem + a10), acc, 0, 0, 0);
-            acc = __builtin_amdgcn_mfma_f32_32x32x16_f16(wf[3], *reinterpret_cast<const half8 *>(smem + a11), acc, 0, 0, 0);
             const int v = 32 * h + pos;
-            const bool live = kh == 0 && v < GW;
-            const f32x4 pl = part[u * GW + min(v, GW - 1)];
-            float l[4];
-#pragma unroll
-            for (int r = 0; r < 4; r++) l[r] = (acc[r] + fbias) + pl[r];
-            if (p.logits && live) {
-#pragma unroll
-                for (int r = 0; r < 4; r++) {
-                    const int Y = 2 * u + (r >> 1) - p.cy, X = 2 * v + (r & 1) - p.cx;
-                    if (Y >= 0 && Y < p.Hd && X >= 0 && X < p.Wd) p.logits[((size_t)b * p.Hd + Y) * p.Wd + X] = l[r];
-                }
-            }
-#pragma unroll
-            for (int r = 0; r < 4; r++) {
-                const uint64_t bits = (uint64_t)(uint32_t)__ballot(live && l[r] > sp.thr) << (32 * h);
-                const int Y = 2 * u + (r >> 1) - p.cy, X0 = (r & 1) - p.cx;
-                const int pln = X0 & 1, sh = X0 >> 1;
-                const int nb = (p.Wd - pln + 1) >> 1;
-                uint64_t w = sh >= 0 ? bits << sh : bits >> (-sh);
-                w &= nb >= 64 ? ~0ull : ((1ull << nb) - 1);
-                if (Y >= 0 && Y < p.Hd && lane == 0) {
-                    uint32_t *rw = planes + (Y + 1) * 4 + 2 * pln;
-                    if ((uint32_t)w) atomicOr(rw, (uint32_t)w);
-                    if ((uint32_t)(w >> 32)) atomicOr(rw + 1, (uint32_t)(w >> 32));
-                }
-            }
+            tail_row_tile(smem, (uint32_t)row_b, lc, wf, part[u * GW + min(v, GW - 1)], fbias, sp.thr, p.logits, p.Hd, p.Wd, p.cy, p.cx, GW, b, u, h,
+                          lane, planes);
         }
         PHASE_MARK(4);
         lds_barrier();
@@ -2128,17 +2283,7 @@
             lds_barrier();
         }
         PHASE_MARK(5);
-        if (p.mask) {
-            uint32_t *dst = reinterpret_cast<uint32_t *>(p.mask + (size_t)b * p.Hd * p.Wd);
-            const int wq = p.Wd >> 2, nq = p.Hd * wq;
-            for (int i = tid; i < nq; i += NW * 64) {
-                const int y = fdiv(i, p.mRC), xq = i - y * wq;
-                const int bx = 2 * xq;
-                const uint32_t *rw = planes + (y + 1) * 4 + (bx >> 5);
-                const uint32_t e2 = (rw[0] >> (bx & 31)) & 3u, o2 = (rw[2] >> (bx & 31)) & 3u;
-                dst[i] = (e2 & 1u) | ((o2 & 1u) << 8) | ((e2 >> 1) << 16) | ((o2 >> 1) << 24);
-            }
-        }
+        if (p.mask) tail_mask_from_planes<NW * 64>(planes, p.mask + (size_t)b * p.Hd * p.Wd, p.Hd, p.Wd, p.mRC, tid);
         PHASE_MARK(6);
         ccwave::frame_wg<ccbody::CC_THREADS, true>(nullptr, smem + q.cc_off, q.wg, stack_area<POST, MS>(qp, q.ms.model_ids, b, q.area_thresh), q.boxes + (size_t)b * q.max_boxes,
                                                    q.counts + b, q.max_boxes, tid, planes);
@@ -2148,6 +2293,30 @@
     if (tid == 0)
         for (int i = 0; i < 9; i++) atomicAdd(&g_phase[64 + i], ph_[i]);
 #endif
+    WGSPAN_END(4);
+}
+
+struct CcPlanesArgs {
+    const uint32_t *planes;
+    ccwave::WvGeom wg;
+    covahip_box *boxes;
+    int32_t *counts;
+    int B, area_thresh, max_boxes;
+    int cc_off, planes_off;
+};
+__global__ __launch_bounds__(ccbody::CC_THREADS) void cc_planes(CcPlanesArgs q) {
+    extern __shared__ __attribute__((aligned(16))) uint8_t smem[];
+    const int tid = threadIdx.x;
+    uint32_t *const planes = reinterpret_cast<uint32_t *>(smem + q.planes_off);
+    WGSPAN_BEGIN();
+    for (int b = blockIdx.x; b < q.B; b += gridDim.x) {
+        if (b != (int)blockIdx.x) lds_barrier();
+        const uint4 *const src = reinterpret_cast<const uint4 *>(q.planes) + (size_t)b * (q.wg.rows_bytes / 16);
+        for (int i = tid; i < q.wg.rows_bytes / 16; i += ccbody::CC_THREADS) reinterpret_cast<uint4 *>(planes)[i] = src[i];
+        lds_barrier();
+        ccwave::frame_wg<ccbody::CC_THREADS, true>(nullptr, smem + q.cc_off, q.wg, q.area_thresh, q.boxes + (size_t)b * q.max_boxes, q.counts + b,
+                                                   q.max_boxes, tid, planes);
+    }
     WGSPAN_END(4);
 }
 
@@ -2417,6 +2586,7 @@
 
 
 constexpr size_t LDS_LIMIT = 160 * 1024 - 256;
+constexpr bool TAIL_IN_DEC012_AUTO = true;
 
 template <typename F>
 int with_bools(F &&f) {
@@ -2721,14 +2891,22 @@
     }, ap, rowtiles, f.ms));
 }
 
-bool run_dec012(const Fwd &f, int &rc) {
+struct TailPlan {
+    Dec3ccArgs t;
+    size_t lds;
+    bool rows;
+    bool in_dec012;
+};
+
+bool run_dec012(const Fwd &f, int &rc, const TailPlan *tail, bool &tail_in) {
     const covahip_blobnet *m = f.m;
     const Prepared *pr = f.pr;
+    tail_in = false;
     if (!(m->fuse_dec && m->dec_ci[0] == 128 && m->dec_ci[1] == 128 && m->dec_ci[2] == 64 && m->dec_co[0] == 64 &&
           m->dec_co[1] == 32 && m->dec_co[2] == 16))
         return false;
     Dec012Args a;
-    size_t off = 0;
+    size_t off = 0, tile_bytes[3];
     for (int j = 0; j < 3; j++) {
         const BnLevelGeom in = m->lv[BN_LEVELS - j], out = m->lv[BN_LEVELS - 1 - j];
         DecLvl &g = a.lv[j];
@@ -2737,7 +2915,8 @@
         g.mRC = magic((in.W + 2) * (m->dec_ci[j] / 8));
         g.swz = choose_swz(false, m->dec_ci[j], in.W, 0, in.H + 1);
         g.tile_off = (int)off;
-        off += align256((size_t)(in.H + 2) * (in.W + 2) * m->dec_ci[j] * 2);
+        tile_bytes[j] = align256((size_t)(in.H + 2) * (in.W + 2) * m->dec_ci[j] * 2);
+        off += tile_bytes[j];
         a.skip[j] = f.ws.act[BN_LEVELS - j];
         a.Ts[j] = j == 0 ? 1 : BN_T;
         a.wf[j] = (const half8 *)(f.prep + pr->dec[j].wfrag);
@@ -2748,10 +2927,41 @@
     if (lds > 160 * 1024 - 256) return false;
     a.out = f.ws.dact[2]; a.B = f.batch; a.zero = f.prep + pr->zero;
     a.model_ids = f.inp.model_ids; a.mstride = f.mstride;
+    const int grid = std::min(f.batch, f.num_cu);
+    if (tail && m->tail_in_dec012 && !f.ms && !f.post && f.ws.planes &&
+        (m->tail_in_dec012 == 2 || (TAIL_IN_DEC012_AUTO && tail->rows && 4 * f.batch >= 3 * f.num_cu && !f.d_logits))) {
+        const DecArgs &d = tail->t.d;
+        Dec012Tail t;
+        t.lv = DecLvl{d.Hi, d.Wi, d.Hd, d.Wd, d.cy, d.cx, 0u, 0u, Swz{3, 1, 0, 0, 0}, 0};
+        const size_t t3 = align256((size_t)(d.Hi + 2) * (d.Wi + 2) * 32);
+        const size_t t2_off = std::max(tile_bytes[0] + tile_bytes[1], t3);
+        const size_t planes_off = t2_off + tile_bytes[2];
+        const size_t lds_t = planes_off + (size_t)tail->t.wg.rows_bytes;
+        if (lds_t <= LDS_LIMIT) {
+            a.lv[2].tile_off = (int)t2_off;
+            a.scr_off = 0; a.out = nullptr;
+            t.wfrag = d.wfrag; t.epi = d.epi; t.part = d.part; t.logits = d.logits; t.mask = d.mask;
+            t.planes_out = f.ws.planes;
+            t.planes_off = (int)planes_off; t.rows_bytes = tail->t.wg.rows_bytes;
+            t.mW4 = magic(d.Wd / 4);
+            tail_in = true;
+            rc = launched(f, launch(f, "dec012_mfma", dec012_mfma<false, true>, grid, 512, lds_t, a, t));
+            return true;
+        }
+    }
     rc = launched(f, with_bools([&](auto MS) {
-        return launch(f, "dec012_mfma", dec012_mfma<MS.value>, std::min(f.batch, f.num_cu), 512, lds, a);
+        return launch(f, "dec012_mfma", dec012_mfma<MS.value, false>, grid, 512, lds, a, Dec012NoTail{});
     }, f.ms));
     return true;
+}
+int run_cc_planes(const Fwd &f, const TailPlan &tp) {
+    CcPlanesArgs q;
+    q.planes = f.ws.planes; q.wg = tp.t.wg;
+    q.boxes = f.cc->boxes; q.counts = f.cc->counts;
+    q.B = f.batch; q.area_thresh = f.cc->area_thresh; q.max_boxes = f.cc->max_boxes;
+    q.cc_off = 0; q.planes_off = tp.t.wg.wave_bytes;
+    const size_t lds = (size_t)tp.t.wg.wave_bytes + (size_t)tp.t.wg.rows_bytes;
+    return launch(f, "dec3_bboxcc_fused", cc_planes, std::min(f.batch, 2 * f.num_cu), ccbody::CC_THREADS, lds, q);
 }
 
 struct DecPlan {
@@ -2828,10 +3038,10 @@
     return launch_dec_block(f, j, p);
 }
 
-bool run_tail_fused(const Fwd &f, const DecPlan &p) {
+bool plan_tail_fused(const Fwd &f, const DecPlan &p, TailPlan &tp) {
     const BnLevelGeom in = p.in, out = p.out;
     const int GH = p.GH;
-    Dec3ccArgs t;
+    Dec3ccArgs &t = tp.t;
     size_t cc_bytes = ccbody::cc_plan(out.H, out.W, t.g);
     t.use_wv = f.ctx->cc_wave_cap >= 0 && ccwave::wv_plan(out.H, out.W, ((out.H + 1) / 2) * ((out.W + 1) / 2), t.wg) ? 1 : 0;
     if (t.use_wv) cc_bytes = (size_t)t.wg.wave_bytes;
@@ -2863,12 +3073,21 @@
     t.tile_bytes = (int)tb; t.cc_off = 0;
     t.mfull_off = (int)std::max((best_nb == 1 ? 1 : 2) * tb, cc_bytes);
     t.part_off = (int)((size_t)t.mfull_off + mfull);
-    const size_t tl = (size_t)t.part_off + partb;
-    const int grid = std::min(f.batch, 2 * f.num_cu);
-    if (p.half && t.use_wv && best_nb == 1 && in.W + 1 <= 64 && f.m->tail_rows && (out.W & 7) == 0 &&
-        (size_t)t.wg.rows_bytes <= mfull && (!f.d_mask || (reinterpret_cast<uintptr_t>(f.d_mask) & 3) == 0)) {
+    tp.lds = (size_t)t.part_off + partb;
+    tp.in_dec012 = p.half && t.use_wv && in.W + 1 <= 64 && f.m->tail_rows && (out.W & 7) == 0 &&
+                   (!f.d_mask || (reinterpret_cast<uintptr_t>(f.d_mask) & 3) == 0);
+    tp.rows = tp.in_dec012 && best_nb == 1 && (size_t)t.wg.rows_bytes <= mfull;
+    if (tp.rows) {
         t.d.swz = Swz{3, 1, 0, 0, 0};
         t.d.mRC = magic(out.W / 4);
+    }
+    return true;
+}
+bool launch_tail_fused(const Fwd &f, const DecPlan &p, const TailPlan &tp) {
+    const Dec3ccArgs &t = tp.t;
+    const size_t tl = tp.lds;
+    const int grid = std::min(f.batch, 2 * f.num_cu);
+    if (tp.rows) {
         if (!f.dry) f.ctx->tail_form = COVAHIP_DEV_TAIL_ROWS;
         return !with_bools([&](auto MS, auto POST) {
             return launch(f, "dec3_bboxcc_fused", dec3cc_rows_mfma<MS.value, POST.value>, grid, ccbody::CC_THREADS, tl, t, post_arg<POST.value>(f));
@@ -2919,13 +3138,22 @@
         if (!rc) rc = run_enc_level(f, 3);
     }
     if (rc) return rc;
-    if (!run_dec012(f, rc))
-        for (int j = 0; j < BN_LEVELS - 1 && !rc; j++) rc = run_dec_block(f, j);
-    if (rc) return rc;
     DecPlan last;
     rc = plan_dec_block(f, BN_LEVELS - 1, last);
     if (rc) return rc;
-    if (!(cc && m->fuse_tail && run_tail_fused(f, last))) {
+    TailPlan tp;
+    const bool fused = cc && m->fuse_tail && plan_tail_fused(f, last, tp);
+    bool tail_in = false;
+    if (!run_dec012(f, rc, fused && tp.in_dec012 ? &tp : nullptr, tail_in))
+        for (int j = 0; j < BN_LEVELS - 1 && !rc; j++) rc = run_dec_block(f, j);
+    if (rc) return rc;
+    if (!dry) ctx->tail_in_dec012 = tail_in;
+    if (tail_in) {
+        if (!dry) ctx->tail_form = COVAHIP_DEV_TAIL_ROWS;
+        if (cc_done) *cc_done = true;
+        return launched(f, run_cc_planes(f, tp));
+    }
+    if (!(fused && launch_tail_fused(f, last, tp))) {
         if (!dry) ctx->tail_form = COVAHIP_DEV_TAIL_ALONE;
         return launch_dec_block(f, BN_LEVELS - 1, last);
     }
diff --git a/cova_amd/csrc/internal.h b/cova_amd/csrc/internal.h
--- a/cova_amd/csrc/internal.h
+++ b/cova_amd/csrc/internal.h
@@ -98,6 +98,7 @@
     size_t sweep_bytes = 0;
     ResidentTable<int32_t> cc_area;
     int cc_wave_cap = 0;
+    int tail_in_dec012 = 0;
     int tail_form = 0;
     CtxLane &lane() { return lanes[cur_lane]; }
     struct { int nbands, nbuf; } enc_plan[4] = {};
diff --git a/cova_amd/elements.py b/cova_amd/elements.py
--- a/cova_amd/elements.py
+++ b/cova_amd/elements.py
@@ -228,7 +228,7 @@
         L.check(self._lib.covahip_blobnet_set_enc_plan(self.ctx.handle, level, nbands, nbuf), "covahip_blobnet_set_enc_plan")
 
     def set_impl(self, impl: str):
-        L.check(self._lib.covahip_blobnet_set_impl(self.ctx.handle, {"mfma": 1, "dec_separate": 4, "enc1_legacy": 5, "enc_general_tiles": 6, "enc23_separate": 7, "enc23_force": 8, "tail_skip_tensor": 9, "tail_band_tiles": 10}[impl]), "set_impl")
+        L.check(self._lib.covahip_blobnet_set_impl(self.ctx.handle, {"mfma": 1, "dec_separate": 4, "enc1_legacy": 5, "enc_general_tiles": 6, "enc23_separate": 7, "enc23_force": 8, "tail_skip_tensor": 9, "tail_band_tiles": 10, "tail_in_dec012": 11, "tail_separate": 12}[impl]), "set_impl")
 
     TAIL_ALONE, TAIL_ROWS, TAIL_BANDS = 1, 2, 4
 
@@ -236,6 +236,11 @@
         v = C.c_int()
         L.check(self._lib.covahip_dev_blobnet_tail_form(self.ctx.handle, C.byref(v)), "covahip_dev_blobnet_tail_form")
         return v.value
+
+    def tail_in_dec012(self) -> bool:
+        v = C.c_int()
+        L.check(self._lib.covahip_dev_blobnet_tail_in_dec012(self.ctx.handle, C.byref(v)), "covahip_dev_blobnet_tail_in_dec012")
+        return bool(v.value)
 
     def read_buffer(self, which: int, index: int = 0) -> np.ndarray:
         p, n, dims = C.c_void_p(), C.c_size_t(), (C.c_int32 * 5)()
diff --git a/include/covahip_dev.h b/include/covahip_dev.h
--- a/include/covahip_dev.h
+++ b/include/covahip_dev.h
@@ -26,6 +26,7 @@
 #define COVAHIP_DEV_TAIL_ROWS 2
 #define COVAHIP_DEV_TAIL_BANDS 4
 int covahip_dev_blobnet_tail_form(covahip_ctx *ctx, int *form);
+int covahip_dev_blobnet_tail_in_dec012(covahip_ctx *ctx, int *in_dec012);
 
 struct covahip_pipe;
 int covahip_dev_pipe_queue_plan(struct covahip_pipe *pipe, int *lanes_on_upload_queue, int *lanes_on_result_queue);
```
